# kchmck/p25rx

Measured on AMD Instinct MI355X. Metric: IQ Msamples/s through FM-demod+C4FM slice, higher is better.
Workload: dtype f32

## Files before the change

p25rx_amd/csrc/p25fe_api.hip:

```cpp
#include "p25fe_kernels.hip"

#include <hip/hip_ext.h>
#include <math.h>
#include <stdio.h>
#include <stdlib.h>
#include <string.h>

#include <chrono>
#include <new>
#include <utility>
#include <string>
#include <vector>

#include "p25fe_jit.h"

using namespace p25k;

namespace {

constexpr size_t BBPAD = 256;
constexpr size_t SHARD_HALO = 2560;
static_assert(SHARD_HALO >= (size_t)(DEC * (PLPAD + CLK_L + 160) + TMAX) && 160 >= TMAX + TMAX - 1 && SHARD_HALO % 8 == 0, "shard halo");
constexpr uint32_t STATE_MAGIC = 0x50323546u;

struct DevBuf {
    void* p = nullptr;
    size_t cap = 0;
    DevBuf() = default; DevBuf(const DevBuf&) = delete; DevBuf& operator=(const DevBuf&) = delete;
    ~DevBuf() { release(); }
    hipError_t ensure(size_t bytes)
    {
        if (bytes <= cap) return hipSuccess;
        if (p) { hipError_t e = hipFree(p); if (e != hipSuccess) return e; p = nullptr; cap = 0; }
        size_t want = bytes + bytes / 8 + 256;
        hipError_t e = hipMalloc(&p, want);
        if (e != hipSuccess) { p = nullptr; return e; }
        cap = want;
        return hipSuccess;
    }
    void release() { if (p) (void)hipFree(p); p = nullptr; cap = 0; }
    template <class T> T* as() const { return reinterpret_cast<T*>(p); }
};
template <class T> struct DevArr {
    DevBuf buf;
    hipError_t ensure(size_t count) { return buf.ensure(count * sizeof(T)); }
    T* get() const { return static_cast<T*>(buf.p); }
};

struct PinBuf {
    void* p = nullptr;
    void* dp = nullptr;
    size_t cap = 0;
    PinBuf() = default; PinBuf(const PinBuf&) = delete; PinBuf& operator=(const PinBuf&) = delete;
    ~PinBuf() { release(); }
    hipError_t ensure(size_t bytes)
    {
        if (bytes <= cap) return hipSuccess;
        release();
        const size_t want = bytes + bytes / 4 + 4096;
        hipError_t e = hipHostMalloc(&p, want, hipHostMallocCoherent | hipHostMallocMapped);
        if (e != hipSuccess) { (void)hipGetLastError(); e = hipHostMalloc(&p, want, hipHostMallocDefault); }
        if (e != hipSuccess) { p = nullptr; return e; }
        e = hipHostGetDevicePointer(&dp, p, 0);
        if (e != hipSuccess) { (void)hipHostFree(p); p = dp = nullptr; return e; }
        cap = want;
        return hipSuccess;
    }
    void release() { if (p) (void)hipHostFree(p); p = dp = nullptr; cap = 0; }
};

inline size_t round_up(size_t v, size_t m) { return (v + m - 1) / m * m; }

struct Arena {
    char* hp; char* dp; size_t off = 0;
    Arena(const PinBuf& b) : hp(static_cast<char*>(b.p)), dp(static_cast<char*>(b.dp)) {}
    template <class T> T* take(size_t count, T** dev)
    {
        T* r = reinterpret_cast<T*>(hp + off);
        *dev = reinterpret_cast<T*>(dp + off);
        off += round_up(count * sizeof(T), 64);
        return r;
    }
};

template <class... Args, class... Act>
inline void launch_ev(void (*kern)(Args...), dim3 grid, dim3 block, size_t lds, hipStream_t st, hipEvent_t e0, hipEvent_t e1,
                      Act... args)
{
    if (e0 || e1) hipExtLaunchKernelGGL(kern, grid, block, (uint32_t)lds, st, e0, e1, 0u, Args(args)...);
    else hipLaunchKernelGGL(kern, grid, block, lds, st, Args(args)...);
}
inline size_t fmt_bytes(int fmt) { return fmt == P25FE_FMT_CF32 ? 8 : 2; }

static_assert(BBPAD == (size_t)TAILN && BBPAD >= (size_t)HIST_BB + CLK_L, "baseband tail kept between calls");

constexpr int MAX_LANES = 4;
constexpr int SH_FLAG_WORDS = 8, SH_FLAG_ERR = 4;
constexpr int PROF_RING = 64, PROF_SAMPLE = 8;

struct RxScratch {
    DevArr<float> pl_f; DevArr<uint32_t> pl_bits;
    DevArr<uint16_t> evl; DevArr<float> evthr;
    DevArr<TileRec> recs; DevArr<unsigned long long> tsum; DevArr<ScanOut> outs;
    DevArr<GroupAgg> gagg; DevArr<GroupPre> gpre; DevArr<unsigned> gtick;
    DevArr<TileSumG> gsum; DevArr<ScanOutG> gouts; DevArr<uint32_t> evg;
    DevArr<GroupSumG> gsg; DevArr<GroupPreG> gpg;
};

struct Lane {
    RxScratch s;
    hipEvent_t ev_k1 = nullptr, ev_rx = nullptr;
    bool pending = false;
    hipStream_t joined = nullptr; bool joined_any = false;
};

static inline void rotate_lanes(int* cur, int* q, int depth)
{
    const int next = q[0];
    for (int k = 0; k + 2 < depth; ++k) q[k] = q[k + 1];
    q[depth - 2] = *cur;
    *cur = next;
}

struct ShardCtx {
    bool valid = false;
    bool main_out = false;
    size_t main_nbb = 0; uint64_t main_abs0 = 0;
    bool head_done = false;
    bool head_flagged = false;
    DevBuf flag;
    unsigned seq = 0; int head_tile_max = -1;
    size_t nbb = 0; long abs_bb0 = 0;
    bool gen = false;
    bool pipe = false;
    bool scan_fresh = false;
    bool main_is(size_t n_bb, uint64_t abs0) const { return main_out && main_nbb == n_bb && main_abs0 == abs0; }
    void invalidate() { valid = false; main_out = false; head_done = false; head_flagged = false; }
    void finish_pass1(size_t n_bb, long bb0, bool general) { valid = true; nbb = n_bb; abs_bb0 = bb0; gen = general; scan_fresh = true; main_out = false; head_done = false; }
};

struct StateHeader { uint32_t magic, abi; int32_t n_channels, fmt_locked; uint64_t abs_iq, abs_bb; };

struct StreamState {
    uint64_t abs_iq = 0, abs_bb = 0;
    int fmt_locked = -1;
    std::vector<char> hist_iq;
    std::vector<float> tail_bb;
    std::vector<p25fe_anchor_t> anchor;
    std::vector<uint64_t> total_dibits;
    void reset(size_t C)
    {
        abs_iq = 0; fmt_locked = -1; abs_bb = 0;
        anchor.assign(C, p25fe_anchor_t{0, 0.f, 0.f, 0.f, 0, SPS, 1}); total_dibits.assign(C, 0);
        hist_iq.assign(C * SHARD_HALO * 8, 0); tail_bb.assign(C * BBPAD, 0.f);
    }
    bool format_refused(int fmt) const { return fmt_locked >= 0 && fmt_locked != fmt && abs_iq > 0; }
    size_t n_hist() const { return abs_iq < SHARD_HALO ? (size_t)abs_iq : SHARD_HALO; }
    void commit_iq(size_t C, int fmt, size_t n, const char* fresh, size_t row_bytes)
    {
        const size_t eb = fmt_bytes(fmt);
        for (size_t c = 0; c < C; ++c) {
            char* hist = hist_iq.data() + c * SHARD_HALO * 8;
            const char* src = fresh + c * row_bytes;
            if (n >= SHARD_HALO) memcpy(hist, src + (n - SHARD_HALO) * eb, SHARD_HALO * eb);
            else { memmove(hist, hist + n * eb, (SHARD_HALO - n) * eb); memcpy(hist + (SHARD_HALO - n) * eb, src, n * eb); }
        }
        fmt_locked = fmt; abs_iq += n;
    }
    void merge_tail(size_t c, size_t nb, long look, const float* fresh)
    {
        float* t = tail_bb.data() + c * BBPAD;
        float merged[BBPAD];
        for (size_t j = 0; j < (size_t)BBPAD; ++j) {
            const long m = (long)nb - (long)BBPAD + (long)j;
            merged[j] = m >= -(long)(HIST_BB + look) ? fresh[j] : t[j + nb];
        }
        memcpy(t, merged, sizeof merged);
    }
    struct Sec { void* p; size_t bytes; };
    void sections(Sec s[4])
    {
        s[0] = {hist_iq.data(), hist_iq.size()}; s[1] = {tail_bb.data(), tail_bb.size() * sizeof(float)};
        s[2] = {anchor.data(), anchor.size() * sizeof(p25fe_anchor_t)}; s[3] = {total_dibits.data(), total_dibits.size() * sizeof(uint64_t)};
    }
    size_t blob_size() { Sec s[4]; sections(s); return sizeof(StateHeader) + s[0].bytes + s[1].bytes + s[2].bytes + s[3].bytes; }
    void write(char* p)
    {
        StateHeader hd = {STATE_MAGIC, P25FE_ABI_VERSION, (int32_t)anchor.size(), fmt_locked, abs_iq, abs_bb};
        memcpy(p, &hd, sizeof hd); p += sizeof hd;
        Sec s[4]; sections(s);
        for (int k = 0; k < 4; ++k) { memcpy(p, s[k].p, s[k].bytes); p += s[k].bytes; }
    }
    bool read(const char* p, int track)
    {
        StateHeader hd;
        memcpy(&hd, p, sizeof hd); p += sizeof hd;
        if (hd.magic != STATE_MAGIC || hd.abi != P25FE_ABI_VERSION || hd.n_channels != (int32_t)anchor.size()) return false;
        if (hd.fmt_locked != -1 && hd.fmt_locked != P25FE_FMT_U8 && hd.fmt_locked != P25FE_FMT_CF32) return false;
        if (hd.abs_iq >= P25FE_MAX_POSITION || hd.abs_bb >= P25FE_MAX_POSITION) return false;
        Sec s[4]; sections(s);
        for (size_t c = 0; c < anchor.size(); ++c) {
            p25fe_anchor_t a;
            memcpy(&a, p + s[0].bytes + s[1].bytes + c * sizeof a, sizeof a);
            if (!(a.period_d == 0 && a.period_n == 0) && !clock_plausible(a.period_d, a.period_n)) return false;
            if (!track && a.valid != 0 && !(a.period_d == 0 && a.period_n == 0) && !(a.period_d == SPS && a.period_n == 1)) return false;
            if (a.valid != 0 && (a.s >= (int64_t)P25FE_MAX_POSITION || a.s <= -(int64_t)P25FE_MAX_POSITION)) return false;
        }
        for (int k = 0; k < 4; ++k) { memcpy(s[k].p, p, s[k].bytes); p += s[k].bytes; }
        fmt_locked = hd.fmt_locked; abs_iq = hd.abs_iq; abs_bb = hd.abs_bb;
        return true;
    }
};

struct Prof {
    bool on = false;
    int level = 1;
    std::vector<hipEvent_t> ev;
    std::vector<uint8_t> mask;
    uint64_t calls = 0, seq = 0;
    int slot = -1;
    void begin()
    {
        if (on && level == 3 && (seq++ % PROF_SAMPLE) != 0) { slot = -1; return; }
        slot = on ? (int)(calls++ % PROF_RING) : -1;
        if (slot >= 0) mask[(size_t)slot] = 0;
    }
    void end() { slot = -1; }
    void mark(int idx, hipStream_t st, bool ext_events)
    {
        if (slot < 0 || (idx > 1 && level != 1) || (idx <= 1 && ext_events)) return;
        if (hipEventRecord(ev[(size_t)slot * 5 + idx], st) == hipSuccess) mask[(size_t)slot] |= (uint8_t)(1u << idx);
    }
    void k1_events(bool ext_events, hipEvent_t* e0, hipEvent_t* e1)
    {
        *e0 = *e1 = nullptr;
        if (slot < 0 || !ext_events) return;
        *e0 = ev[(size_t)slot * 5 + 0]; *e1 = ev[(size_t)slot * 5 + 1];
        mask[(size_t)slot] |= 3u;
    }
};

struct Windows {
    DevBuf buf[2], dib[2], res, anc;
    PinBuf stage[2], out;
    hipStream_t cs = nullptr, os = nullptr;
    hipEvent_t ev[4][5] = {};
    hipError_t ensure()
    {
        if (cs) return hipSuccess;
        hipError_t e = hipStreamCreateWithFlags(&cs, hipStreamNonBlocking);
        if (e == hipSuccess) e = hipStreamCreateWithFlags(&os, hipStreamNonBlocking);
        for (auto& slot : ev) for (hipEvent_t& x : slot) if (e == hipSuccess) e = hipEventCreate(&x);
        return e;
    }
};

}

struct p25fe {
    p25fe_config_t cfg;
    int C = 1, n_cu = 256;
    Taps taps;
    int k1_p = 5;
    int variant = P25FE_VARIANT_BUILTIN;
    bool long_taps = false;
    int phase = P25FE_DECIM_PHASE;
    int n_avg = BOX;
    bool u8_lut_mode = false;
    int track = 0;
    bool causal_ok = false;
    long look = 0;
    bool ext_events = true;
    int rx_cus = 0;
    int run_depth = 2;
    int sh_depth = MAX_LANES;

    int last_hip = 0;
    DevBuf d_taps;
    hipModule_t jit_mod = nullptr;
    hipFunction_t jit_fn[2][3] = {{nullptr, nullptr, nullptr}, {nullptr, nullptr, nullptr}};
    hipStream_t stream = nullptr, rx_stream = nullptr;
    const long* rs_idx = nullptr; size_t rs_n = 0, rs_stride = 0;
    Lane lanes[MAX_LANES];
    int cur = 0, lane_q[MAX_LANES - 1] = {1, 2, 3};
    Lane& lane() { return lanes[cur]; }
    RxScratch& rx() { return lanes[cur].s; }
    const RxScratch& rx() const { return lanes[cur].s; }
    DevBuf power_partial, chunk_cnt, evrec, evnext, evoff;
    unsigned long long ev_seq = 0;
    PinBuf hin, hbb, hout;
    unsigned chunk_seq = 0;
    Windows win; StreamState state; Prof prof; ShardCtx sh;
};

struct PlanarGeo {
    size_t n_tiles, n_blocks;
    explicit PlanarGeo(size_t n_bb)
    {
        n_tiles = (n_bb + TS - 1) / TS;
        if (n_tiles == 0) n_tiles = 1;
        n_blocks = (size_t)TWORDS * n_tiles + 6;
    }
    size_t floats() const { return n_blocks * PL_BLK; }
    size_t words() const { return n_blocks * SPS; }
};

constexpr size_t MAX_RANGE_BB = (size_t)0x7ff00000u * 10u;
static inline bool position_refused(uint64_t pos) { return pos >= P25FE_MAX_POSITION; }

struct Resolved {
    Taps taps;
    bool long_taps;
    bool lut_affine;
    float u8_scale, u8_offset;
    bool dflt;
};

static inline bool finite_f(float v) { return v - v == 0.0f; }
static inline bool same_bits(float a, float b) { return memcmp(&a, &b, sizeof a) == 0; }

static bool lut_is_affine(const float* lut, float sc, float of)
{
    for (int b = 0; b < 256; ++b)
        if (!same_bits(lut[b], fmaf((float)b, sc, of))) return false;
    return true;
}

static int resolve_config(const p25fe_config_t* cfg, Resolved* r)
{
    if (cfg->abi_version != P25FE_ABI_VERSION || cfg->n_decim_taps < 1 || cfg->n_decim_taps > P25FE_MAX_TAPS || cfg->n_chan_taps < 1 ||
        cfg->n_chan_taps > P25FE_MAX_TAPS || (cfg->symbol_clock != P25FE_CLOCK_FIXED && cfg->symbol_clock != P25FE_CLOCK_TRACKING && cfg->symbol_clock != P25FE_CLOCK_TRACKING_RESLICE &&
         cfg->symbol_clock != (P25FE_CLOCK_TRACKING_RESLICE | P25FE_CLOCK_CAUSAL_OK)) ||
        cfg->specialize < P25FE_SPECIALIZE_OFF || cfg->specialize > P25FE_SPECIALIZE_FORCE || cfg->decim_phase < 0 || cfg->decim_phase >= DEC ||
        cfg->n_avg_taps < 1 || cfg->n_avg_taps > P25FE_MAX_TAPS)
        return P25FE_ERR_ARG;
    memset(&r->taps, 0, sizeof r->taps);
    r->taps.n_avg = cfg->n_avg_taps;
    r->taps.avg_uniform = 1;
    for (int k = 0; k < cfg->n_avg_taps; ++k) {
        if (!finite_f(cfg->avg_taps[k])) return P25FE_ERR_ARG;
        r->taps.avg[k] = cfg->avg_taps[k];
        if (!same_bits(cfg->avg_taps[k], cfg->avg_taps[0])) r->taps.avg_uniform = 0;
    }
    for (int k = 0; k < cfg->n_decim_taps; ++k) { if (!finite_f(cfg->decim_taps[k])) return P25FE_ERR_ARG; r->taps.dec[k] = cfg->decim_taps[k]; }
    for (int k = 0; k < cfg->n_chan_taps; ++k) { if (!finite_f(cfg->chan_taps[k])) return P25FE_ERR_ARG; r->taps.ch[k] = cfg->chan_taps[k]; }
    r->long_taps = cfg->n_decim_taps > P25FE_T1 || cfg->n_chan_taps > P25FE_T2;
    if (cfg->fm_gain != 0.0f) {
        if (!finite_f(cfg->fm_gain)) return P25FE_ERR_ARG;
        r->taps.fm_gain = cfg->fm_gain;
    } else {
        if (cfg->fm_deviation_hz == 0 || cfg->fm_sample_rate_hz == 0) return P25FE_ERR_ARG;
        r->taps.fm_gain = (float)((double)cfg->fm_sample_rate_hz / (2.0 * M_PI * (double)cfg->fm_deviation_hz));
    }
    if (cfg->u8_lut_valid) {
        for (int b = 0; b < 256; ++b) { if (!finite_f(cfg->u8_lut[b])) return P25FE_ERR_ARG; r->taps.lut[b] = cfg->u8_lut[b]; }
        const float* L = r->taps.lut;
        const float cand[3][2] = {{cfg->u8_scale, cfg->u8_offset}, {L[1] - L[0], L[0]},
                                  {(float)(((double)L[255] - (double)L[0]) / 255.0), L[0]}};
        r->lut_affine = false;
        for (int c = 0; c < 3 && !r->lut_affine; ++c)
            if (finite_f(cand[c][0]) && finite_f(cand[c][1]) && lut_is_affine(L, cand[c][0], cand[c][1])) {
                r->lut_affine = true; r->u8_scale = cand[c][0]; r->u8_offset = cand[c][1];
            }
        if (!r->lut_affine) r->u8_scale = r->u8_offset = 0.0f;
    } else {
        if (!finite_f(cfg->u8_scale) || !finite_f(cfg->u8_offset)) return P25FE_ERR_ARG;
        r->lut_affine = true; r->u8_scale = cfg->u8_scale; r->u8_offset = cfg->u8_offset;
        for (int b = 0; b < 256; ++b) r->taps.lut[b] = fmaf((float)b, cfg->u8_scale, cfg->u8_offset);
    }
    Taps def;
    memset(&def, 0, sizeof def);
    memcpy(def.dec, P25FE_DEFAULT_DECIM_TAPS, sizeof(float) * P25FE_T1);
    memcpy(def.ch, P25FE_DEFAULT_CHAN_TAPS, sizeof(float) * P25FE_T2);
    memcpy(def.avg, P25FE_DEFAULT_AVG_TAPS, sizeof(float) * BOX);
    r->dflt = !r->long_taps && memcmp(def.dec, r->taps.dec, sizeof def.dec) == 0 && memcmp(def.ch, r->taps.ch, sizeof def.ch) == 0 &&
              r->taps.n_avg == BOX && memcmp(def.avg, r->taps.avg, sizeof def.avg) == 0 &&
              same_bits(r->taps.fm_gain, P25FE_FM_GAIN) && r->lut_affine && same_bits(r->u8_scale, P25FE_U8_SCALE) &&
              same_bits(r->u8_offset, P25FE_U8_OFFSET);
    return P25FE_OK;
}

static p25jit::Spec jit_spec(const Resolved& r)
{
    p25jit::Spec s;
    memset(&s, 0, sizeof s);
    s.tx = r.long_taps ? 1 : 0;
    s.t1 = r.long_taps ? TMAX : T1;
    s.t2 = r.long_taps ? TMAX : T2;
    memcpy(s.dec, r.taps.dec, sizeof s.dec);
    memcpy(s.ch, r.taps.ch, sizeof s.ch);
    s.fm_gain = r.taps.fm_gain;
    s.u8_lut = r.lut_affine ? 0 : 1;
    s.u8_scale = r.u8_scale; s.u8_offset = r.u8_offset;
    s.n_avg = r.taps.n_avg; s.avg_uniform = r.taps.avg_uniform;
    memcpy(s.avg, r.taps.avg, sizeof s.avg);
    return s;
}

static thread_local std::string t_jit_log;

static std::vector<std::string> jit_dirs()
{
    std::vector<std::string> d;
    const char* e = getenv("P25FE_SPEC_DIR");
    if (e && *e) d.push_back(e);
    d.push_back(p25jit::default_cache_dir());
    return d;
}

static void fallback_notice()
{
    static bool said = false;
    if (said) return;
    said = true;
    const char* q = getenv("P25FE_QUIET");
    if (q && atoi(q) != 0) return;
    fprintf(stderr, "p25fe: no specialised kernels for this configuration's numbers (no usable cached code object and hipRTC did not "
                    "deliver one): running the GENERIC kernels, 1.3 - 2.4 x slower.  p25fe_specialize_log() has the details; "
                    "p25fe_specialize() / $P25FE_SPEC_DIR is the ahead-of-time form.\n");
}

static int choose_variant(const p25fe_config_t* cfg, const Resolved& rs, std::vector<char>* code, std::string* path, bool* from_cache)
{
    static const bool jit_env_off = [] { const char* v = getenv("P25FE_JIT"); return v && atoi(v) == 0; }();
    const bool must = cfg->specialize >= P25FE_SPECIALIZE_REQUIRE;
    const bool want_jit = (!rs.dflt || cfg->specialize == P25FE_SPECIALIZE_FORCE) && cfg->specialize != P25FE_SPECIALIZE_OFF && !(jit_env_off && !must);
    const int plain = rs.dflt ? P25FE_VARIANT_BUILTIN : P25FE_VARIANT_GENERIC;
    if (!want_jit) return plain;
    bool ok = false;
    try {
        t_jit_log.clear();
        ok = p25jit::get_code(jit_spec(rs), jit_dirs(), true, p25jit::default_cache_dir(), false, *code, *path, t_jit_log, from_cache);
    } catch (...) {
        ok = false;
        try { t_jit_log += "exception while specialising\n"; } catch (...) { }
    }
    if (ok) return P25FE_VARIANT_SPECIALIZED;
    if (must) return P25FE_ERR_JIT;
    if (plain == P25FE_VARIANT_GENERIC) fallback_notice();
    return plain;
}

#define HIPCHK(h, expr)                                                        \
    do {                                                                       \
        hipError_t e__ = (expr);                                               \
        if (e__ != hipSuccess) { (h)->last_hip = (int)e__; return P25FE_ERR_HIP; } \
    } while (0)

extern "C" {

void p25fe_default_config(p25fe_config_t* cfg)
{
    if (!cfg) return;
    memset(cfg, 0, sizeof *cfg);
    cfg->abi_version = P25FE_ABI_VERSION;
    cfg->device = 0;
    cfg->n_channels = 1;
    cfg->n_decim_taps = P25FE_T1;
    cfg->n_chan_taps = P25FE_T2;
    memcpy(cfg->decim_taps, P25FE_DEFAULT_DECIM_TAPS, sizeof(float) * P25FE_T1);
    memcpy(cfg->chan_taps, P25FE_DEFAULT_CHAN_TAPS, sizeof(float) * P25FE_T2);
    cfg->specialize = P25FE_SPECIALIZE_AUTO;
    cfg->fm_deviation_hz = P25FE_FM_DEVIATION_HZ;
    cfg->fm_sample_rate_hz = P25FE_FM_SAMPLE_RATE_HZ;
    cfg->fm_gain = 0.0f;
    cfg->u8_scale = P25FE_U8_SCALE;
    cfg->u8_offset = P25FE_U8_OFFSET;
    cfg->u8_lut_valid = 0;
    cfg->decim_phase = P25FE_DECIM_PHASE;
    cfg->n_avg_taps = P25FE_BOXCAR;
    memcpy(cfg->avg_taps, P25FE_DEFAULT_AVG_TAPS, sizeof(float) * P25FE_BOXCAR);
}

const char* p25fe_strerror(int status)
{
    switch (status) {
    case P25FE_OK: return "ok";
    case P25FE_ERR_ARG: return "invalid argument";
    case P25FE_ERR_NO_DEVICE: return "no usable HIP device (gfx950 required; there is no CPU fallback)";
    case P25FE_ERR_HIP: return "HIP runtime error";
    case P25FE_ERR_CAPACITY: return "output buffer too small";
    case P25FE_ERR_FORMAT: return "sample format changed within a stream";
    case P25FE_ERR_NOMEM: return "out of memory";
    case P25FE_ERR_JIT: return "kernel specialisation failed (p25fe_specialize_log)";
    case P25FE_ERR_TIMEOUT: return "a device-side wait gave up (time shard: the head segment never arrived)";
    default: return "unknown status";
    }
}

int p25fe_last_hip_error(const p25fe_t* h) { return h ? h->last_hip : 0; }
int p25fe_device(const p25fe_t* h) { return h ? h->cfg.device : -1; }
int p25fe_kernel_variant(const p25fe_t* h) { return h ? h->variant : -1; }

size_t p25fe_specialize_log(char* buf, size_t cap)
{
    if (!buf || cap == 0) return 0;
    const size_t n = t_jit_log.size() < cap - 1 ? t_jit_log.size() : cap - 1;
    memcpy(buf, t_jit_log.data(), n);
    buf[n] = '\0';
    return n;
}

int p25fe_specialize(const p25fe_config_t* cfg, const char* dir, char* path_out, size_t path_cap)
{
    if (!cfg) return P25FE_ERR_ARG;
    if (path_out && path_cap) path_out[0] = '\0';
    Resolved r;
    const int rc = resolve_config(cfg, &r);
    if (rc) return rc;
    if (r.dflt && cfg->specialize != P25FE_SPECIALIZE_FORCE) return P25FE_OK;
    try {
        t_jit_log.clear();
        const std::string d = (dir && *dir) ? std::string(dir) : p25jit::default_cache_dir();
        std::vector<char> code;
        std::string path;
        if (!p25jit::get_code(jit_spec(r), {d}, true, d, true, code, path, t_jit_log) || path.empty()) return P25FE_ERR_JIT;
        if (path_out && path_cap) snprintf(path_out, path_cap, "%s", path.c_str());
    } catch (...) {
        return P25FE_ERR_NOMEM;
    }
    return P25FE_OK;
}

int p25fe_probe_variant(const p25fe_config_t* cfg)
{
    if (!cfg) return P25FE_ERR_ARG;
    Resolved r;
    const int rc = resolve_config(cfg, &r);
    if (rc) return rc;
    std::vector<char> code;
    std::string path;
    try {
        return choose_variant(cfg, r, &code, &path, nullptr);
    } catch (...) {
        return P25FE_ERR_NOMEM;
    }
}

static inline size_t n_baseband_ph(int phase, uint64_t abs0, size_t n)
{
    const size_t o0 = (size_t)(((uint64_t)phase + 5 - abs0 % 5) % 5);
    return n > o0 ? (n - o0 - 1) / 5 + 1 : 0;
}
size_t p25fe_n_baseband(uint64_t abs0, size_t n) { return n_baseband_ph(P25FE_DECIM_PHASE, abs0, n); }
size_t p25fe_n_baseband_h(const p25fe_t* h, uint64_t abs0, size_t n) { return n_baseband_ph(h ? h->phase : P25FE_DECIM_PHASE, abs0, n); }

size_t p25fe_shard_halo(void) { return SHARD_HALO; }

int p25fe_reset(p25fe_t* h)
{
    if (!h) return P25FE_ERR_ARG;
    h->rs_idx = nullptr; h->rs_n = 0; h->rs_stride = 0;
    try {
        h->state.reset((size_t)h->C);
    } catch (...) {
        return P25FE_ERR_NOMEM;
    }
    return P25FE_OK;
}

int p25fe_create(const p25fe_config_t* cfg, p25fe_t** out)
{
    if (!cfg || !out) return P25FE_ERR_ARG;
    *out = nullptr;
    if (cfg->abi_version != P25FE_ABI_VERSION || cfg->n_channels < 1 || cfg->n_channels > 65535 ) return P25FE_ERR_ARG;
    Resolved rs;
    if (int rrc = resolve_config(cfg, &rs)) return rrc;
    int ndev = 0;
    if (hipGetDeviceCount(&ndev) != hipSuccess || ndev <= 0 || cfg->device < 0 || cfg->device >= ndev)
        return P25FE_ERR_NO_DEVICE;
    if (hipSetDevice(cfg->device) != hipSuccess) return P25FE_ERR_NO_DEVICE;
    hipDeviceProp_t prop;
    if (hipGetDeviceProperties(&prop, cfg->device) != hipSuccess) return P25FE_ERR_NO_DEVICE;
    if (strncmp(prop.gcnArchName, "gfx950", 6) != 0) return P25FE_ERR_NO_DEVICE;

    p25fe_t* h = new (std::nothrow) p25fe;
    if (!h) return P25FE_ERR_NOMEM;
    h->cfg = *cfg;
    h->C = cfg->n_channels;
    h->track = cfg->symbol_clock & 0xff;
    h->causal_ok = (cfg->symbol_clock & P25FE_CLOCK_CAUSAL_OK) != 0;
    h->look = h->track ? CLK_L : 0;
    h->n_cu = prop.multiProcessorCount > 0 ? prop.multiProcessorCount : 256;
    h->taps = rs.taps;
    h->phase = cfg->decim_phase;
    h->n_avg = rs.taps.n_avg;
    h->long_taps = rs.long_taps;
    h->u8_lut_mode = !rs.lut_affine;
    h->variant = rs.dflt ? P25FE_VARIANT_BUILTIN : P25FE_VARIANT_GENERIC;
    if (hipStreamCreateWithFlags(&h->stream, hipStreamNonBlocking) != hipSuccess) { p25fe_destroy(h); return P25FE_ERR_HIP; }
    hipError_t e = hipSuccess;
    {
        const char* pv = getenv("P25FE_K1_P");
        h->k1_p = (pv && atoi(pv) == 3) ? 3 : 5;
        const char* ee = getenv("P25FE_EXT_EVENTS");
        h->ext_events = !(ee && atoi(ee) == 0);
        const char* rc_ = getenv("P25FE_RX_CUS");
        h->rx_cus = rc_ ? atoi(rc_) : 0;
        const char* pd = getenv("P25FE_SHARD_PIPE_DEPTH");
        if (pd && atoi(pd) >= 2 && atoi(pd) <= MAX_LANES) h->sh_depth = atoi(pd);
        if (cfg->symbol_clock != P25FE_CLOCK_FIXED) h->run_depth = 3;
        const char* rd = getenv("P25FE_PIPE_DEPTH");
        if (rd && atoi(rd) >= 2 && atoi(rd) <= MAX_LANES) h->run_depth = atoi(rd);
    }
    if (e == hipSuccess) e = h->d_taps.ensure(sizeof(Taps));
    if (e == hipSuccess) e = hipMemcpy(h->d_taps.p, &h->taps, sizeof(Taps), hipMemcpyHostToDevice);
    if (e != hipSuccess) { p25fe_destroy(h); return P25FE_ERR_HIP; }
    {
        std::vector<char> code;
        std::string path;
        bool from_cache = false;
        int var = choose_variant(cfg, rs, &code, &path, &from_cache);
        if (var < 0) { p25fe_destroy(h); return var; }
        if (var == P25FE_VARIANT_SPECIALIZED) {
            bool ok = false;
            try {
                hipError_t me = hipModuleLoadData(&h->jit_mod, code.data());
                if (me != hipSuccess && from_cache) {
                    (void)hipGetLastError();
                    t_jit_log += "cached code object " + path + " did not load: recompiling\n";
                    const std::string store = p25jit::default_cache_dir();
                    if (path.compare(0, store.size() + 1, store + "/") == 0) (void)remove(path.c_str());
                    h->jit_mod = nullptr;
                    if (p25jit::get_code(jit_spec(rs), {}, true, store, false, code, path, t_jit_log)) me = hipModuleLoadData(&h->jit_mod, code.data());
                }
                ok = me == hipSuccess;
                for (int f = 0; f < 2 && ok; ++f)
                    for (int k = 0; k < 3 && ok; ++k)
                        ok = hipModuleGetFunction(&h->jit_fn[f][k], h->jit_mod, p25jit::KERNEL_NAMES[f][k]) == hipSuccess;
                if (!ok) { (void)hipGetLastError(); t_jit_log += "loading the specialised code object failed\n"; }
            } catch (...) {
                ok = false;
            }
            if (!ok) {
                if (h->jit_mod) { (void)hipModuleUnload(h->jit_mod); h->jit_mod = nullptr; }
                if (cfg->specialize >= P25FE_SPECIALIZE_REQUIRE) { p25fe_destroy(h); return P25FE_ERR_JIT; }
                var = rs.dflt ? P25FE_VARIANT_BUILTIN : P25FE_VARIANT_GENERIC;
                if (var == P25FE_VARIANT_GENERIC) fallback_notice();
            }
        }
        h->variant = var;
    }
    int rc = p25fe_reset(h);
    if (rc != P25FE_OK) { p25fe_destroy(h); return rc; }
    *out = h;
    return P25FE_OK;
}

void p25fe_destroy(p25fe_t* h)
{
    if (!h) return;
    (void)hipSetDevice(h->cfg.device);
    for (hipStream_t st : {h->stream, h->rx_stream, h->win.cs, h->win.os})
        if (st) { (void)hipStreamSynchronize(st); (void)hipStreamDestroy(st); }
    if (h->jit_mod) (void)hipModuleUnload(h->jit_mod);
    for (auto& slot : h->win.ev) for (hipEvent_t e : slot) if (e) (void)hipEventDestroy(e);
    for (Lane& l : h->lanes)
        for (hipEvent_t e : {l.ev_k1, l.ev_rx}) if (e) (void)hipEventDestroy(e);
    for (auto& e : h->prof.ev) if (e) (void)hipEventDestroy(e);
    delete h;
}

}

enum K1Part { K1_ALL = 0, K1_MAIN = 1, K1_HEAD = 2 };
struct K1Launch {
    const void* src = nullptr;
    int fmt = P25FE_FMT_CF32;
    size_t ch_stride = 0, n_hist = 0, n = 0;
    uint64_t abs0 = 0;
    float* bb = nullptr; size_t bb_stride = 0;
    float* power_dbm = nullptr;
    bool planar = false;
    K1Part part = K1_ALL;
    hipEvent_t ev0 = nullptr, ev1 = nullptr;
    const ChunkRecvArgs* chunk = nullptr;
    long* head_end = nullptr;
    unsigned* done_flag = nullptr; unsigned done_seq = 0u;
    hipStream_t stream = nullptr;
};

struct K1Plan {
    bool empty;
    K1Args a;
    bool u8, ct; int pk;
    long n_seg;
    long head_end;
    size_t lds;
};
static int k1_plan(const p25fe_t* h, const K1Launch& L, K1Plan* p)
{
    const int fmt = L.fmt;
    if (fmt != P25FE_FMT_CF32 && fmt != P25FE_FMT_U8) return P25FE_ERR_ARG;
    if ((reinterpret_cast<uintptr_t>(L.src) & 15u) != 0) return P25FE_ERR_ARG;
    if (h->C > 1 && (L.ch_stride % (fmt == P25FE_FMT_CF32 ? 2 : 8)) != 0) return P25FE_ERR_ARG;
    if (L.chunk && (!L.planar || L.part)) return P25FE_ERR_ARG;
    const bool pro = seg_prologue(fmt);
    const long m_begin = !L.planar ? 0 : (pro ? -(long)PLPAD - h->look : -(long)HIST_BB - h->look);
    const size_t n_out = p25fe_n_baseband_h(h, L.abs0, L.n);
    const long total = (long)n_out - m_begin;
    K1Args& a = p->a;
    a.m_begin = m_begin; a.n_out = (long)n_out; p->head_end = 0;
    p->empty = total <= 0;
    if (p->empty) return P25FE_OK;
    const int pk = (L.planar || h->long_taps || h->variant == P25FE_VARIANT_SPECIALIZED) ? 5 : h->k1_p;
    const int t1 = h->long_taps ? TMAX : T1;
    const long sub = (long)WV * pk;
    static const long subs_env = [] { const char* e = getenv("P25FE_SUBS"); return e ? atol(e) : 0L; }();
    long subs = subs_env > 0 ? subs_env : (fmt == P25FE_FMT_U8 ? 9 : 3);
    if (L.chunk) subs = 1;
    if (subs > 32768) subs = 32768;
    const bool ct = h->variant != P25FE_VARIANT_GENERIC;
    const int t2e = h->long_taps ? TMAX : T2;
    const int t3geo = ct ? h->n_avg : TMAX;
    const long segh = seg_halo_for(h->n_avg, t2e);
    const long seg_len = pro ? subs * sub : (sub - segh) + (subs - 1) * sub;
    const long nd = pro ? t3geo + t2e - 1 : segh;
    const long lead_len = pro ? sub : sub - segh;
    const long o0 = (long)(((uint64_t)h->phase + 5 - L.abs0 % 5) % 5);
    long lead = 0;
    if (L.part && subs > 1 && !L.chunk)
        while (lead < 64 && o0 + DEC * (m_begin + lead * lead_len - nd) - (t1 - 1) < 0 && lead * lead_len < total) ++lead;
    auto seg_start = [&](long k) { return k < lead ? m_begin + k * lead_len : m_begin + lead * lead_len + (k - lead) * seg_len; };
    const long n_seg = lead * lead_len >= total ? (total + lead_len - 1) / lead_len : lead + (total - lead * lead_len + seg_len - 1) / seg_len;
    const long pl_shift = PLPAD + h->look;
    if (L.planar && pro && (m_begin + pl_shift < 0 || (m_begin + pl_shift) % PL_BLK != 0 || seg_len % PL_BLK != 0)) return P25FE_ERR_ARG;
    if (L.planar && !pro && (m_begin + pl_shift < 0 || (m_begin + pl_shift) % 80 != 0 || seg_len % 80 != 0)) return P25FE_ERR_ARG;
    if (L.planar && n_out > MAX_RANGE_BB) return P25FE_ERR_ARG;
    long seg_first = 0, seg_count = n_seg;
    if (L.part) {
        if (L.power_dbm) return P25FE_ERR_ARG;
        long k_min = 0;
        while (k_min < n_seg && o0 + DEC * (seg_start(k_min) - nd) - (t1 - 1) < 0) ++k_min;
        if (L.part == K1_MAIN) { seg_first = k_min; seg_count = n_seg - k_min; }
        else seg_count = k_min;
        p->head_end = seg_start(k_min) - m_begin;
        p->empty = seg_count <= 0;
        if (p->empty) return P25FE_OK;
    }
    if (seg_count * (long)h->C > 0x7fffffffL) return P25FE_ERR_ARG;
    p->u8 = fmt == P25FE_FMT_U8; p->ct = ct; p->pk = pk; p->n_seg = n_seg;
    a.x = L.src; a.ch_stride = (long)L.ch_stride; a.n_hist = (long)L.n_hist; a.n_new = (long)L.n; a.o0 = (int)o0; a.n_ch = h->C;
    a.bb = L.bb; a.bb_stride = (long)L.bb_stride; a.power_partial = nullptr;
    a.subs_per_seg = (int)subs; a.seg_first = (int)seg_first; a.seg_count = (int)seg_count; a.lead_segs = (int)lead; a.seg_halo = (int)segh;
    a.bbp = nullptr; a.bbp_ch_stride = 0; a.bits = nullptr; a.bits_ch_stride = 0; a.pl_shift = (int)pl_shift;
    a.done_flag = L.planar ? L.done_flag : nullptr; a.done_seq = L.done_seq;
    if (L.planar) {
        const PlanarGeo g(n_out);
        a.bbp = h->rx().pl_f.get(); a.bbp_ch_stride = (long)g.floats();
        a.bits = reinterpret_cast<uint8_t*>(h->rx().pl_bits.get()); a.bits_ch_stride = (long)(4 * g.words());
    }
    const bool lut = p->u8 && (!ct || h->u8_lut_mode);
    p->lds = h->long_taps ? k1_lds_bytes<Geo<5, 1>>(ct, lut, t3geo) : (pk == 3 ? k1_lds_bytes<Geo<3>>(ct, lut, t3geo) : k1_lds_bytes<Geo<5>>(ct, lut, t3geo));
    static const size_t lds_pad_env = [] { const char* e = getenv("P25FE_K1_LDS_PAD"); return e ? (size_t)atol(e) : (size_t)0; }();
    p->lds += lds_pad_env;
    return P25FE_OK;
}

using K1Kernel = void (*)(K1Args, const Taps*);
using ChunkKernel = void (*)(K1Args, const Taps*, ChunkTail);
template <int FMT> static K1Kernel k1_kernel_of(bool ct, int pk, bool planar, bool long_taps)
{
    if (long_taps) return planar ? k_frontend<FMT, false, 5, OUT_PLANAR, 1> : k_frontend<FMT, false, 5, OUT_LINEAR, 1>;
    if (planar) return ct ? k_frontend<FMT, true, 5, OUT_PLANAR, 0> : k_frontend<FMT, false, 5, OUT_PLANAR, 0>;
    if (pk == 3) return ct ? k_frontend<FMT, true, 3, OUT_LINEAR, 0> : k_frontend<FMT, false, 3, OUT_LINEAR, 0>;
    return ct ? k_frontend<FMT, true, 5, OUT_LINEAR, 0> : k_frontend<FMT, false, 5, OUT_LINEAR, 0>;
}
template <int FMT> static ChunkKernel chunk_kernel_of(bool ct, bool long_taps)
{
    if (long_taps) return k_chunk<FMT, false, 1>;
    return ct ? k_chunk<FMT, true, 0> : k_chunk<FMT, false, 0>;
}

static int launch_k1(p25fe_t* h, const K1Launch& L)
{
    K1Plan p;
    if (int rc = k1_plan(h, L, &p)) return rc;
    if (L.head_end) *L.head_end = p.head_end;
    hipStream_t st = L.stream;
    if (p.empty) {
        if (L.power_dbm) HIPCHK(h, hipMemsetAsync(L.power_dbm, 0xff, sizeof(float) * (size_t)h->C, st));
        return P25FE_OK;
    }
    K1Args& a = p.a;
    if (L.power_dbm) {
        HIPCHK(h, h->power_partial.ensure(sizeof(float) * (size_t)h->C * (size_t)p.n_seg));
        a.power_partial = h->power_partial.as<float>();
    }
    ChunkTail tail;
    if (L.chunk) {
        if (!h->chunk_cnt.p) {
            HIPCHK(h, h->chunk_cnt.ensure(sizeof(unsigned) * (size_t)h->C));
            HIPCHK(h, hipMemsetAsync(h->chunk_cnt.p, 0, sizeof(unsigned) * (size_t)h->C, h->stream));
        }
        tail.r = *L.chunk; tail.counter = h->chunk_cnt.as<unsigned>(); tail.wg_per_ch = a.seg_count;
    }
    const Taps* dt = h->d_taps.as<Taps>();
    const dim3 grid((unsigned)a.seg_count, (unsigned)h->C);
    if (h->variant == P25FE_VARIANT_SPECIALIZED) {
        hipFunction_t f = h->jit_fn[p.u8 ? 1 : 0][L.chunk ? 2 : (L.planar ? 1 : 0)];
        void* params[3] = {&a, &dt, &tail};
        if (L.ev0 || L.ev1)
            HIPCHK(h, hipExtModuleLaunchKernel(f, grid.x * WV, grid.y, 1, WV, 1, 1, p.lds, st, params, nullptr, L.ev0, L.ev1, 0));
        else
            HIPCHK(h, hipModuleLaunchKernel(f, grid.x, grid.y, 1, WV, 1, 1, (unsigned)p.lds, st, params, nullptr));
    } else if (L.chunk) {
        const ChunkKernel k = p.u8 ? chunk_kernel_of<P25FE_FMT_U8>(p.ct, h->long_taps) : chunk_kernel_of<P25FE_FMT_CF32>(p.ct, h->long_taps);
        hipLaunchKernelGGL(k, grid, dim3(WV), p.lds, st, a, dt, tail);
    } else {
        const K1Kernel k = p.u8 ? k1_kernel_of<P25FE_FMT_U8>(p.ct, p.pk, L.planar, h->long_taps)
                                : k1_kernel_of<P25FE_FMT_CF32>(p.ct, p.pk, L.planar, h->long_taps);
        launch_ev(k, grid, dim3(WV), p.lds, st, L.ev0, L.ev1, a, dt);
    }
    HIPCHK(h, hipGetLastError());
    if (L.power_dbm) {
        hipLaunchKernelGGL(k_power_finish, dim3((unsigned)h->C), dim3(256), 0, st, a.power_partial, (int)p.n_seg, a.n_out, L.power_dbm);
        HIPCHK(h, hipGetLastError());
    }
    return P25FE_OK;
}

static int ensure_slice_scratch(p25fe_t* h, size_t n_bb)
{
    const size_t C = (size_t)h->C;
    const PlanarGeo g(n_bb);
    const size_t nt = C * g.n_tiles, ng = C * (size_t)n_groups_of((int)g.n_tiles);
    RxScratch& s = h->rx();
    HIPCHK(h, s.pl_f.ensure(C * g.floats())); HIPCHK(h, s.pl_bits.ensure(C * g.words()));
    HIPCHK(h, s.evl.ensure(nt * EVCAP)); HIPCHK(h, s.evthr.ensure(nt * EVTHR_N * 3));
    HIPCHK(h, s.recs.ensure(nt)); HIPCHK(h, s.tsum.ensure(nt)); HIPCHK(h, s.outs.ensure(nt));
    HIPCHK(h, s.gagg.ensure(ng)); HIPCHK(h, s.gpre.ensure(ng));
    const unsigned* before = s.gtick.get();
    HIPCHK(h, s.gtick.ensure(ng + C));
    if (s.gtick.get() != before) HIPCHK(h, hipMemset(s.gtick.get(), 0, s.gtick.buf.cap));
    if (h->track || h->rs_n) {
        HIPCHK(h, s.gsum.ensure(nt)); HIPCHK(h, s.gouts.ensure(nt)); HIPCHK(h, s.evg.ensure(nt * EVCAP));
        HIPCHK(h, s.gsg.ensure(ng)); HIPCHK(h, s.gpg.ensure(ng));
    }
    return P25FE_OK;
}

struct RecvRange {
    size_t n_bb = 0;
    long abs_bb0 = 0;
    const p25fe_anchor_t* anchor_in = nullptr;
};
struct RecvDest {
    uint8_t* dibits = nullptr; size_t dibit_stride = 0;
    uint8_t* dibits2 = nullptr;
    int64_t* sync_pos = nullptr; uint64_t* sync_dibit = nullptr;
    size_t sync_stride = 0;
    p25fe_result_t* result = nullptr;
};
struct RecvCall {
    bool gen = false;
    bool reslice = false;
    RecvOpt opt;
    RecvRange range;
    RecvDest dest;
    bool detect = true;
    bool slice = true;
    bool wait_head = false;
    const ShardFix* fix = nullptr;
    hipEvent_t ev_done = nullptr;
    hipStream_t stream = nullptr;
};
static RecvCall recv_call(const p25fe_t* h)
{
    RecvCall c;
    c.opt.track = h->track;
    c.opt.n_resync = (int)h->rs_n;
    c.opt.resync = h->rs_idx;
    c.opt.resync_stride = (long)h->rs_stride;
    c.gen = h->track != 0 || h->rs_n != 0;
    return c;
}
static inline int n_tiles_of(const RecvRange& r) { return r.n_bb ? (int)PlanarGeo(r.n_bb).n_tiles : 0; }

static Planar planar_view(const p25fe_t* h, const PlanarGeo& g)
{
    Planar p;
    p.f = h->rx().pl_f.get(); p.f_ch = (long)g.floats();
    p.bits = h->rx().pl_bits.get(); p.bits_ch = (long)g.words();
    return p;
}

template <class A> static void view_planes(const p25fe_t* h, const RecvRange& r, A* a)
{
    a->pl = planar_view(h, PlanarGeo(r.n_bb)); a->n = (long)r.n_bb; a->abs0 = r.abs_bb0;
    a->evl = h->rx().evl.get(); a->evthr = h->rx().evthr.get();
}
template <class A> static void view_tiles(const p25fe_t* h, A* a) { a->recs = h->rx().recs.get(); a->tsum = h->rx().tsum.get(); }
template <class A> static void view_general(const p25fe_t* h, A* a) { a->gsum = h->rx().gsum.get(); a->evg = h->rx().evg.get(); }
template <class A> static void view_scan(const p25fe_t* h, const RecvCall& rc, A* a)
{
    a->recs = h->rx().recs.get(); a->tickets = h->rx().gtick.get();
    a->n_tiles = n_tiles_of(rc.range); a->n = (long)rc.range.n_bb; a->abs0 = rc.range.abs_bb0; a->n_baseband = rc.range.n_bb;
    a->anchor_in = rc.range.anchor_in; a->result = rc.dest.result;
}
template <class A> static void view_dest(const RecvRange& r, const RecvDest& d, A* a)
{
    a->anchor_in = r.anchor_in;
    a->dibits = d.dibits; a->dibit_stride = (long)d.dibit_stride;
    a->sync_pos = (d.sync_pos && d.sync_dibit) ? d.sync_pos : nullptr; a->sync_dibit = d.sync_dibit; a->sync_stride = (long)d.sync_stride;
}

static int launch_planarize(p25fe_t* h, const float* d_bb, size_t bb_stride, size_t n_hist_bb, size_t n_bb, hipStream_t st)
{
    const PlanarGeo g(n_bb);
    PlanarizeArgs a;
    a.bb = d_bb; a.bb_stride = (long)bb_stride; a.n_hist = (long)n_hist_bb; a.n = (long)n_bb;
    a.f = h->rx().pl_f.get(); a.f_ch = (long)g.floats();
    a.bits = h->rx().pl_bits.get(); a.bits_ch = (long)g.words(); a.n_blocks = (long)g.n_blocks;
    a.shift = (int)h->look;
    hipLaunchKernelGGL(k_planarize, dim3((unsigned)((g.n_blocks + 1) / 2), (unsigned)h->C), dim3(WV * SPS), 0, st, a);
    HIPCHK(h, hipGetLastError());
    return P25FE_OK;
}

static int launch_detect(p25fe_t* h, const RecvCall& rc)
{
    DetArgs d;
    d.head_flag = nullptr; d.head_seq = 0u; d.head_tile_max = -1; d.head_err = nullptr;
    if (rc.wait_head) {
        d.head_flag = h->sh.flag.as<unsigned>(); d.head_seq = h->sh.seq; d.head_tile_max = h->sh.head_tile_max;
        d.head_err = h->sh.flag.as<unsigned>() + SH_FLAG_ERR;
    }
    view_planes(h, rc.range, &d); view_tiles(h, &d); view_general(h, &d);
    d.n_tiles = n_tiles_of(rc.range); d.opt = rc.opt;
    const dim3 grid((unsigned)d.n_tiles, (unsigned)h->C);
    if (rc.gen) hipLaunchKernelGGL(k_detect<true>, grid, dim3(WV), 0, rc.stream, d);
    else hipLaunchKernelGGL(k_detect<false>, grid, dim3(WV), 0, rc.stream, d);
    HIPCHK(h, hipGetLastError());
    return P25FE_OK;
}

enum ScanStep { SCAN_WHOLE, SCAN_RANGE, SCAN_TILES_G };
static int launch_scan(p25fe_t* h, const RecvCall& rc, ScanStep step, hipEvent_t ev_done)
{
    const dim3 grid = step == SCAN_RANGE ? dim3((unsigned)h->C) : dim3((unsigned)n_groups_of(n_tiles_of(rc.range)), (unsigned)h->C);
    if (rc.gen) {
        ScanArgsG c;
        view_scan(h, rc, &c);
        c.gsum = h->rx().gsum.get(); c.outs = h->rx().gouts.get(); c.gsg = h->rx().gsg.get(); c.gpg = h->rx().gpg.get();
        c.track = h->track;
        launch_ev(step == SCAN_WHOLE ? k_scan_tiles_g : step == SCAN_RANGE ? k_range_scan_g : k_scan_g_groups, grid, dim3(WV), 0, rc.stream,
                  nullptr, ev_done, c);
    } else {
        ScanArgs c;
        view_scan(h, rc, &c);
        c.tsum = h->rx().tsum.get(); c.outs = h->rx().outs.get(); c.gagg = h->rx().gagg.get(); c.gpre = h->rx().gpre.get();
        launch_ev(step == SCAN_WHOLE ? k_scan_tiles : k_range_scan, grid, dim3(WV), 0, rc.stream, nullptr, ev_done, c);
    }
    HIPCHK(h, hipGetLastError());
    return P25FE_OK;
}

static int launch_slice(p25fe_t* h, const RecvCall& rc)
{
    SliceArgs l;
    view_planes(h, rc.range, &l); view_tiles(h, &l); view_dest(rc.range, rc.dest, &l);
    l.n_tiles = n_tiles_of(rc.range); l.outs = h->rx().outs.get(); l.gpre = h->rx().gpre.get(); l.dibits2 = rc.dest.dibits2;
    if (rc.fix) l.fix = *rc.fix; else memset(&l.fix, 0, sizeof l.fix);
    launch_ev(k_slice, dim3((unsigned)l.n_tiles + (rc.fix ? 1u : 0u), (unsigned)h->C), dim3(WV), 0, rc.stream, nullptr, rc.ev_done, l);
    HIPCHK(h, hipGetLastError());
    return P25FE_OK;
}

static int launch_slice_g(p25fe_t* h, const RecvCall& rc)
{
    SliceArgsG l;
    view_planes(h, rc.range, &l); view_general(h, &l); view_dest(rc.range, rc.dest, &l);
    l.n_tiles = n_tiles_of(rc.range); l.outs = h->rx().gouts.get(); l.recs = h->rx().recs.get();
    l.track = h->track; l.dibits2 = rc.dest.dibits2;
    launch_ev(k_slice_g, dim3((unsigned)l.n_tiles, (unsigned)h->C), dim3(WV), 0, rc.stream, nullptr, rc.ev_done, l);
    HIPCHK(h, hipGetLastError());
    return P25FE_OK;
}

static int launch_slice_by_detection(p25fe_t* h, const RecvCall& rc)
{
    const size_t C = (size_t)h->C, n_bb = rc.range.n_bb;
    const int n_tiles = n_tiles_of(rc.range);
    hipStream_t st = rc.stream;
    size_t cap_ev = (size_t)n_tiles * EVCAP;
    const size_t bound = n_bb / (size_t)(W + 1) + (size_t)n_tiles + 8;
    if (bound < cap_ev) cap_ev = bound;
    const size_t stride = cap_ev + 2;
    HIPCHK(h, h->evrec.ensure(C * stride * sizeof(EvRec)));
    HIPCHK(h, h->evoff.ensure(C * (stride + 1) * sizeof(unsigned long long)));
    {
        const void* before = h->evnext.p;
        HIPCHK(h, h->evnext.ensure(C * stride * sizeof(EvNext)));
        if (h->evnext.p != before) HIPCHK(h, hipMemsetAsync(h->evnext.p, 0, h->evnext.cap, st));
    }
    EvArgs e;
    view_planes(h, rc.range, &e); view_general(h, &e); view_dest(rc.range, rc.dest, &e);
    e.n_tiles = n_tiles; e.outs = h->rx().gouts.get();
    e.rec = h->evrec.as<EvRec>(); e.nxt = h->evnext.as<EvNext>(); e.off = h->evoff.as<unsigned long long>();
    e.ev_stride = (long)stride; e.seq = ++h->ev_seq; e.result = rc.dest.result;
    hipLaunchKernelGGL(k_ev_collect, dim3((unsigned)n_tiles, (unsigned)h->C), dim3(WV), 0, st, e);
    HIPCHK(h, hipGetLastError());
    hipLaunchKernelGGL(k_ev_count, dim3((unsigned)(n_tiles < 1024 ? n_tiles : 1024), (unsigned)h->C), dim3(WV), 0, st, e);
    HIPCHK(h, hipGetLastError());
    hipLaunchKernelGGL(k_ev_scan, dim3((unsigned)h->C), dim3(WV), 0, st, e);
    HIPCHK(h, hipGetLastError());
    const size_t max_dibits = n_bb / (SPS - 1) + (size_t)n_tiles + 64;
    const size_t lim = rc.dest.dibit_stride < max_dibits ? rc.dest.dibit_stride : max_dibits;
    launch_ev(k_ev_slice, dim3((unsigned)((lim + WV * 4 - 1) / (WV * 4)), (unsigned)h->C), dim3(WV), 0, st, nullptr, rc.ev_done, e);
    HIPCHK(h, hipGetLastError());
    return P25FE_OK;
}

static int launch_recv(p25fe_t* h, const RecvCall& rc)
{
    const int n_tiles = n_tiles_of(rc.range);
    const bool detect = rc.detect && n_tiles != 0, slice = rc.slice && n_tiles != 0, scan = rc.fix == nullptr;
    hipStream_t st = rc.stream;
    int e = detect ? launch_detect(h, rc) : P25FE_OK;
    if (e) return e;
    h->prof.mark(2, st, h->ext_events);
    if (scan && (e = launch_scan(h, rc, detect ? SCAN_WHOLE : SCAN_RANGE, slice ? nullptr : rc.ev_done)) != P25FE_OK) return e;
    h->prof.mark(3, st, h->ext_events);
    if (slice) {
        if (!rc.gen) e = launch_slice(h, rc);
        else if ((e = launch_scan(h, rc, SCAN_TILES_G, nullptr)) == P25FE_OK) e = rc.reslice ? launch_slice_by_detection(h, rc) : launch_slice_g(h, rc);
        if (e) return e;
    }
    if (rc.ev_done && !scan && !slice) HIPCHK(h, hipEventRecord(rc.ev_done, st));
    h->prof.mark(4, st, h->ext_events);
    return P25FE_OK;
}

static int launch_k1_planar(p25fe_t* h, K1Launch& k, hipEvent_t k1_done, hipStream_t waiter)
{
    h->prof.mark(0, k.stream, h->ext_events);
    bool attached = false;
    if (p25fe_n_baseband_h(h, k.abs0, k.n)) {
        h->prof.k1_events(h->ext_events, &k.ev0, &k.ev1);
        if (k1_done && h->ext_events) {
            if (k.ev1) k1_done = k.ev1;
            else k.ev1 = k1_done;
            attached = true;
        }
        k.planar = true;
        if (int rc = launch_k1(h, k)) return rc;
    }
    if (k1_done) {
        if (!attached) HIPCHK(h, hipEventRecord(k1_done, k.stream));
        HIPCHK(h, hipStreamWaitEvent(waiter, k1_done, 0));
    }
    return P25FE_OK;
}

static int launch_planar_recv(p25fe_t* h, K1Launch& k, const RecvCall& rc, hipEvent_t k1_done = nullptr)
{
    if (int e = launch_k1_planar(h, k, k1_done, rc.stream)) return e;
    if (rc.range.n_bb) h->prof.mark(1, k.stream, h->ext_events);
    return launch_recv(h, rc);
}

static inline bool piecewise_refused(const p25fe_t* h) { return h->track == P25FE_CLOCK_TRACKING_RESLICE && !h->causal_ok; }

extern "C" {

int p25fe_demod_dev(p25fe_t* h, const void* d_iq, int fmt, size_t ch_stride, size_t n_hist, size_t n, uint64_t abs0,
                    float* d_bb, size_t bb_stride, float* d_power_dbm, void* stream)
{
    if (!h || !d_iq || !d_bb || position_refused(abs0)) return P25FE_ERR_ARG;
    HIPCHK(h, hipSetDevice(h->cfg.device));
    K1Launch k;
    k.src = d_iq; k.fmt = fmt; k.ch_stride = ch_stride; k.n_hist = n_hist; k.n = n; k.abs0 = abs0;
    k.bb = d_bb; k.bb_stride = bb_stride; k.power_dbm = d_power_dbm; k.stream = (hipStream_t)stream;
    return launch_k1(h, k);
}

size_t p25fe_n_predecim(uint64_t abs0, size_t n)
{
    const size_t o0 = (size_t)((PD - 1 + PD - abs0 % PD) % PD);
    return n > o0 ? (n - o0 - 1) / PD + 1 : 0;
}

int p25fe_predecim_dev(p25fe_t* h, const float* d_iq, size_t ch_stride, size_t n_hist, size_t n, uint64_t abs0,
                       float* d_out, size_t out_stride, void* stream)
{
    if (!h || !d_iq || !d_out || position_refused(abs0)) return P25FE_ERR_ARG;
    if ((reinterpret_cast<uintptr_t>(d_iq) & 15u) != 0 || (h->C > 1 && (ch_stride & 1))) return P25FE_ERR_ARG;
    HIPCHK(h, hipSetDevice(h->cfg.device));
    const size_t n_out = p25fe_n_predecim(abs0, n);
    if (n_out == 0) return P25FE_OK;
    K0Args a;
    a.x = d_iq; a.ch_stride = (long)ch_stride; a.n_hist = (long)n_hist; a.n_new = (long)n;
    a.o0 = (int)((PD - 1 + PD - abs0 % PD) % PD);
    a.y = d_out; a.y_stride = (long)out_stride; a.n_out = (long)n_out;
    const size_t per_wg = (size_t)K0_SUB * K0_SUBS;
    dim3 grid((unsigned)((n_out + per_wg - 1) / per_wg), (unsigned)h->C);
    hipLaunchKernelGGL(k_predecim, grid, dim3(WV), 0, (hipStream_t)stream, a);
    HIPCHK(h, hipGetLastError());
    return P25FE_OK;
}

int p25fe_channelise_dev(p25fe_t* h, const float* d_iq, size_t n_hist, size_t n, uint64_t abs0, float* d_out,
                         size_t out_stride, void* stream)
{
    static_assert(P25FE_CHZ_CHANNELS_ABI == CZ_M, "header and spec disagree");
    if (!h || !d_iq || !d_out || position_refused(abs0)) return P25FE_ERR_ARG;
    if ((reinterpret_cast<uintptr_t>(d_iq) & 15u) != 0 || (reinterpret_cast<uintptr_t>(d_out) & 7u) != 0) return P25FE_ERR_ARG;
    HIPCHK(h, hipSetDevice(h->cfg.device));
    const size_t n_out = p25fe_n_predecim(abs0, n);
    if (n_out == 0) return P25FE_OK;
    if (out_stride < round_up(n_out, (size_t)WV)) return P25FE_ERR_ARG;
    ChzArgs a;
    a.x = d_iq; a.n_hist = (long)n_hist; a.n_new = (long)n; a.abs0 = (long)abs0;
    a.o0 = (int)((PD - 1 + PD - abs0 % PD) % PD);
    a.y = d_out; a.y_stride = (long)out_stride; a.n_out = (long)n_out;
    hipLaunchKernelGGL(k_channelise, dim3((unsigned)((n_out + WV - 1) / WV)), dim3(WV), 0, (hipStream_t)stream, a);
    HIPCHK(h, hipGetLastError());
    return P25FE_OK;
}

static int pipe_join(p25fe_t* h, hipStream_t st)
{
    for (Lane& l : h->lanes)
        if (l.pending && !(l.joined_any && l.joined == st)) {
            HIPCHK(h, hipStreamWaitEvent(st, l.ev_rx, 0));
            l.joined = st; l.joined_any = true;
        }
    return P25FE_OK;
}

int p25fe_slice_dev(p25fe_t* h, const float* d_bb, size_t bb_stride, size_t n_hist_bb, size_t n_bb, uint64_t abs_bb0,
                    const p25fe_anchor_t* d_anchor_in, uint8_t* d_dibits, size_t dibit_stride, int64_t* d_sync_pos,
                    uint64_t* d_sync_dibit, size_t sync_stride, p25fe_result_t* d_result, void* stream)
{
    if (!h || !d_bb || !d_dibits || !d_result || position_refused(abs_bb0)) return P25FE_ERR_ARG;
    HIPCHK(h, hipSetDevice(h->cfg.device));
    if (n_bb > MAX_RANGE_BB) return P25FE_ERR_ARG;
    hipStream_t st = (hipStream_t)stream;
    h->sh.invalidate();
    if (int jrc = pipe_join(h, st)) return jrc;
    int rc = ensure_slice_scratch(h, n_bb ? n_bb : 1);
    if (rc) return rc;
    RecvCall rcall = recv_call(h);
    rcall.reslice = h->track == P25FE_CLOCK_TRACKING_RESLICE;
    h->rs_n = 0;
    rcall.range.n_bb = n_bb; rcall.range.anchor_in = d_anchor_in;
    rcall.range.abs_bb0 = (long)abs_bb0 - h->look;
    rcall.dest.dibits = d_dibits; rcall.dest.dibit_stride = dibit_stride; rcall.dest.result = d_result;
    rcall.dest.sync_pos = d_sync_pos; rcall.dest.sync_dibit = d_sync_dibit; rcall.dest.sync_stride = sync_stride;
    rcall.stream = st;
    if (n_bb)
        if ((rc = launch_planarize(h, d_bb, bb_stride, n_hist_bb, n_bb, st)) != P25FE_OK) return rc;
    return launch_recv(h, rcall);
}

int p25fe_join_dev(p25fe_t* h, void* stream)
{
    if (!h) return P25FE_ERR_ARG;
    HIPCHK(h, hipSetDevice(h->cfg.device));
    return pipe_join(h, (hipStream_t)stream);
}

static int ensure_rx_stream(p25fe_t* h)
{
    if (!h->rx_stream) {
        if (h->rx_cus > 0) {
            uint32_t mask[8] = {0, 0, 0, 0, 0, 0, 0, 0};
            const int ncu = h->n_cu < 256 ? h->n_cu : 256;
            const int want = h->rx_cus < ncu ? h->rx_cus : ncu;
            for (int k = 0; k < want; ++k) mask[k / 32] |= 1u << (k % 32);
            if (hipExtStreamCreateWithCUMask(&h->rx_stream, (uint32_t)((ncu + 31) / 32), mask) != hipSuccess) {
                (void)hipGetLastError();
                h->rx_stream = nullptr;
            }
        }
        if (!h->rx_stream) {
            int prio_lo = 0, prio_hi = 0;
            if (hipDeviceGetStreamPriorityRange(&prio_lo, &prio_hi) != hipSuccess ||
                hipStreamCreateWithPriority(&h->rx_stream, hipStreamNonBlocking, prio_hi) != hipSuccess) {
                (void)hipGetLastError();
                h->rx_stream = nullptr;
                HIPCHK(h, hipStreamCreateWithFlags(&h->rx_stream, hipStreamNonBlocking));
            }
        }
    }
    return P25FE_OK;
}
static int pipe_open(p25fe_t* h, hipStream_t st, int depth = 2)
{
    if (int rc = ensure_rx_stream(h)) return rc;
    for (Lane& l : h->lanes) {
        if (!l.ev_k1) HIPCHK(h, hipEventCreateWithFlags(&l.ev_k1, hipEventDisableTiming));
        if (!l.ev_rx) HIPCHK(h, hipEventCreateWithFlags(&l.ev_rx, hipEventDisableTiming));
    }
    rotate_lanes(&h->cur, h->lane_q, depth);
    Lane& l = h->lane();
    if (l.pending) {
        const bool nowait = P25FE_M_PIPE_NOWAIT();
        if (!nowait && !(l.joined_any && l.joined == st)) HIPCHK(h, hipStreamWaitEvent(st, l.ev_rx, 0));
        l.pending = false;
    }
    l.joined_any = false;
    return P25FE_OK;
}

static int run_dev(p25fe_t* h, const void* d_iq, int fmt, size_t ch_stride, size_t n, const RecvDest& dest, hipStream_t st, bool pipelined)
{
    if (!h || !d_iq || !dest.dibits || !dest.result || p25fe_n_baseband_h(h, 0, n) > MAX_RANGE_BB) return P25FE_ERR_ARG;
    HIPCHK(h, hipSetDevice(h->cfg.device));
    h->sh.invalidate();
    if (int orc = pipelined ? pipe_open(h, st, h->run_depth) : pipe_join(h, st)) return orc;
    Lane& lane = h->lane();
    const size_t n_bb = p25fe_n_baseband_h(h, 0, n);
    int rc = ensure_slice_scratch(h, n_bb ? n_bb : 1);
    if (rc) return rc;
    RecvCall rcall = recv_call(h);
    rcall.reslice = h->track == P25FE_CLOCK_TRACKING_RESLICE;
    h->rs_n = 0;
    rcall.range.n_bb = n_bb; rcall.range.abs_bb0 = -h->look;
    rcall.dest = dest;
    rcall.stream = pipelined ? h->rx_stream : st;
    if (pipelined && h->ext_events) rcall.ev_done = lane.ev_rx;
    K1Launch k;
    k.src = d_iq; k.fmt = fmt; k.ch_stride = ch_stride; k.n = n; k.stream = st;
    if (n_bb) h->prof.begin();
    rc = launch_planar_recv(h, k, rcall, pipelined ? lane.ev_k1 : nullptr);
    h->prof.end();
    if (rc || !pipelined) return rc;
    if (!h->ext_events) HIPCHK(h, hipEventRecord(lane.ev_rx, h->rx_stream));
    lane.pending = true;
    return P25FE_OK;
}

int p25fe_run_dev_pipelined(p25fe_t* h, const void* d_iq, int fmt, size_t ch_stride, size_t n, uint8_t* d_dibits,
                            size_t dibit_stride, p25fe_result_t* d_result, void* stream)
{
    RecvDest dest;
    dest.dibits = d_dibits; dest.dibit_stride = dibit_stride; dest.result = d_result;
    return run_dev(h, d_iq, fmt, ch_stride, n, dest, (hipStream_t)stream, true);
}

int p25fe_run_dev(p25fe_t* h, const void* d_iq, int fmt, size_t ch_stride, size_t n, uint8_t* d_dibits,
                  size_t dibit_stride, p25fe_result_t* d_result, void* stream)
{
    RecvDest dest;
    dest.dibits = d_dibits; dest.dibit_stride = dibit_stride; dest.result = d_result;
    return run_dev(h, d_iq, fmt, ch_stride, n, dest, (hipStream_t)stream, false);
}

enum { SH_MAIN = 1, SH_HEAD = 2, SH_RECV = 4 };
static int shard_pass1_part(p25fe_t* h, const void* d_iq, int fmt, size_t ch_stride, size_t n_hist, size_t n, uint64_t abs0,
                            p25fe_result_t* d_result, hipStream_t st, int what)
{
    const bool do_main = (what & SH_MAIN) != 0, do_finish = (what & SH_RECV) != 0;
    bool do_head = (what & SH_HEAD) != 0;
    if (!h || !d_iq || (do_finish && !d_result) || position_refused(abs0) || p25fe_n_baseband_h(h, abs0, n) > MAX_RANGE_BB || piecewise_refused(h)) return P25FE_ERR_ARG;
    if (do_main) h->sh.invalidate();
    if (n_hist < SHARD_HALO && n_hist != abs0) return P25FE_ERR_ARG;
    HIPCHK(h, hipSetDevice(h->cfg.device));
    if (!h->sh.pipe)
        if (int jrc = pipe_join(h, st)) return jrc;
    const size_t n_bb = p25fe_n_baseband_h(h, abs0, n);
    const long abs_bb0 = (long)p25fe_n_baseband_h(h, 0, (size_t)abs0) - h->look;
    int rc = ensure_slice_scratch(h, n_bb ? n_bb : 1);
    if (rc) return rc;
    K1Launch k;
    k.src = d_iq; k.fmt = fmt; k.ch_stride = ch_stride; k.n_hist = n_hist; k.n = n; k.abs0 = abs0; k.planar = true; k.stream = st;
    if (do_main) {
        h->prof.begin();
        k.part = do_head ? K1_ALL : K1_MAIN;
        rc = launch_k1_planar(h, k, h->sh.pipe ? h->lane().ev_k1 : nullptr, h->rx_stream);
        if (rc) return rc;
        h->sh.main_out = true; h->sh.main_nbb = n_bb; h->sh.main_abs0 = abs0;
        h->sh.head_done = do_head;
        do_head = false;
    } else {
        if (!h->sh.main_is(n_bb, abs0)) return P25FE_ERR_ARG;
    }
    if ((do_head || do_finish) && !h->sh.head_done) {
        long head_end = 0;
        const bool own_stream = !do_finish;
        h->sh.head_flagged = false;
        if (n_bb) {
            if (own_stream) {
                if (!h->sh.flag.p) {
                    HIPCHK(h, h->sh.flag.ensure(SH_FLAG_WORDS * sizeof(unsigned)));
                    HIPCHK(h, hipMemsetAsync(h->sh.flag.p, 0, SH_FLAG_WORDS * sizeof(unsigned), st));
                }
                ++h->sh.seq;
                if (h->sh.seq == 0u) ++h->sh.seq;
            }
            k.part = K1_HEAD; k.ev0 = k.ev1 = nullptr; k.head_end = &head_end;
            k.done_flag = own_stream ? h->sh.flag.as<unsigned>() : nullptr; k.done_seq = h->sh.seq;
            rc = launch_k1(h, k);
            if (rc) return rc;
            if (own_stream && head_end > 0) {
                h->sh.head_flagged = true;
                h->sh.head_tile_max = (int)(head_end / TS);
            }
        }
        h->sh.head_done = true;
    }
    if (!do_finish) return P25FE_OK;
    h->prof.mark(1, st, h->ext_events);
    RecvCall rcall = recv_call(h);
    h->rs_n = 0;
    rcall.range.n_bb = n_bb; rcall.range.abs_bb0 = abs_bb0;
    rcall.dest.result = d_result;
    rcall.slice = false; rcall.wait_head = h->sh.head_flagged; rcall.stream = st;
    rc = launch_recv(h, rcall);
    h->sh.head_flagged = false;
    h->prof.end();
    if (rc) return rc;
    h->sh.finish_pass1(n_bb, abs_bb0, rcall.gen);
    return P25FE_OK;
}

int p25fe_shard_pass1(p25fe_t* h, const void* d_iq, int fmt, size_t ch_stride, size_t n_hist, size_t n, uint64_t abs0,
                      p25fe_result_t* d_result, void* stream)
{
    return shard_pass1_part(h, d_iq, fmt, ch_stride, n_hist, n, abs0, d_result, (hipStream_t)stream, SH_MAIN | SH_HEAD | SH_RECV);
}

int p25fe_shard_pass1_main(p25fe_t* h, const void* d_iq, int fmt, size_t ch_stride, size_t n_hist, size_t n, uint64_t abs0,
                           void* stream)
{
    return shard_pass1_part(h, d_iq, fmt, ch_stride, n_hist, n, abs0, nullptr, (hipStream_t)stream, SH_MAIN);
}

int p25fe_shard_pass1_head(p25fe_t* h, const void* d_iq, int fmt, size_t ch_stride, size_t n_hist, size_t n, uint64_t abs0,
                           void* stream)
{
    return shard_pass1_part(h, d_iq, fmt, ch_stride, n_hist, n, abs0, nullptr, (hipStream_t)stream, SH_HEAD);
}

int p25fe_shard_pass1_k1(p25fe_t* h, const void* d_iq, int fmt, size_t ch_stride, size_t n_hist, size_t n, uint64_t abs0, void* stream)
{
    return shard_pass1_part(h, d_iq, fmt, ch_stride, n_hist, n, abs0, nullptr, (hipStream_t)stream, SH_MAIN | SH_HEAD);
}

int p25fe_shard_pass1_finish(p25fe_t* h, const void* d_iq, int fmt, size_t ch_stride, size_t n_hist, size_t n, uint64_t abs0,
                             p25fe_result_t* d_result, void* stream)
{
    return shard_pass1_part(h, d_iq, fmt, ch_stride, n_hist, n, abs0, d_result, (hipStream_t)stream, SH_RECV);
}

int p25fe_shard_pipe_begin(p25fe_t* h, void* stream, void** rx_stream)
{
    if (!h || !rx_stream || h->sh.pipe) return P25FE_ERR_ARG;
    HIPCHK(h, hipSetDevice(h->cfg.device));
    h->sh.invalidate();
    if (int orc = pipe_open(h, (hipStream_t)stream, h->sh_depth)) return orc;
    h->sh.pipe = true;
    *rx_stream = h->rx_stream;
    return P25FE_OK;
}

int p25fe_rx_stream(p25fe_t* h, void** rx_stream)
{
    if (!h || !rx_stream) return P25FE_ERR_ARG;
    HIPCHK(h, hipSetDevice(h->cfg.device));
    if (int rc = ensure_rx_stream(h)) return rc;
    *rx_stream = h->rx_stream;
    return P25FE_OK;
}

int p25fe_shard_pipe_end(p25fe_t* h, void* last_stream)
{
    if (!h || !h->sh.pipe) return P25FE_ERR_ARG;
    h->sh.pipe = false;
    HIPCHK(h, hipSetDevice(h->cfg.device));
    HIPCHK(h, hipEventRecord(h->lane().ev_rx, last_stream ? (hipStream_t)last_stream : h->rx_stream));
    h->lane().pending = true;
    return P25FE_OK;
}

static RecvCall shard_pass2_call(const p25fe_t* h, const p25fe_anchor_t* d_anchor_in, uint8_t* d_dibits, size_t dibit_stride, p25fe_result_t* d_result,
                                 hipStream_t st)
{
    RecvCall c = recv_call(h);
    c.gen = h->sh.gen;
    c.detect = false;
    c.range.n_bb = h->sh.nbb; c.range.abs_bb0 = h->sh.abs_bb0; c.range.anchor_in = d_anchor_in;
    c.dest.dibits = d_dibits; c.dest.dibit_stride = dibit_stride; c.dest.result = d_result;
    c.stream = st;
    return c;
}

int p25fe_shard_pass2(p25fe_t* h, const p25fe_anchor_t* d_anchor_in, uint8_t* d_dibits, size_t dibit_stride,
                      p25fe_result_t* d_result, void* stream)
{
    if (!h || !d_dibits || !d_result || !h->sh.valid) return P25FE_ERR_ARG;
    HIPCHK(h, hipSetDevice(h->cfg.device));
    RecvCall rcall = shard_pass2_call(h, d_anchor_in, d_dibits, dibit_stride, d_result, (hipStream_t)stream);
    h->sh.scan_fresh = false;
    h->prof.begin();
    const int rc = launch_recv(h, rcall);
    h->prof.end();
    return rc;
}

int p25fe_shard_pass2_dev(p25fe_t* h, const p25fe_result_t* d_summaries, const uint64_t* d_shard_bb0, const uint64_t* d_shard_bb_n,
                          size_t n_shards, size_t rank, p25fe_anchor_t* d_anchor_in, uint64_t* d_dibit_offset, uint8_t* d_dibits,
                          size_t dibit_stride, uint8_t* d_dibits_dup, p25fe_result_t* d_result, void* stream)
{
    if (!h || !d_summaries || !d_shard_bb0 || !d_shard_bb_n || !d_anchor_in || !d_dibit_offset || !d_dibits || !d_result || !h->sh.valid ||
        n_shards == 0 || n_shards > 0x7fffffffu || rank >= n_shards || h->C != 1)
        return P25FE_ERR_ARG;
    HIPCHK(h, hipSetDevice(h->cfg.device));
    hipStream_t st = (hipStream_t)stream;
    RecvCall rcall = shard_pass2_call(h, d_anchor_in + rank, d_dibits, dibit_stride, d_result, st);
    rcall.dest.dibits2 = d_dibits_dup;
    ShardFix fx;
    if (rcall.gen || !h->sh.scan_fresh || h->sh.nbb == 0) {
        h->sh.scan_fresh = false;
        hipLaunchKernelGGL(k_shard_resolve, dim3(1), dim3(64), 0, st, d_summaries, d_shard_bb0, d_shard_bb_n, (int)n_shards, h->track,
                           d_anchor_in, d_dibit_offset);
        HIPCHK(h, hipGetLastError());
    } else {
        fx.summ = d_summaries; fx.bb0 = d_shard_bb0; fx.bbn = d_shard_bb_n; fx.n_shards = (int)n_shards; fx.rank = (int)rank;
        fx.anc_out = d_anchor_in; fx.off_out = d_dibit_offset; fx.result = d_result;
        rcall.range.anchor_in = nullptr; rcall.fix = &fx;
    }
    h->prof.begin();
    const int rc = launch_recv(h, rcall);
    h->prof.end();
    return rc;
}

int p25fe_shard_resolve(const p25fe_result_t* summaries, const uint64_t* shard_bb0, const uint64_t* shard_bb_n,
                        size_t n_shards, int symbol_clock, p25fe_anchor_t* anchor_in, uint64_t* dibit_offset)
{
    if (!summaries || !shard_bb0 || !shard_bb_n || !anchor_in || !dibit_offset || n_shards > 0x7fffffffu) return P25FE_ERR_ARG;
    for (size_t r = 0; r < n_shards; ++r)
        if (position_refused(shard_bb0[r]) || position_refused(shard_bb_n[r]) || position_refused(shard_bb0[r] + shard_bb_n[r])) return P25FE_ERR_ARG;
    shard_resolve_impl(summaries, shard_bb0, shard_bb_n, (int)n_shards, symbol_clock, anchor_in, dibit_offset);
    return P25FE_OK;
}

int p25fe_shard_resolve_dev(p25fe_t* h, const p25fe_result_t* d_summaries, const uint64_t* d_shard_bb0,
                            const uint64_t* d_shard_bb_n, size_t n_shards, p25fe_anchor_t* d_anchor_in,
                            uint64_t* d_dibit_offset, void* stream)
{
    if (!h || !d_summaries || !d_shard_bb0 || !d_shard_bb_n || !d_anchor_in || !d_dibit_offset || n_shards > 0x7fffffffu) return P25FE_ERR_ARG;
    HIPCHK(h, hipSetDevice(h->cfg.device));
    hipLaunchKernelGGL(k_shard_resolve, dim3(1), dim3(64), 0, (hipStream_t)stream, d_summaries, d_shard_bb0, d_shard_bb_n,
                       (int)n_shards, h->track, d_anchor_in, d_dibit_offset);
    HIPCHK(h, hipGetLastError());
    return P25FE_OK;
}

int p25fe_shard_head_check(p25fe_t* h)
{
    if (!h) return P25FE_ERR_ARG;
    if (!h->sh.flag.p) return P25FE_OK;
    HIPCHK(h, hipSetDevice(h->cfg.device));
    unsigned err = 0u;
    HIPCHK(h, hipMemcpy(&err, h->sh.flag.as<unsigned>() + SH_FLAG_ERR, sizeof err, hipMemcpyDeviceToHost));
    return err ? P25FE_ERR_TIMEOUT : P25FE_OK;
}

int p25fe_streams_share_queue(p25fe_t* h, void* stream_a, void* stream_b, int* shared)
{
    if (!h || !shared) return P25FE_ERR_ARG;
    *shared = 0;
    if (stream_a == stream_b) { *shared = 1; return P25FE_OK; }
    HIPCHK(h, hipSetDevice(h->cfg.device));
    if (!h->sh.flag.p) {
        HIPCHK(h, h->sh.flag.ensure(SH_FLAG_WORDS * sizeof(unsigned)));
        HIPCHK(h, hipMemset(h->sh.flag.p, 0, SH_FLAG_WORDS * sizeof(unsigned)));
    }
    unsigned* w = h->sh.flag.as<unsigned>() + 2;
    HIPCHK(h, hipStreamSynchronize((hipStream_t)stream_a));
    HIPCHK(h, hipStreamSynchronize((hipStream_t)stream_b));
    int votes = 0;
    for (int rep = 0; rep < 3; ++rep) {
        HIPCHK(h, hipMemset(w, 0, 2 * sizeof(unsigned)));
        hipLaunchKernelGGL(k_queue_probe_wait, dim3(1), dim3(1), 0, (hipStream_t)stream_a, w, 20000ull);
        hipLaunchKernelGGL(k_queue_probe_set, dim3(1), dim3(1), 0, (hipStream_t)stream_b, w);
        HIPCHK(h, hipGetLastError());
        HIPCHK(h, hipStreamSynchronize((hipStream_t)stream_a));
        HIPCHK(h, hipStreamSynchronize((hipStream_t)stream_b));
        unsigned r[2] = {0u, 0u};
        HIPCHK(h, hipMemcpy(r, w, sizeof r, hipMemcpyDeviceToHost));
        if (r[1] == 2u) ++votes;
    }
    *shared = votes == 3;
    return P25FE_OK;
}

int p25fe_shard_compact_dev(p25fe_t* h, const uint8_t* d_gathered, size_t cap, const uint64_t* d_dibit_offset,
                            size_t n_shards, uint8_t* d_out, size_t out_cap, void* stream)
{
    if (!h || !d_gathered || !d_dibit_offset || !d_out || n_shards == 0 || n_shards > 65535) return P25FE_ERR_ARG;
    HIPCHK(h, hipSetDevice(h->cfg.device));
    const unsigned bx = (unsigned)((cap + 256 * 16 - 1) / (256 * 16));
    hipLaunchKernelGGL(k_shard_compact, dim3(bx ? bx : 1, (unsigned)n_shards), dim3(256), 0, (hipStream_t)stream, d_gathered,
                       (unsigned long long)cap, d_dibit_offset, 0, (int)n_shards, d_out, (unsigned long long)out_cap);
    HIPCHK(h, hipGetLastError());
    return P25FE_OK;
}

int p25fe_shard_compact_from_dev(p25fe_t* h, const uint8_t* d_gathered, size_t cap, const uint64_t* d_dibit_offset, size_t first_shard,
                                 size_t n_shards, uint8_t* d_out, size_t out_cap, void* stream)
{
    if (!h || !d_gathered || !d_dibit_offset || !d_out || n_shards == 0 || n_shards > 65535 || first_shard > n_shards) return P25FE_ERR_ARG;
    if (first_shard == n_shards) return P25FE_OK;
    HIPCHK(h, hipSetDevice(h->cfg.device));
    const unsigned bx = (unsigned)((cap + 256 * 16 - 1) / (256 * 16));
    hipLaunchKernelGGL(k_shard_compact, dim3(bx ? bx : 1, (unsigned)(n_shards - first_shard)), dim3(256), 0, (hipStream_t)stream, d_gathered,
                       (unsigned long long)cap, d_dibit_offset, (int)first_shard, (int)n_shards, d_out, (unsigned long long)out_cap);
    HIPCHK(h, hipGetLastError());
    return P25FE_OK;
}

struct Staged { size_t stride, n_hist; char* host; const char* dev; };
static int stage_iq(p25fe_t* h, const void* iq, int fmt, size_t n, Staged* s)
{
    if (h->state.format_refused(fmt)) return P25FE_ERR_FORMAT;
    const size_t C = (size_t)h->C, eb = fmt_bytes(fmt);
    s->stride = SHARD_HALO + round_up(n, 8) + 8;
    HIPCHK(h, h->hin.ensure(C * s->stride * eb));
    s->host = static_cast<char*>(h->hin.p);
    s->dev = static_cast<const char*>(h->hin.dp);
    s->n_hist = h->state.n_hist();
    for (size_t c = 0; c < C; ++c) {
// ... 595 lines not shown
```

p25rx_amd/csrc/p25fe_jit.cpp:

```cpp
#include "p25fe_jit.h"

#include <dlfcn.h>
#include <errno.h>
#include <fcntl.h>
#include <hip/hiprtc.h>
#include <math.h>
#include <stdio.h>
#include <stdlib.h>
#include <string.h>
#include <sys/stat.h>
#include <sys/types.h>
#include <unistd.h>

#include "p25fe_embed.inc"

namespace p25jit {

const char* const KERNEL_NAMES[2][3] = {
    {"p25jit_k1_cf32_lin", "p25jit_k1_cf32_pl", "p25jit_chunk_cf32"},
    {"p25jit_k1_u8_lin", "p25jit_k1_u8_pl", "p25jit_chunk_u8"},
};

static const char* const OPTIONS[] = {"--offload-arch=gfx950", "-O3", "-std=c++17", "-ffp-contract=off", "-fno-fast-math",
                                      "-fhip-fp32-correctly-rounded-divide-sqrt", "-Wno-unused-function"};
static const int N_OPTIONS = (int)(sizeof OPTIONS / sizeof OPTIONS[0]);

static const char WRAPPER[] =
    "#include \"p25fe_jit_spec.h\"\n"
    "#include \"p25fe_kernels.hip\"\n"
    "using namespace p25k;\n"
    "#define P25JIT_K1(NAME, FMT, OM, WPS) extern \"C\" __global__ __launch_bounds__(WV, WPS) void NAME(K1Args a, const Taps* __restrict__ t) "
    "{ frontend_body<FMT, true, 5, OM, P25FE_JIT_TX>(a, t); }\n"
    "P25JIT_K1(p25jit_k1_cf32_lin, P25FE_FMT_CF32, OUT_LINEAR, Geo<5>::WAVES_PER_SIMD)\n"
    "P25JIT_K1(p25jit_k1_u8_lin, P25FE_FMT_U8, OUT_LINEAR, Geo<5>::WAVES_PER_SIMD)\n"
    "P25JIT_K1(p25jit_k1_cf32_pl, P25FE_FMT_CF32, OUT_PLANAR, P25FE_K1_PLANAR_WPS)\n"
    "P25JIT_K1(p25jit_k1_u8_pl, P25FE_FMT_U8, OUT_PLANAR, (P25FE_JIT_AVG_N > AVG_DPP_MAX ? 2 : P25FE_K1_PLANAR_WPS_U8))\n"
    "extern \"C\" __global__ __launch_bounds__(WV, 2) void p25jit_chunk_cf32(K1Args a, const Taps* __restrict__ t, ChunkTail c) "
    "{ chunk_body<P25FE_FMT_CF32, true, P25FE_JIT_TX>(a, t, c); }\n"
    "extern \"C\" __global__ __launch_bounds__(WV, 2) void p25jit_chunk_u8(K1Args a, const Taps* __restrict__ t, ChunkTail c) "
    "{ chunk_body<P25FE_FMT_U8, true, P25FE_JIT_TX>(a, t, c); }\n";

namespace rtc {
struct Api {
    void* lib = nullptr;
    decltype(&hiprtcCreateProgram) create = nullptr;
    decltype(&hiprtcCompileProgram) compile = nullptr;
    decltype(&hiprtcGetProgramLogSize) log_size = nullptr;
    decltype(&hiprtcGetProgramLog) log = nullptr;
    decltype(&hiprtcGetCodeSize) code_size = nullptr;
    decltype(&hiprtcGetCode) code = nullptr;
    decltype(&hiprtcDestroyProgram) destroy = nullptr;
    decltype(&hiprtcGetErrorString) error_string = nullptr;
    decltype(&hiprtcVersion) version = nullptr;
    bool ok = false;
};
static const Api& api()
{
    static const Api a = [] {
        Api x;
        const char* env = getenv("P25FE_HIPRTC");
        const char* names[] = {"libhiprtc.so.7", "libhiprtc.so", "/opt/rocm/lib/libhiprtc.so"};
        if (env && *env) x.lib = dlopen(env, RTLD_NOW | RTLD_LOCAL);
        else
            for (const char* n : names)
                if ((x.lib = dlopen(n, RTLD_NOW | RTLD_LOCAL)) != nullptr) break;
        if (!x.lib) return x;
#define P25_SYM(field, name) x.field = reinterpret_cast<decltype(x.field)>(dlsym(x.lib, name))
        P25_SYM(create, "hiprtcCreateProgram"); P25_SYM(compile, "hiprtcCompileProgram");
        P25_SYM(log_size, "hiprtcGetProgramLogSize"); P25_SYM(log, "hiprtcGetProgramLog"); P25_SYM(code_size, "hiprtcGetCodeSize");
        P25_SYM(code, "hiprtcGetCode"); P25_SYM(destroy, "hiprtcDestroyProgram"); P25_SYM(error_string, "hiprtcGetErrorString");
        P25_SYM(version, "hiprtcVersion");
#undef P25_SYM
        x.ok = x.create && x.compile && x.log_size && x.log && x.code_size && x.code && x.destroy && x.error_string;
        return x;
    }();
    return a;
}
}

static uint64_t fnv(uint64_t h, const void* p, size_t n)
{
    const unsigned char* b = static_cast<const unsigned char*>(p);
    for (size_t i = 0; i < n; ++i) { h ^= b[i]; h *= 0x100000001b3ull; }
    return h;
}

uint64_t spec_hash(const Spec& s)
{
    uint64_t h = 0xcbf29ce484222325ull;
    h = fnv(h, "p25fe-jit-2", 11);
    h = fnv(h, P25FE_SRC_KERNELS, sizeof P25FE_SRC_KERNELS);
    h = fnv(h, P25FE_SRC_RECV, sizeof P25FE_SRC_RECV);
    h = fnv(h, P25FE_SRC_P25FE_H, sizeof P25FE_SRC_P25FE_H);
    h = fnv(h, P25FE_SRC_SPEC_H, sizeof P25FE_SRC_SPEC_H);
    h = fnv(h, WRAPPER, sizeof WRAPPER);
    for (int i = 0; i < N_OPTIONS; ++i) h = fnv(h, OPTIONS[i], strlen(OPTIONS[i]) + 1);
    h = fnv(h, &s.tx, sizeof s.tx);
    h = fnv(h, &s.t1, sizeof s.t1);
    h = fnv(h, &s.t2, sizeof s.t2);
    h = fnv(h, s.dec, sizeof(float) * (size_t)s.t1);
    h = fnv(h, s.ch, sizeof(float) * (size_t)s.t2);
    h = fnv(h, &s.fm_gain, sizeof s.fm_gain);
    h = fnv(h, &s.u8_lut, sizeof s.u8_lut);
    if (s.u8_lut) {
    } else {
        h = fnv(h, &s.u8_scale, sizeof s.u8_scale);
        h = fnv(h, &s.u8_offset, sizeof s.u8_offset);
    }
    h = fnv(h, &s.n_avg, sizeof s.n_avg);
    h = fnv(h, &s.avg_uniform, sizeof s.avg_uniform);
    h = fnv(h, s.avg, sizeof(float) * (size_t)s.n_avg);
    return h;
}

std::string file_name(uint64_t hash)
{
    char b[64];
    snprintf(b, sizeof b, "p25fe-%016llx.hsaco", (unsigned long long)hash);
    return b;
}

std::string versioned_file_name(uint64_t hash)
{
    const rtc::Api& R = rtc::api();
    int major = 0, minor = 0;
    if (!R.ok || !R.version || R.version(&major, &minor) != HIPRTC_SUCCESS) return std::string();
    char b[96];
    snprintf(b, sizeof b, "p25fe-%016llx-rtc%d_%d.hsaco", (unsigned long long)hash, major, minor);
    return b;
}

std::string default_cache_dir()
{
    const char* e = getenv("P25FE_CACHE_DIR");
    if (e && *e) return e;
    e = getenv("XDG_CACHE_HOME");
    if (e && *e) return std::string(e) + "/p25fe";
    e = getenv("HOME");
    if (e && *e && access(e, W_OK) == 0) return std::string(e) + "/.cache/p25fe";
    char b[64];
    snprintf(b, sizeof b, "/tmp/p25fe-cache-%u", (unsigned)geteuid());
    return b;
}

static bool owner_ok(const struct stat& st) { return (st.st_uid == geteuid() || st.st_uid == 0) && (st.st_mode & 022) == 0; }
bool dir_trusted(const std::string& dir, std::string* why)
{
    struct stat st;
    if (lstat(dir.c_str(), &st) != 0) { if (why) *why = dir + ": does not exist"; return false; }
    if (!S_ISDIR(st.st_mode)) { if (why) *why = dir + ": not a directory (symbolic links are not followed)"; return false; }
    if (!owner_ok(st)) { if (why) *why = dir + ": owned by another user or writable by group / others -- not used for code objects"; return false; }
    return true;
}

static bool mkdir_p(const std::string& dir)
{
    std::string cur;
    for (size_t i = 0; i <= dir.size(); ++i) {
        if (i == dir.size() || dir[i] == '/') {
            if (!cur.empty() && mkdir(cur.c_str(), 0700) != 0 && errno != EEXIST) return false;
        }
        if (i < dir.size()) cur.push_back(dir[i]);
    }
    return dir_trusted(dir, nullptr);
}

static bool elf_complete(const char* d, size_t n)
{
    if (n < 64 || memcmp(d, "\x7f" "ELF", 4) != 0 || d[4] != 2 ) return false;
    uint64_t shoff = 0;
    uint16_t shentsize = 0, shnum = 0;
    memcpy(&shoff, d + 0x28, 8);
    memcpy(&shentsize, d + 0x3a, 2);
    memcpy(&shnum, d + 0x3c, 2);
    return shoff >= 64 && shnum > 0 && shoff <= n && (uint64_t)shentsize * shnum <= n - shoff;
}

struct Trailer { char magic[8]; uint64_t spec, content, length; };
static const char TRAILER_MAGIC[8] = {'P', '2', '5', 'F', 'E', 'H', 'S', '1'};
static uint64_t content_hash(const char* d, size_t n) { return fnv(fnv(0xcbf29ce484222325ull, "p25fe-obj", 9), d, n); }

static bool read_file(const std::string& path, uint64_t spec, std::vector<char>& out, std::string* why)
{
    struct stat st;
    if (lstat(path.c_str(), &st) != 0) return false;
    if (!S_ISREG(st.st_mode) || !owner_ok(st)) { if (why) *why += path + ": not a private regular file -- ignored\n"; return false; }
    FILE* f = fopen(path.c_str(), "rb");
    if (!f) return false;
    bool ok = false;
    if (fseek(f, 0, SEEK_END) == 0) {
        const long n = ftell(f);
        if (n > 64 + (long)sizeof(Trailer) && n < (64L << 20) && fseek(f, 0, SEEK_SET) == 0) {
            out.resize((size_t)n);
            if (fread(out.data(), 1, (size_t)n, f) == (size_t)n) {
                Trailer t;
                const size_t len = (size_t)n - sizeof t;
                memcpy(&t, out.data() + len, sizeof t);
                ok = memcmp(t.magic, TRAILER_MAGIC, 8) == 0 && t.length == len && t.spec == spec && elf_complete(out.data(), len) &&
                     t.content == content_hash(out.data(), len);
                if (ok) out.resize(len);
            }
        }
    }
    fclose(f);
    if (!ok) { out.clear(); if (why) *why += path + ": truncated, damaged or built for other numbers -- ignored\n"; }
    return ok;
}

static bool write_file_atomic(const std::string& dir, const std::string& name, uint64_t spec, const std::vector<char>& data)
{
    if (!mkdir_p(dir)) return false;
    char tmp[64];
    snprintf(tmp, sizeof tmp, "/.tmp-%ld-%p", (long)getpid(), (const void*)&data);
    const std::string t = dir + tmp, final_ = dir + "/" + name;
    Trailer tr;
    memcpy(tr.magic, TRAILER_MAGIC, 8);
    tr.spec = spec; tr.content = content_hash(data.data(), data.size()); tr.length = data.size();
    const int fd = open(t.c_str(), O_WRONLY | O_CREAT | O_EXCL | O_NOFOLLOW, 0600);
    if (fd < 0) return false;
    FILE* f = fdopen(fd, "wb");
    if (!f) { close(fd); unlink(t.c_str()); return false; }
    const bool ok = fwrite(data.data(), 1, data.size(), f) == data.size() && fwrite(&tr, 1, sizeof tr, f) == sizeof tr;
    if (fclose(f) != 0 || !ok || rename(t.c_str(), final_.c_str()) != 0) { unlink(t.c_str()); return false; }
    return true;
}

static void put_float(std::string& o, float v)
{
    char b[48];
    if (v != v || v - v != 0.0f) snprintf(b, sizeof b, "__builtin_nanf(\"\")");
    else snprintf(b, sizeof b, "%af", (double)v);
    o += b;
}

static std::string gen_header(const Spec& s)
{
    std::string o;
    o.reserve(8192);
    o += "typedef signed char int8_t; typedef unsigned char uint8_t; typedef short int16_t; typedef unsigned short uint16_t;\n"
         "typedef int int32_t; typedef unsigned int uint32_t; typedef long int64_t; typedef unsigned long uint64_t;\n"
         "typedef unsigned long size_t; typedef unsigned long uintptr_t;\n"
         "#define P25FE_JIT 1\n";
    char b[256];
// ... 87 lines not shown
```

p25rx_amd/csrc/p25fe_kernels.hip:

```cpp
#ifndef __HIPCC_RTC__
#include <hip/hip_runtime.h>
#include <stdint.h>
#endif

#include "p25fe.h"
#include "p25fe_spec.h"

namespace p25k {

#ifdef P25FE_MEASURE
#include "p25fe_measure.inc"
#else
#define P25FE_M_LOAD_OFFSET(product_, cached_row_) (product_)
#define P25FE_M_ENTRY do { } while (0)
#define P25FE_M_LOCALS do { } while (0)
#define P25FE_M_ITEM do { } while (0)
#define P25FE_M_SUBTILE do { } while (0)
#define P25FE_M_EXIT do { } while (0)
#define K1_STAMP(i) do { } while (0)
#define K1_PIN2(a, b) do { } while (0)
#define P25FE_M_PIN_V2(arr_, n_) do { } while (0)
#define P25FE_M_PIN_F2(arr_, n_) do { } while (0)
#define P25FE_M_CUT_LOADS do { } while (0)
#define P25FE_M_CUT(stage_) do { } while (0)
#define P25FE_M_CUT_KEEP_F2(stage_, arr_, n_) do { } while (0)
#define P25FE_M_CUT_KEEP_F(stage_, arr_, n_) do { } while (0)
#define P25FE_M_KEEP1(a_) do { } while (0)
#define P25FE_M_KEEP2(a_, b_) do { } while (0)
#define P25FE_M_K6_STORES_ONLY do { } while (0)
#define P25FE_M_NO_BB_STORES false
#define P25FE_M_NO_SIGN_PLANES false
#define P25FE_M_NO_CH_FMA false
#define P25FE_M_NO_OUT_STAGE false
#define P25FE_M_DET_CUT_SCREEN do { } while (0)
#define P25FE_M_DET_NO_PEAK_TEST false
#define P25FE_M_PIPE_NOWAIT() false
#define P25FE_M_API_EXTRAS
#endif


template <int V> struct icst { static constexpr int value = V; };
template <bool B, class A, class C> struct cond { using type = A; };
template <class A, class C> struct cond<false, A, C> { using type = C; };

#ifdef P25FE_JIT
#define K1_CT_DECIM_TAPS P25FE_JIT_DECIM_TAPS
#define K1_CT_CHAN_TAPS P25FE_JIT_CHAN_TAPS
#define K1_CT_FM_GAIN P25FE_JIT_FM_GAIN
#define K1_CT_U8_SCALE P25FE_JIT_U8_SCALE
#define K1_CT_U8_OFFSET P25FE_JIT_U8_OFFSET
#define K1_CT_U8_LUT P25FE_JIT_U8_LUT
#define K1_CT_AVG_N P25FE_JIT_AVG_N
#define K1_CT_AVG_TAPS P25FE_JIT_AVG_TAPS
#define K1_CT_AVG_UNIFORM P25FE_JIT_AVG_UNIFORM
#else
#define K1_CT_DECIM_TAPS P25FE_DEFAULT_DECIM_TAPS
#define K1_CT_CHAN_TAPS P25FE_DEFAULT_CHAN_TAPS
#define K1_CT_FM_GAIN P25FE_FM_GAIN
#define K1_CT_U8_SCALE P25FE_U8_SCALE
#define K1_CT_U8_OFFSET P25FE_U8_OFFSET
#define K1_CT_U8_LUT 0
#define K1_CT_AVG_N P25FE_BOXCAR
#define K1_CT_AVG_TAPS P25FE_DEFAULT_AVG_TAPS
#define K1_CT_AVG_UNIFORM 1
#endif

constexpr int WV = 64;
constexpr int DEC = P25FE_DECIM;
constexpr int T1 = P25FE_T1;
constexpr int T2 = P25FE_T2;
constexpr int BOX = P25FE_BOXCAR;
constexpr int HALO_Y = BOX;
constexpr int HALO_D = HALO_Y + (T2 - 1);
constexpr int TMAX = P25FE_MAX_TAPS;
constexpr int AVG_DPP_MAX = 11;
constexpr int SEG_HALO = 80;
__host__ __device__ constexpr int seg_halo_for(int t3, int t2) { return t3 + t2 - 1 <= 80 ? 80 : 160; }
static_assert(SEG_HALO == seg_halo_for(BOX, TMAX) && seg_halo_for(TMAX, TMAX) >= TMAX + TMAX - 1, "segment halo covers the filter memory and is byte-aligned per plane");
#ifndef P25FE_K1_PRO_CF32
#define P25FE_K1_PRO_CF32 0
#endif
__host__ __device__ constexpr bool seg_prologue(int fmt) { return fmt == P25FE_FMT_U8 || P25FE_K1_PRO_CF32 != 0; }

constexpr int SPS_ = P25FE_SPS;
constexpr int PLPAD = 320;
static_assert(PLPAD % 320 == 0 && PLPAD >= 240 + 2, "planar pad holds the receiver's history");
constexpr int OUT_LINEAR = 0, OUT_PLANAR = 1;
constexpr int PL_BLK = 32 * P25FE_SPS;
__host__ __device__ inline long planar_index(long i, int r) { return (i >> 5) * PL_BLK + r * 32 + (i & 31); }
constexpr int HIST_IQ = DEC * HALO_D + (T1 - 1) + (DEC - 1);
constexpr int HIST_IQ_MAX = DEC * (TMAX + TMAX - 1) + (TMAX - 1) + (DEC - 1);

template <int PK, int TX = 0> struct Geo {
    static constexpr int T1 = TX ? TMAX : P25FE_T1;
    static constexpr int T2 = TX ? TMAX : P25FE_T2;
    static constexpr int D_CARRY = (T2 - 1 + 1) & ~1;
    static constexpr int P = PK;
    static constexpr int SUB = WV * PK;
    static constexpr int XWIN = DEC * SUB + (T1 - DEC);
    static constexpr int XIN_N = (XWIN + 1 + 7) / 8 * 8;
    static constexpr int D_N = D_CARRY + SUB;
    static constexpr int TAPS_N = T1 + T2 + 3 + TMAX + 1;
    static constexpr size_t LDS_BASE = sizeof(float2) * (D_CARRY + XIN_N);
    static_assert(sizeof(float2) * XIN_N >= sizeof(float2) * SUB + sizeof(float) * SUB, "d and the transpose fit the window region");
    static constexpr int WAVES_PER_SIMD = PK <= 3 ? 4 : 2;
};

struct Taps {
    float dec[TMAX];
    float ch[TMAX];
    float lut[256];
    float fm_gain;
    int n_avg;
    int avg_uniform;
    float pad_;
    float avg[TMAX];
};
#ifndef P25FE_K1_AVG_LDS_CF32
#define P25FE_K1_AVG_LDS_CF32 0
#endif
template <class G> __host__ __device__ constexpr size_t k1_lds_bytes(bool ct, bool lut, int t3)
{
    return G::LDS_BASE + sizeof(float) * (size_t)((ct ? 0 : G::TAPS_N) + (lut ? 256 : 0) + (t3 > AVG_DPP_MAX || !ct || P25FE_K1_AVG_LDS_CF32 ? t3 - 1 + G::SUB : 0));
}

__device__ __forceinline__ float spec_atan2f(float y, float x)
{
    const float ax = __builtin_fabsf(x), ay = __builtin_fabsf(y);
    const float mx = ax > ay ? ax : ay;
    const float mn = ax > ay ? ay : ax;
    const float t = mn / mx;
    const float s = t * t;
    float p = P25FE_ATAN_COEFFS[P25FE_ATAN_NCOEF - 1];
#pragma unroll
    for (int i = P25FE_ATAN_NCOEF - 2; i >= 0; --i) p = __builtin_fmaf(p, s, P25FE_ATAN_COEFFS[i]);
    float r = p * t;
    if (ay > ax) r = P25FE_HALF_PI - r;
    if (x < 0.0f) r = P25FE_PI - r;
    if (y < 0.0f) r = -r;
    return mx == 0.0f ? 0.0f : r;
}

__device__ __forceinline__ float fm_discriminate(float2 s, float2 prev, float gain)
{
    const float t = s.y * prev.y;
    const float re = __builtin_fmaf(s.x, prev.x, t);
    const float u = s.x * prev.y;
    const float im = __builtin_fmaf(s.y, prev.x, -u);
    return spec_atan2f(im, re) * gain;
}

typedef float v2f __attribute__((ext_vector_type(2)));
#ifndef P25FE_K1_SCALAR_FMA
#define P25FE_K1_SCALAR_FMA 0
#endif
__device__ __forceinline__ v2f cfma(float tap, v2f s, v2f acc)
{
#if P25FE_K1_SCALAR_FMA
    float re = __builtin_fmaf(tap, s.x, acc.x), im = __builtin_fmaf(tap, s.y, acc.y);
    asm volatile("" : "+v"(re));
    return v2f{re, im};
#else
    const v2f t = {tap, tap};
    return __builtin_elementwise_fma(t, s, acc);
#endif
}

__device__ __forceinline__ v2f lds_read_v2(const float2* p)
{
    typedef const volatile unsigned long long __attribute__((address_space(3))) * lds_u64_ptr;
    const unsigned long long u = *((lds_u64_ptr)p);
    return __builtin_bit_cast(v2f, u);
}
__device__ __forceinline__ float2 lds_read_c(const float2* p)
{
    const v2f v = lds_read_v2(p);
    return make_float2(v.x, v.y);
}

template <int OFF> __device__ __forceinline__ v2f lds_issue_b64(unsigned addr)
{
    v2f v;
    asm volatile("ds_read_b64 %0, %1 offset:%2" : "=v"(v) : "v"(addr), "n"(OFF) : "memory");
    return v;
}
template <int N> __device__ __forceinline__ void lds_landed(v2f& v)
{
    static_assert(N >= 0 && N <= 15, "lgkmcnt is a 4-bit field");
    asm volatile("s_waitcnt lgkmcnt(%1)" : "+v"(v) : "n"(N));
// ... 114 lines not shown
        "v_writelane_b32 %0, %1, 0\n\tv_writelane_b32 %0, %2, 5\n\t"
        "v_writelane_b32 %0, %3, 1\n\tv_writelane_b32 %0, %4, 6\n\t"
        "v_writelane_b32 %0, %5, 2\n\tv_writelane_b32 %0, %6, 7\n\t"
        "v_writelane_b32 %0, %7, 3\n\tv_writelane_b32 %0, %8, 8\n\t"
        "v_writelane_b32 %0, %9, 4\n\tv_writelane_b32 %0, %10, 9"
        : "+v"(v)
        : "s"((unsigned)m[0]), "s"((unsigned)(m[0] >> 32)), "s"((unsigned)m[1]), "s"((unsigned)(m[1] >> 32)),
          "s"((unsigned)m[2]), "s"((unsigned)(m[2] >> 32)), "s"((unsigned)m[3]), "s"((unsigned)(m[3] >> 32)),
          "s"((unsigned)m[4]), "s"((unsigned)(m[4] >> 32)));
    return v;
}
__device__ __forceinline__ unsigned lane_gather(unsigned v, int src)
{
    return (unsigned)__builtin_amdgcn_ds_bpermute(src << 2, (int)v);
}

__device__ __forceinline__ void phase_sync()
{
    __builtin_amdgcn_fence(__ATOMIC_RELEASE, "wavefront");
    __builtin_amdgcn_wave_barrier();
    __builtin_amdgcn_fence(__ATOMIC_ACQUIRE, "wavefront");
}

__device__ __forceinline__ float u8_to_f32(unsigned b) { return __builtin_fmaf((float)b, K1_CT_U8_SCALE, K1_CT_U8_OFFSET); }

#ifndef P25FE_K1_LD_AUX
#define P25FE_K1_LD_AUX 0
#endif
template <int FMT, int PK, int TX = 0, int NVX = 0> struct Loader {
    using G = Geo<PK, TX>;
    static constexpr int LOG_SPV = 1;
    static constexpr int SPV = 1 << LOG_SPV;
    static constexpr int NV = NVX ? NVX : (G::XWIN + SPV + SPV * WV - 1) / (SPV * WV);
    using V = typename cond<FMT == P25FE_FMT_CF32, uint4, unsigned>::type;
    V v[NV];

    typedef unsigned v4u_t __attribute__((ext_vector_type(4)));
    static constexpr int BPS = FMT == P25FE_FMT_CF32 ? 8 : 2;
    static constexpr int VB = BPS * SPV;
    __amdgpu_buffer_rsrc_t rs;
    long base_idx;

    __device__ __forceinline__ void init(const void* base, long first0, long n_hist, long n_new, long i_last)
    {
        const long f_al = (first0 >> LOG_SPV) << LOG_SPV;
        const long lo_al = ((-n_hist) >> LOG_SPV) << LOG_SPV;
        base_idx = f_al > lo_al ? f_al : lo_al;
        const long last = i_last < n_new - 1 ? i_last : n_new - 1;
        long bytes = ((last + 1 - base_idx + SPV - 1) >> LOG_SPV) * VB;
        bytes = bytes < 0 ? 0 : (bytes > (1L << 30) ? (1L << 30) : bytes);
        const uintptr_t p = reinterpret_cast<uintptr_t>(base) + (uintptr_t)(base_idx * BPS);
        const unsigned plo = __builtin_amdgcn_readfirstlane((unsigned)p), phi = __builtin_amdgcn_readfirstlane((unsigned)(p >> 32));
        rs = __builtin_amdgcn_make_buffer_rsrc(reinterpret_cast<void*>(((uintptr_t)phi << 32) | plo), 0,
                                               __builtin_amdgcn_readfirstlane((int)bytes), 0x00020000);
    }
    __device__ __forceinline__ void load_first(long first, int tid)
    {
        const long f_al = (first >> LOG_SPV) << LOG_SPV;
        long rel = (f_al - base_idx) * BPS;
        rel = rel < -(1L << 30) ? -(1L << 30) : (rel > (1L << 30) ? (1L << 30) : rel);
        const int voff = (int)rel + VB * tid;
#pragma unroll
        for (int j = 0; j < NV; ++j) {
            int o = voff + j * VB * WV;
            o = o < 0 ? 0x7ffffff0 : o;
            if constexpr (FMT == P25FE_FMT_CF32) {
                const v4u_t t = __builtin_amdgcn_raw_buffer_load_b128(rs, o, 0, P25FE_K1_LD_AUX);
                v[j] = make_uint4(t.x, t.y, t.z, t.w);
            } else {
                v[j] = __builtin_amdgcn_raw_buffer_load_b32(rs, o, 0, P25FE_K1_LD_AUX);
            }
        }
    }
    __device__ __forceinline__ void load(long first, int tid)
    {
        const long f_al = (first >> LOG_SPV) << LOG_SPV;
        long rel = (f_al - base_idx) * BPS;
        rel = rel < -(1L << 30) ? -(1L << 30) : (rel > (1L << 30) ? (1L << 30) : rel);
        const int voff = (int)rel + VB * tid;
#pragma unroll
        for (int j = 0; j < NV; ++j) {
            const int o = P25FE_M_LOAD_OFFSET(voff + j * VB * WV, VB * tid);
            if constexpr (FMT == P25FE_FMT_CF32) {
                const v4u_t t = __builtin_amdgcn_raw_buffer_load_b128(rs, o, 0, P25FE_K1_LD_AUX);
                v[j] = make_uint4(t.x, t.y, t.z, t.w);
            } else {
                v[j] = __builtin_amdgcn_raw_buffer_load_b32(rs, o, 0, P25FE_K1_LD_AUX);
            }
        }
    }

    template <bool LUTM = false>
    __device__ __forceinline__ void store(float2* XIN, long first, long n_hist, long n_new, int tid, const float* lut = nullptr) const
    {
        float4* XV = reinterpret_cast<float4*>(__builtin_assume_aligned(XIN, 16));
#pragma unroll
        for (int j = 0; j < NV; ++j) {
            float2 s[SPV];
#pragma unroll
            for (int e = 0; e < SPV; ++e) {
                if constexpr (FMT == P25FE_FMT_CF32) {
                    const unsigned w[4] = {v[j].x, v[j].y, v[j].z, v[j].w};
                    s[e] = make_float2(__uint_as_float(w[2 * e]), __uint_as_float(w[2 * e + 1]));
                } else {
                    const unsigned pair = (v[j] >> (16 * e)) & 0xffffu;
                    if constexpr (LUTM) s[e] = make_float2(lut[pair & 0xffu], lut[pair >> 8]);
                    else s[e] = make_float2(u8_to_f32(pair & 0xffu), u8_to_f32(pair >> 8));
                }
            }
            if (j < NV - 1 || SPV * (tid + j * WV) + SPV <= G::XIN_N) XV[tid + j * WV] = make_float4(s[0].x, s[0].y, s[1].x, s[1].y);
        }
    }
    __device__ __forceinline__ void fixup(float2* XIN, long first, long n_hist, long n_new, int tid) const
    {
        const long first_al = (first >> LOG_SPV) << LOG_SPV;
        if (first_al >= -n_hist && first_al + (long)NV * SPV * WV <= n_new) return;
#pragma unroll
        for (int j = 0; j < NV; ++j)
#pragma unroll
            for (int e = 0; e < SPV; ++e) {
                const long i = first_al + SPV * (long)(tid + j * WV) + e;
                const int k = SPV * (tid + j * WV) + e;
                if ((i < -n_hist || i >= n_new) && k < G::XIN_N) XIN[k] = make_float2(0.f, 0.f);
            }
    }
};

struct K1Args {
    const void* x;
    long ch_stride;
    long n_hist;
    long n_new;
    int o0;
    float* bb;
    long bb_stride;
    long n_out;
    int subs_per_seg;
    int seg_count;
    int n_ch;
    int seg_first;
    long m_begin;
    float* power_partial;
    float* bbp;
    long bbp_ch_stride;
    uint8_t* bits;
    long bits_ch_stride;
    int pl_shift;
    unsigned* done_flag;
    unsigned done_seq;
    int lead_segs;
    int seg_halo;
};

#ifndef P25FE_K1_PLANAR_WPS
#define P25FE_K1_PLANAR_WPS 2
#endif
#ifndef P25FE_K1_PLANAR_WPS_U8
#define P25FE_K1_PLANAR_WPS_U8 3
#endif
#ifndef P25FE_K1_TURNAROUND_PRIO
#define P25FE_K1_TURNAROUND_PRIO 3
#endif
#ifndef P25FE_K1_PF_CF32
#define P25FE_K1_PF_CF32 1
#endif
#ifndef P25FE_K1_NT_STORES
#define P25FE_K1_NT_STORES 1
#endif
#ifndef P25FE_K1_PF_U8
#define P25FE_K1_PF_U8 2
#endif
template <int FMT, bool CT, int PK, int OM = OUT_LINEAR, int TX = 0>
__device__ __forceinline__ void frontend_body(const K1Args& a, const Taps* __restrict__ gtaps)
{
    constexpr int PF = (PK != 5 || TX != 0) ? 1 : (FMT == P25FE_FMT_U8 ? P25FE_K1_PF_U8 : P25FE_K1_PF_CF32);
#ifndef P25FE_JIT
    static_assert(TX == 0 || !CT, "the 64-tap geometry is for caller-supplied taps");
#endif
    static_assert(OM == OUT_LINEAR || PK == 5, "the planar epilogue maps a 320-sample sub-tile onto 10 planes x 32 symbols");
    P25FE_M_ENTRY;
    using G = Geo<PK, TX>;
    constexpr int SUB = G::SUB;
    constexpr int P = PK;
    constexpr int T1 = G::T1, T2 = G::T2, D_CARRY = G::D_CARRY;
    constexpr int T3 = CT ? K1_CT_AVG_N : TMAX;
    constexpr bool AVG_DPP = CT && T3 <= AVG_DPP_MAX && !(P25FE_K1_AVG_LDS_CF32 != 0 && FMT == P25FE_FMT_CF32);
    constexpr int HY = T3;
    constexpr int NBACK = AVG_DPP ? ((T3 - 1 + PK - 1) / PK > 0 ? (T3 - 1 + PK - 1) / PK : 1) : 1;
    static_assert(T3 >= 1 && T3 <= TMAX && NBACK <= 3, "post-discriminator filter length");
    extern __shared__ __attribute__((aligned(16))) char smem[];
    float2* D = reinterpret_cast<float2*>(smem);
    float2* XIN = D + D_CARRY;
    float* OUT = reinterpret_cast<float*>(D + G::D_N);
    float* TAPS = reinterpret_cast<float*>(D + D_CARRY + G::XIN_N);
    float* const LUT = TAPS + (CT ? 0 : G::TAPS_N);
    float* const AVT = TAPS + (T1 + T2 + 3);
    constexpr bool LUTM = FMT == P25FE_FMT_U8 && (!CT || K1_CT_U8_LUT != 0);
    const int tid = threadIdx.x;
    if (!CT) {
        for (int k = tid; k < T1; k += WV) TAPS[k] = gtaps->dec[k];
        for (int k = tid; k < T2; k += WV) TAPS[T1 + k] = gtaps->ch[k];
        for (int k = tid; k < TMAX; k += WV) AVT[k] = gtaps->avg[k];
    }
    if constexpr (LUTM)
        for (int k = tid; k < 256; k += WV) LUT[k] = gtaps->lut[k];
    float* const FM = LUT + (FMT == P25FE_FMT_U8 && (!CT || K1_CT_U8_LUT != 0) ? 256 : 0);
    float fm_gain = K1_CT_FM_GAIN;
    int n_avg = T3, avg_uniform = K1_CT_AVG_UNIFORM;
    if constexpr (!CT) {
        fm_gain = __int_as_float(__builtin_amdgcn_readfirstlane(__float_as_int(gtaps->fm_gain)));
        n_avg = __builtin_amdgcn_readfirstlane(gtaps->n_avg);
        avg_uniform = __builtin_amdgcn_readfirstlane(gtaps->avg_uniform);
    }
    const int SEGH = CT ? seg_halo_for(T3, T2) : a.seg_halo;
    auto tap_dec = [&](int k) -> float { return CT ? K1_CT_DECIM_TAPS[k] : TAPS[k]; };
    auto tap_ch = [&](int k) -> float { return CT ? K1_CT_CHAN_TAPS[k] : TAPS[T1 + k]; };

    constexpr bool PRO = seg_prologue(FMT);
    const long seg_len = PRO ? (long)a.subs_per_seg * SUB : (long)(SUB - SEGH) + (long)(a.subs_per_seg - 1) * SUB;
    constexpr int ND = HY + (T2 - 1);
    constexpr int PWIN = DEC * (ND - 1) + T1;
    constexpr int NVP = (PWIN + 2 + 2 * WV - 1) / (2 * WV);
    constexpr int PBASE = 2 * WV * NVP;
    constexpr int NDL = (ND + WV - 1) / WV;
    static_assert(PBASE + ND <= G::XIN_N && D_CARRY <= ND, "prologue scratch fits the window region");
    P25FE_M_LOCALS;
    const long n_items = (long)a.seg_count * a.n_ch;
    const bool grid2d = gridDim.x == (unsigned)a.seg_count;
    for (long item = grid2d ? (long)blockIdx.y * a.seg_count + blockIdx.x : (long)blockIdx.x; item < n_items;
         item += grid2d ? n_items : (long)gridDim.x) {
    P25FE_M_ITEM;
    const int ch = grid2d ? (int)blockIdx.y : (int)((unsigned)item / (unsigned)a.seg_count);
    const long seg_rel = grid2d ? (long)blockIdx.x : item - (long)ch * a.seg_count;
    const long seg = seg_rel + a.seg_first;
    const bool lead = seg < (long)a.lead_segs;
    const long LEAD_LEN = PRO ? (long)SUB : (long)(SUB - SEGH);
    const long this_len = lead ? LEAD_LEN : seg_len;
    const int subs_this = lead ? 1 : a.subs_per_seg;
    const long m_seg0 = a.m_begin + (lead ? seg * LEAD_LEN : (long)a.lead_segs * LEAD_LEN + (seg - a.lead_segs) * seg_len);
    if (m_seg0 >= a.n_out) continue;
    const long m_seg1 = (m_seg0 + this_len < a.n_out) ? m_seg0 + this_len : a.n_out;
    const char* xb = reinterpret_cast<const char*>(a.x) + (size_t)ch * a.ch_stride * (FMT == P25FE_FMT_CF32 ? 8 : 2);
    float* bb = a.bb + (size_t)ch * a.bb_stride;
    phase_sync();

    using LoaderT = Loader<FMT, PK, TX>;
    using LoaderP = Loader<FMT, PK, TX, NVP>;
    LoaderT ld0, ld1;
    long dlo = PRO ? m_seg0 : m_seg0 - SEGH;
    const long i_last = (long)a.o0 + DEC * (m_seg1 - 1);
    float pw = 0.f;
    float2 y_carry = make_float2(0.f, 0.f);
    float f_carry[NBACK][P];
    if constexpr (!PRO) {
        for (int k = tid; k < D_CARRY; k += WV) D[k] = make_float2(0.f, 0.f);
        if constexpr (!AVG_DPP)
            for (int k = tid; k < T3 - 1; k += WV) FM[k] = 0.f;
        ld0.init(xb, (long)a.o0 + DEC * dlo - (T1 - 1), a.n_hist, a.n_new, i_last);
        ld0.load_first((long)a.o0 + DEC * dlo - (T1 - 1), tid);
        if constexpr (PF == 2) {
            ld1.rs = ld0.rs; ld1.base_idx = ld0.base_idx;
            ld1.load((long)a.o0 + DEC * (dlo + SUB) - (T1 - 1), tid);
        }
#pragma unroll
        for (int b = 0; b < NBACK; ++b)
#pragma unroll
            for (int p = 0; p < P; ++p) f_carry[b][p] = 0.f;
    } else {
    LoaderP lp;
    const long pfirst = (long)a.o0 + DEC * (m_seg0 - ND) - (T1 - 1);
    ld0.init(xb, pfirst, a.n_hist, a.n_new, i_last);
    lp.rs = ld0.rs; lp.base_idx = ld0.base_idx;
    lp.load_first(pfirst, tid);
    constexpr bool LATE_LD0 = FMT == P25FE_FMT_CF32;
    if constexpr (!LATE_LD0) {
        ld0.load_first((long)a.o0 + DEC * dlo - (T1 - 1), tid);
        if constexpr (PF == 2) {
            ld1.rs = ld0.rs; ld1.base_idx = ld0.base_idx;
            ld1.load_first((long)a.o0 + DEC * (dlo + SUB) - (T1 - 1), tid);
        }
    }
    {
        float2* const PD_ = XIN + PBASE;
        lp.template store<LUTM>(XIN, pfirst, a.n_hist, a.n_new, tid, LUT);
        lp.fixup(XIN, pfirst, a.n_hist, a.n_new, tid);
        if constexpr (LATE_LD0) {
            ld0.load_first((long)a.o0 + DEC * dlo - (T1 - 1), tid);
            if constexpr (PF == 2) {
                ld1.rs = ld0.rs; ld1.base_idx = ld0.base_idx;
                ld1.load_first((long)a.o0 + DEC * (dlo + SUB) - (T1 - 1), tid);
            }
        }
        phase_sync();
        const int pxsh = (int)(pfirst & 1);
        v2f dacc[NDL];
#pragma unroll
        for (int r = 0; r < NDL; ++r) {
            dacc[r] = v2f{0.f, 0.f};
            const int l = tid + WV * r;
            if (NDL == 1 || l < ND) {
                const float2* w = XIN + pxsh + DEC * l;
                lds_walk<T1, CT>(w, [&](auto jc, v2f sv) {
                    constexpr int j = decltype(jc)::value;
                    dacc[r] = cfma(tap_dec(T1 - 1 - j), sv, dacc[r]);
                });
            }
        }
#pragma unroll
        for (int r = 0; r < NDL; ++r) {
            const int l = tid + WV * r;
            if (l < ND) PD_[l] = make_float2(dacc[r].x, dacc[r].y);
        }
        phase_sync();
        v2f yv = v2f{0.f, 0.f};
        if (tid < HY) {
            const float2* w = PD_ + (ND - HY) - (T2 - 1) + tid;
            lds_walk<T2, CT>(w, [&](auto jc, v2f sv) {
                constexpr int j = decltype(jc)::value;
                yv = cfma(tap_ch(T2 - 1 - j), sv, yv);
            });
        }
        float2 yp;
        yp.x = wave_shr1(yv.x, 0.f);
        yp.y = wave_shr1(yv.y, 0.f);
        const float fmv = fm_discriminate(make_float2(yv.x, yv.y), yp, fm_gain);
        y_carry.x = lane_bcast<HY - 1>(yv.x);
        y_carry.y = lane_bcast<HY - 1>(yv.y);
        static_for<0, NBACK>([&](auto bc) {
            constexpr int b = decltype(bc)::value;
            static_for<0, P>([&](auto pc) {
                constexpr int p = decltype(pc)::value;
                constexpr int l = HY - (b + 1) * P + p;
                if constexpr (AVG_DPP && l >= 1) f_carry[b][p] = lane_bcast<l>(fmv);
                else f_carry[b][p] = 0.f;
            });
        });
        if constexpr (!AVG_DPP)
            if (tid >= 1 && tid < HY) FM[tid - 1] = fmv;
        for (int k = tid; k < D_CARRY; k += WV) D[k] = PD_[ND - D_CARRY + k];
        phase_sync();
    }
    }

    float outv[P];
#pragma unroll
    for (int q = 0; q < P; ++q) outv[q] = 0.f;
    int out_rel = -2 * SUB;
    const int seg_n = (int)(m_seg1 - m_seg0);
    float* const bb_seg = OM == OUT_LINEAR ? bb + m_seg0 : nullptr;
    const int pl_sym = tid & 31, pl_h5 = (tid >> 5) * 5;
    const int i_seg = OM == OUT_PLANAR ? (int)((m_seg0 + a.pl_shift) / SPS_) : 0;
    float* const bbp_ch = OM == OUT_PLANAR ? a.bbp + (size_t)ch * a.bbp_ch_stride : nullptr;
    uint8_t* const bits_ch = OM == OUT_PLANAR ? a.bits + (size_t)ch * a.bits_ch_stride : nullptr;
    unsigned bitsv = 0u;
    auto flush_outputs = [&]() {
        if constexpr (OM == OUT_LINEAR) {
#pragma unroll
            for (int q = 0; q < P; ++q) {
                const int r = out_rel + tid + q * WV;
                if (r >= 0 && r < seg_n) bb_seg[r] = outv[q];
            }
        } else {
            if constexpr (PRO) {
            const int blk = (i_seg >> 5) + out_rel / SUB;
            float* const row = bbp_ch + (size_t)blk * PL_BLK + pl_sym + 32 * pl_h5;
#pragma unroll
            for (int q = 0; q < P; ++q) {
                const int r = out_rel + SPS_ * pl_sym + pl_h5 + q;
#if P25FE_K1_NT_STORES
                if (r >= 0 && r < seg_n) __builtin_nontemporal_store(outv[q], row + 32 * q);
#else
                if (r >= 0 && r < seg_n) row[32 * q] = outv[q];
#endif
            }
            if (tid < SPS_ && out_rel >= 0 && out_rel < seg_n)
                reinterpret_cast<unsigned*>(bits_ch)[(size_t)blk * SPS_ + tid] = bitsv;
            } else {
            const int i_sub = i_seg + out_rel / SPS_;
            const int i = i_sub + pl_sym;
            float* const row = bbp_ch + (size_t)(i >> 5) * PL_BLK + (i & 31) + 32 * pl_h5;
#pragma unroll
            for (int q = 0; q < P; ++q) {
                const int r = out_rel + SPS_ * pl_sym + pl_h5 + q;
                if constexpr (P25FE_M_NO_BB_STORES) { P25FE_M_KEEP2(outv[q], r); }
                else {
#if P25FE_K1_NT_STORES
                if (r >= 0 && r < seg_n) __builtin_nontemporal_store(outv[q], row + 32 * q);
#else
                if (r >= 0 && r < seg_n) row[32 * q] = outv[q];
#endif
                }
            }
            const int r0 = out_rel + 8 * SPS_ * (tid & 3) + (tid >> 2);
            const int ib = i_sub + 8 * (tid & 3);
            if constexpr (!P25FE_M_NO_SIGN_PLANES)
            if (tid < 4 * SPS_ && r0 >= 0 && r0 < seg_n)
                bits_ch[((size_t)(ib >> 5) * SPS_ + (tid >> 2)) * 4 + ((ib >> 3) & 3)] = (uint8_t)bitsv;
            }
        }
    };

    auto sub_tile = [&](auto& ld) -> bool {
        if (dlo >= m_seg1) return false;
        P25FE_M_SUBTILE;
        const long first = (long)a.o0 + DEC * dlo - (T1 - 1);
        const int xsh = (int)(first & 1);
#if P25FE_K1_TURNAROUND_PRIO
        __builtin_amdgcn_s_setprio(P25FE_K1_TURNAROUND_PRIO);
#endif
        ld.template store<LUTM>(XIN, first, a.n_hist, a.n_new, tid, LUT);
        ld.fixup(XIN, first, a.n_hist, a.n_new, tid);
        phase_sync();
        K1_STAMP(0);
        flush_outputs();
        ld.load(first + (long)(PF * DEC) * SUB, tid);
#if P25FE_K1_TURNAROUND_PRIO
        __builtin_amdgcn_s_setprio(0);
#endif
        K1_STAMP(1);

        P25FE_M_CUT_LOADS;
        {
            const float2* w = XIN + xsh + (DEC * P) * tid;
            v2f acc[P];
#pragma unroll
            for (int p = 0; p < P; ++p) acc[p] = v2f{0.f, 0.f};
            lds_walk<DEC * (P - 1) + T1, CT>(w, [&](auto jc, v2f s) {
                constexpr int j = decltype(jc)::value;
#pragma unroll
                for (int p = 0; p < P; ++p) {
                    const int k = DEC * p + (T1 - 1) - j;
                    if (k >= 0 && k < T1) acc[p] = cfma(tap_dec(k), s, acc[p]);
                }
            });
            phase_sync();
            P25FE_M_PIN_V2(acc, P);
            K1_STAMP(2);
#pragma unroll
            for (int p = 0; p < P; ++p) D[D_CARRY + P * tid + p] = make_float2(acc[p].x, acc[p].y);
        }
        phase_sync();

        P25FE_M_CUT(2);
        float2 y[P];
        {
            const float2* w = D + (D_CARRY - (T2 - 1)) + P * tid;
            v2f yv[P];
#pragma unroll
            for (int p = 0; p < P; ++p) yv[p] = v2f{0.f, 0.f};
            lds_walk<(P - 1) + T2, CT>(w, [&](auto jc, v2f s) {
                constexpr int j = decltype(jc)::value;
#pragma unroll
                for (int p = 0; p < P; ++p) {
                    const int k = p + (T2 - 1) - j;
                    if constexpr (P25FE_M_NO_CH_FMA) { if (k == 0) yv[p] = s; }
                    else if (k >= 0 && k < T2) yv[p] = cfma(tap_ch(k), s, yv[p]);
                }
            });
#pragma unroll
            for (int p = 0; p < P; ++p) y[p] = make_float2(yv[p].x, yv[p].y);
            if (a.power_partial) {
#pragma unroll
                for (int p = 0; p < P; ++p) {
                    const long m = dlo + P * tid + p;
                    if (m >= m_seg0 && m < m_seg1 && m >= 0) {
                        const float q0 = y[p].x * y[p].x, q1 = y[p].y * y[p].y;
                        pw = pw + (q0 + q1);
                    }
                }
            }
        }
        P25FE_M_PIN_F2(y, P);
        K1_STAMP(3);
        phase_sync();
        for (int k = tid; k < D_CARRY; k += WV) D[k] = D[SUB + k];

        P25FE_M_CUT_KEEP_F2(3, y, P);
        float f[P];
        {
            float2 yprev;
            yprev.x = wave_shr1(y[P - 1].x, y_carry.x);
            yprev.y = wave_shr1(y[P - 1].y, y_carry.y);
            f[0] = fm_discriminate(y[0], yprev, fm_gain);
#pragma unroll
            for (int p = 1; p < P; ++p) f[p] = fm_discriminate(y[p], y[p - 1], fm_gain);
            y_carry.x = lane_bcast<WV - 1>(y[P - 1].x);
            y_carry.y = lane_bcast<WV - 1>(y[P - 1].y);
        }
        K1_PIN2(f[0], f[1]); K1_PIN2(f[2], f[P - 2]); K1_PIN2(f[P - 1], f[0]);
        K1_STAMP(4);
        P25FE_M_CUT_KEEP_F(4, f, P);
        if constexpr (AVG_DPP) {
        {
            float prevf[NBACK][P];
#pragma unroll
            for (int p = 0; p < P; ++p) prevf[0][p] = wave_shr1(f[p], f_carry[0][p]);
#pragma unroll
            for (int b = 1; b < NBACK; ++b)
#pragma unroll
                for (int p = 0; p < P; ++p) prevf[b][p] = wave_shr1(prevf[b - 1][p], f_carry[b][p]);
            auto fm_back = [&](int p, int j) -> float {
                const int q = p - j;
                if (q >= 0) return f[q];
                const int b = (-q + P - 1) / P;
                return prevf[b - 1][q + b * P];
            };
#pragma unroll
            for (int p = 0; p < P; ++p) {
// ... 4 lines not shown
                    for (int j = 1; j < T3; ++j) acc = acc + fm_back(p, j);
                    acc = acc * K1_CT_AVG_TAPS[0];
                } else {
                    acc = 0.f;
#pragma unroll
                    for (int j = 0; j < T3; ++j) acc = __builtin_fmaf(K1_CT_AVG_TAPS[j], fm_back(p, j), acc);
                }
                if constexpr (P25FE_M_NO_OUT_STAGE) { P25FE_M_KEEP1(acc); }
                else OUT[P * tid + p] = acc;
            }
#pragma unroll
            for (int p = 0; p < P; ++p) {
                if constexpr (NBACK >= 3) f_carry[2][p] = lane_bcast<WV - 3>(f[p]);
                if constexpr (NBACK >= 2) f_carry[1][p] = lane_bcast<WV - 2>(f[p]);
                f_carry[0][p] = lane_bcast<WV - 1>(f[p]);
            }
        }
        } else {
#pragma unroll
            for (int p = 0; p < P; ++p) FM[(T3 - 1) + P * tid + p] = f[p];
            phase_sync();
            const float* w = FM + (T3 - 1) + P * tid;
            float acc[P];
            if constexpr (CT) {
                if constexpr (K1_CT_AVG_UNIFORM) {
#pragma unroll
                    for (int p = 0; p < P; ++p) acc[p] = 0.f;
                    static_for<0, T3 + P - 1>([&](auto ic) {
                        constexpr int i = decltype(ic)::value;
                        const float v = w[(P - 1) - i];
#pragma unroll
                        for (int p = 0; p < P; ++p) {
                            const int j = p + i - (P - 1);
                            if (j == 0) acc[p] = v;
                            else if (j > 0 && j < T3) acc[p] = acc[p] + v;
                        }
                        if constexpr (i % 8 == 7) __builtin_amdgcn_sched_barrier(0);
                    });
#pragma unroll
                    for (int p = 0; p < P; ++p) acc[p] = acc[p] * K1_CT_AVG_TAPS[0];
                } else {
#pragma unroll
                    for (int p = 0; p < P; ++p) acc[p] = 0.f;
                    static_for<0, T3 + P - 1>([&](auto ic) {
                        constexpr int i = decltype(ic)::value;
                        const float v = w[(P - 1) - i];
#pragma unroll
                        for (int p = 0; p < P; ++p) {
                            const int j = p + i - (P - 1);
                            if (j >= 0 && j < T3) acc[p] = __builtin_fmaf(K1_CT_AVG_TAPS[j], v, acc[p]);
                        }
                        if constexpr (i % 8 == 7) __builtin_amdgcn_sched_barrier(0);
                    });
                }
            } else if (avg_uniform) {
#pragma unroll
                for (int p = 0; p < P; ++p) acc[p] = w[p];
                for (int j = 1; j < n_avg; ++j)
#pragma unroll
                    for (int p = 0; p < P; ++p) acc[p] = acc[p] + w[p - j];
                const float sc = AVT[0];
#pragma unroll
                for (int p = 0; p < P; ++p) acc[p] = acc[p] * sc;
            } else {
#pragma unroll
                for (int p = 0; p < P; ++p) acc[p] = 0.f;
                for (int j = 0; j < n_avg; ++j) {
                    const float hj = AVT[j];
#pragma unroll
                    for (int p = 0; p < P; ++p) acc[p] = __builtin_fmaf(hj, w[p - j], acc[p]);
                }
            }
#pragma unroll
            for (int p = 0; p < P; ++p) OUT[P * tid + p] = acc[p];
            phase_sync();
            for (int k = tid; k < T3 - 1; k += WV) FM[k] = FM[SUB + k];
        }
        if constexpr (P25FE_M_NO_OUT_STAGE) return true;
        phase_sync();
        K1_STAMP(5);
        if constexpr (OM == OUT_LINEAR) {
#pragma unroll
            for (int q = 0; q < P; ++q) outv[q] = OUT[tid + q * WV];
        } else {
            unsigned w = 0u;
            unsigned long long sg[5];
#pragma unroll
            for (int q = 0; q < P; ++q) {
                outv[q] = OUT[SPS_ * pl_sym + pl_h5 + q];
                sg[q] = __builtin_amdgcn_ballot_w64(__float_as_int(outv[q]) < 0);
            }
            if constexpr (!P25FE_M_NO_SIGN_PLANES) w = lanes_from_ballots(sg);
            if constexpr (PRO) {
                bitsv = w;
            } else {
                const unsigned pw_ = lane_gather(w, tid >> 2);
                bitsv = (pw_ >> (8 * (tid & 3))) & 0xffu;
            }
        }
        out_rel = (int)(dlo - m_seg0);
        phase_sync();
        K1_PIN2(outv[0], outv[P - 1]);
        K1_STAMP(6);
        return true;
    };
    if constexpr (PF == 1) {
        for (int it = 0; it < subs_this; ++it, dlo += SUB)
            if (!sub_tile(ld0)) break;
    } else {
        for (int it = 0; it < subs_this; it += 2) {
            if (!sub_tile(ld0)) break;
            dlo += SUB;
            if (it + 1 >= subs_this || !sub_tile(ld1)) break;
            dlo += SUB;
        }
    }
    flush_outputs();

    if (a.power_partial) {
#pragma unroll
        for (int d = 32; d > 0; d >>= 1) pw = pw + __shfl_down(pw, d, 64);
        if (tid == 0) a.power_partial[(size_t)ch * a.seg_count + seg_rel] = pw;
    }
    }
    if constexpr (OM == OUT_PLANAR) {
        if (a.done_flag) {
            asm volatile("s_waitcnt vmcnt(0)" ::: "memory");
            __builtin_amdgcn_fence(__ATOMIC_RELEASE, "agent");
            asm volatile("s_waitcnt vmcnt(0)" ::: "memory");
            unsigned ticket = 0u;
            if (tid == 0) ticket = __hip_atomic_fetch_add(a.done_flag + 1, 1u, __ATOMIC_RELAXED, __HIP_MEMORY_SCOPE_AGENT);
            ticket = (unsigned)__builtin_amdgcn_readfirstlane((int)ticket);
            if (ticket == gridDim.x * gridDim.y - 1u) {
                __builtin_amdgcn_fence(__ATOMIC_ACQUIRE, "agent");
                if (tid == 0) {
                    __hip_atomic_store(a.done_flag + 1, 0u, __ATOMIC_RELAXED, __HIP_MEMORY_SCOPE_AGENT);
                    __hip_atomic_store(a.done_flag, a.done_seq, __ATOMIC_RELEASE, __HIP_MEMORY_SCOPE_AGENT);
                }
            }
        }
    }
    P25FE_M_EXIT;
}

constexpr int k1_wps(int fmt, bool ct, int pk, int om)
{
    if (om == OUT_PLANAR) return fmt == P25FE_FMT_U8 ? (ct ? P25FE_K1_PLANAR_WPS_U8 : 2) : P25FE_K1_PLANAR_WPS;
    return (fmt == P25FE_FMT_U8 && !ct && pk <= 3) ? 3 : (pk <= 3 ? 4 : 2);
}
template <int FMT, bool CT, int PK, int OM = OUT_LINEAR, int TX = 0>
__global__ __launch_bounds__(WV, k1_wps(FMT, CT, PK, OM)) void k_frontend(K1Args a, const Taps* __restrict__ gtaps)
{
    frontend_body<FMT, CT, PK, OM, TX>(a, gtaps);
}

constexpr int PD = P25FE_PRE_DECIM;
constexpr int T0 = P25FE_T0;
#ifndef P25FE_K0_P
#define P25FE_K0_P 3
#endif
constexpr int K0_P = P25FE_K0_P;
constexpr int K0_SUB = WV * K0_P;
#ifndef P25FE_K0_SUBS
#define P25FE_K0_SUBS 2
#endif
#ifndef P25FE_K0_WPS
#define P25FE_K0_WPS 2
#endif
constexpr int K0_SUBS = P25FE_K0_SUBS;
constexpr int K0_HALO = T0 - PD;
constexpr int K0_NIN = PD * K0_SUB + K0_HALO;
constexpr int k0_row_pitch(int need) { return need + ((13 - need % 16) + 16) % 16; }
constexpr int K0_JP = k0_row_pitch(K0_NIN / PD + 2);
static_assert(K0_JP >= K0_NIN / PD + 2 && K0_JP % 16 == 13, "polyphase row pitch");
constexpr int K0_NV = (K0_NIN + 2 + 2 * WV - 1) / (2 * WV);
constexpr int HIST_PRE = K0_HALO + PD - 1;

struct K0Args {
    const float* x;
    long ch_stride;
    long n_hist, n_new;
    int o0;
    float* y;
    long y_stride;
    long n_out;
};

#ifndef P25FE_JIT
__global__ __launch_bounds__(WV, P25FE_K0_WPS) void k_predecim(K0Args a)
{
    __shared__ float2 X[PD * K0_JP];
    __shared__ float2 OUT[K0_SUB];
    const int tid = threadIdx.x, ch = blockIdx.y;
    const long m_wg0 = (long)blockIdx.x * (K0_SUB * K0_SUBS);
    const uint4* xb = reinterpret_cast<const uint4*>(a.x + 2 * (size_t)ch * a.ch_stride);
    float2* yb = reinterpret_cast<float2*>(a.y) + (size_t)ch * a.y_stride;

    const long wg_last = (long)a.o0 + PD * (m_wg0 + (long)(K0_SUBS - 1) * K0_SUB) - (T0 - 1);
    uint4 v[K0_NV];
    auto load = [&](long m0) {
        const long base = (long)a.o0 + PD * m0 - (T0 - 1);
        const long v0 = base >> 1;
        long lo = ((-a.n_hist) >> 1) - v0, hi = ((a.n_new - 1) >> 1) - v0;
        const long seg_hi = ((wg_last + K0_NIN) >> 1) - v0;
        hi = hi < seg_hi ? hi : seg_hi;
        lo = lo < -(1L << 30) ? -(1L << 30) : (lo > (1L << 30) ? (1L << 30) : lo);
        hi = hi < -(1L << 30) ? -(1L << 30) : (hi > (1L << 30) ? (1L << 30) : hi);
        const int lo32 = (int)lo, hi32 = (int)hi;
        const uint4* q = xb + v0;
#pragma unroll
        for (int j = 0; j < K0_NV; ++j) {
            int r = tid + j * WV;
            r = r < lo32 ? lo32 : r;
            r = r > hi32 ? hi32 : r;
            v[j] = q[r];
        }
    };
    auto stage = [&](long m0) {
        const long base = (long)a.o0 + PD * m0 - (T0 - 1);
        const long v0 = base >> 1;
        const int sh = (int)(base - (v0 << 1));
        const bool interior = (v0 << 1) >= -a.n_hist && (v0 << 1) + 2L * K0_NV * WV <= a.n_new;
#pragma unroll
        for (int j = 0; j < K0_NV; ++j) {
            const unsigned w[4] = {v[j].x, v[j].y, v[j].z, v[j].w};
#pragma unroll
            for (int e = 0; e < 2; ++e) {
                const int k = 2 * (tid + j * WV) + e - sh;
                float2 s2 = make_float2(__uint_as_float(w[2 * e]), __uint_as_float(w[2 * e + 1]));
                if (!interior) {
                    const long i = ((v0 + tid + (long)j * WV) << 1) + e;
                    if (i < -a.n_hist || i >= a.n_new) s2 = make_float2(0.f, 0.f);
                }
                if (k >= 0 && k < K0_NIN) X[((unsigned)k % PD) * K0_JP + (unsigned)k / PD] = s2;
            }
        }
    };

    float2 outv[K0_P];
#pragma unroll
    for (int q = 0; q < K0_P; ++q) outv[q] = make_float2(0.f, 0.f);
    long out_m0 = -1;
    auto flush = [&]() {
        if (out_m0 >= 0) {
#pragma unroll
            for (int q = 0; q < K0_P; ++q) {
                const long m = out_m0 + tid + q * WV;
                if (m < a.n_out) yb[m] = outv[q];
            }
        }
    };

    load(m_wg0);
#pragma unroll 1
    for (int it = 0; it < K0_SUBS; ++it) {
        const long m0 = m_wg0 + (long)it * K0_SUB;
        if (m0 >= a.n_out) break;
        stage(m0);
        phase_sync();
        flush();
        load(m0 + K0_SUB);
        float2 acc[K0_P];
#pragma unroll
        for (int p = 0; p < K0_P; ++p) acc[p] = make_float2(0.f, 0.f);
        const float2* col = X + K0_P * tid;
#pragma unroll
        for (int u = K0_P - 1 + T0 / PD - 1; u >= 0; --u) {
            float2 ph[PD];
#pragma unroll
            for (int r = 0; r < PD; ++r) ph[r] = lds_read_c(col + r * K0_JP + u);
#pragma unroll
            for (int p = 0; p < K0_P; ++p) {
                const int q = p + (T0 / PD - 1) - u;
                if (q >= 0 && q < T0 / PD) {
#pragma unroll
                    for (int rr = 0; rr < PD; ++rr) {
                        const float h = P25FE_DEFAULT_PRE_TAPS[PD * q + rr];
                        acc[p].x = __builtin_fmaf(h, ph[PD - 1 - rr].x, acc[p].x);
                        acc[p].y = __builtin_fmaf(h, ph[PD - 1 - rr].y, acc[p].y);
                    }
                }
            }
        }
#pragma unroll
        for (int p = 0; p < K0_P; ++p) OUT[K0_P * tid + p] = acc[p];
        phase_sync();
#pragma unroll
        for (int q = 0; q < K0_P; ++q) outv[q] = OUT[tid + q * WV];
        out_m0 = m0;
        phase_sync();
    }
    flush();
}
#endif

constexpr int CZ_M = P25FE_CHZ_CHANNELS;
constexpr int CZ_C1 = 12, CZ_C2 = 16, CZ_P1 = T0 / CZ_C2;
static_assert(T0 == CZ_C2 * CZ_P1 && CZ_M == CZ_C1 * CZ_C2 && CZ_P1 == 5, "factorisation of the 192-point DFT");
#ifndef P25FE_CZ_G
#define P25FE_CZ_G 3
#endif
#ifndef P25FE_CZ_WPS
#define P25FE_CZ_WPS 3
#endif
constexpr int CZ_G = P25FE_CZ_G;
constexpr int CZ_NIN = PD * WV + (T0 - PD);
// ... 214 lines not shown
                                             unsigned long long dibit_stride, unsigned long long sync_stride)
{
    __shared__ unsigned long long LO[256], HI[256];
    __shared__ unsigned long long raw_sh;
    __shared__ unsigned best_sh[4];
    const int tid = threadIdx.x, k = blockIdx.x;
    if (results) {
        const p25fe_result_t r = results[blockIdx.y];
        if ((unsigned long long)k >= r.n_sync) return;
        n_dibits = r.n_dibits;
        dibits += blockIdx.y * dibit_stride;
        sync_dibit += blockIdx.y * sync_stride;
        if (sync_pos) sync_pos += blockIdx.y * sync_stride;
        out += blockIdx.y * sync_stride;
    }
    {
        unsigned long long a = 0, b = 0;
#pragma unroll
        for (int i = 0; i < 8; ++i)
            if (tid & (1 << i)) { a ^= P25FE_NID_ROWS[i]; b ^= P25FE_NID_ROWS[8 + i]; }
        LO[tid] = a; HI[tid] = b;
    }
    const unsigned long long D = sync_dibit[k];
    const bool have = D + 33 <= n_dibits;
    if (tid == 0) {
        unsigned long long raw = 0;
        if (have)
            for (int j = 0; j < 33; ++j)
                if (j != 11) raw = (raw << 2) | (unsigned long long)(dibits[D + j] & 3u);
        raw_sh = raw;
    }
    __syncthreads();
    const unsigned long long cw = raw_sh >> 1;
    unsigned best = 0xffffffffu;
    for (unsigned d = (unsigned)tid; d < 65536u; d += 256u) {
        const unsigned dist = (unsigned)__popcll((HI[d >> 8] ^ LO[d & 255u]) ^ cw);
        const unsigned key = (dist << 16) | d;
        best = key < best ? key : best;
    }
#pragma unroll
    for (int o = 32; o > 0; o >>= 1) {
        const unsigned v = __shfl_down(best, o, 64);
        best = v < best ? v : best;
    }
    if ((tid & 63) == 0) best_sh[tid >> 6] = best;
    __syncthreads();
    if (tid == 0) {
        unsigned b = best_sh[0];
        for (int w = 1; w < 4; ++w) b = best_sh[w] < b ? best_sh[w] : b;
        p25fe_nid_t r;
        r.raw = have ? raw_sh : 0ull;
        r.sync_pos = sync_pos ? sync_pos[k] : 0;
        const unsigned data = b & 0xffffu, dist = b >> 16;
        r.nac = have ? (uint16_t)(data >> 4) : 0;
        r.duid = have ? (uint8_t)(data & 15u) : 0;
        r.n_errors = have ? (uint8_t)dist : 0;
        r.valid = have ? (dist <= P25FE_NID_T ? 1 : 0) : -1;
        out[k] = r;
    }
}
#endif

#ifndef P25FE_JIT
__global__ __launch_bounds__(256) void k_chan_stats(const p25fe_result_t* results, const p25fe_nid_t* nid,
                                                    unsigned long long sync_stride, const float* power_dbm,
                                                    p25fe_chan_stats_t* stats)
{
    __shared__ unsigned long long sh[3][4];
    const int tid = threadIdx.x, ch = blockIdx.x;
    const p25fe_result_t r = results[ch];
    unsigned long long words = 0, errs = 0, fixed = 0;
    if (nid) {
        const unsigned long long n = r.n_sync < sync_stride ? r.n_sync : sync_stride;
        for (unsigned long long k = tid; k < n; k += 256) {
            const p25fe_nid_t v = nid[ch * sync_stride + k];
            if (v.valid >= 0) { ++words; if (v.valid == 0) ++errs; else fixed += v.n_errors; }
        }
    }
    unsigned long long acc[3] = {words, errs, fixed};
#pragma unroll
    for (int q = 0; q < 3; ++q) {
#pragma unroll
        for (int o = 32; o > 0; o >>= 1) acc[q] += __shfl_down(acc[q], o, 64);
        if ((tid & 63) == 0) sh[q][tid >> 6] = acc[q];
    }
    __syncthreads();
    if (tid == 0) {
        p25fe_chan_stats_t o;
        o.sig_power_dbm = power_dbm ? power_dbm[ch] : __int_as_float(0x7fc00000);
        o.locked = r.anchor_out.valid != 0 ? 1 : 0;
        o.n_dibits = r.n_dibits;
        o.n_sync = r.n_sync;
        o.last_sync_pos = (r.n_sync > 0 && r.anchor_out.valid) ? r.anchor_out.s : -1;
        o.bch.words = sh[0][0] + sh[0][1] + sh[0][2] + sh[0][3];
        o.bch.errs = sh[1][0] + sh[1][1] + sh[1][2] + sh[1][3];
        o.bch.fixed = sh[2][0] + sh[2][1] + sh[2][2] + sh[2][3];
        o.bch.size = 63; o.bch.reserved = 0;
        stats[ch] = o;
    }
}
#endif

struct ChunkTail {
    ChunkRecvArgs r;
    unsigned* counter;
    int wg_per_ch;
};

template <int FMT, bool CT, int TX>
__device__ __forceinline__ void chunk_body(const K1Args& a, const Taps* __restrict__ gtaps, const ChunkTail& t)
{
    frontend_body<FMT, CT, 5, OUT_PLANAR, TX>(a, gtaps);
    asm volatile("s_waitcnt vmcnt(0)" ::: "memory");
    __builtin_amdgcn_fence(__ATOMIC_RELEASE, "agent");
    asm volatile("s_waitcnt vmcnt(0)" ::: "memory");
    unsigned ticket = 0u;
    if (threadIdx.x == 0) ticket = __hip_atomic_fetch_add(&t.counter[blockIdx.y], 1u, __ATOMIC_RELAXED, __HIP_MEMORY_SCOPE_AGENT);
    ticket = (unsigned)__builtin_amdgcn_readfirstlane((int)ticket);
    if (ticket != (unsigned)t.wg_per_ch - 1u) return;
    __builtin_amdgcn_fence(__ATOMIC_ACQUIRE, "agent");
    if (threadIdx.x == 0) t.counter[blockIdx.y] = 0u;
    recv_one_tile(t.r, (int)blockIdx.y);
}

template <int FMT, bool CT, int TX>
__global__ __launch_bounds__(WV, 2) void k_chunk(K1Args a, const Taps* __restrict__ gtaps, ChunkTail t)
{
    chunk_body<FMT, CT, TX>(a, gtaps, t);
}


#ifndef P25FE_JIT
__global__ __launch_bounds__(256) void k_shard_compact(const uint8_t* gathered, unsigned long long cap, const uint64_t* offset,
                                                        int first_shard, int n_shards, uint8_t* out, unsigned long long out_cap)
{
    const int r = first_shard + (int)blockIdx.y;
    if (r >= n_shards) return;
    const unsigned long long o0 = offset[r], n = offset[r + 1] - o0;
    const uint8_t* src = gathered + (unsigned long long)r * cap;
    for (unsigned long long i = (unsigned long long)blockIdx.x * 256 + threadIdx.x; i < n && i < cap; i += (unsigned long long)gridDim.x * 256)
        if (o0 + i < out_cap) out[o0 + i] = src[i];
}
#endif

#ifndef P25FE_JIT
__global__ void k_queue_probe_wait(unsigned* word, unsigned long long ticks)
{
    const unsigned long long t0 = wall_clock64();
    unsigned seen = 0u;
    while (!(seen = __hip_atomic_load(word, __ATOMIC_RELAXED, __HIP_MEMORY_SCOPE_AGENT)) && wall_clock64() - t0 < ticks) __builtin_amdgcn_s_sleep(8);
    word[1] = seen ? 1u : 2u;
}
__global__ void k_queue_probe_set(unsigned* word) { __hip_atomic_store(word, 1u, __ATOMIC_RELAXED, __HIP_MEMORY_SCOPE_AGENT); }
#endif

#ifndef P25FE_JIT
__global__ void k_anchors_from_results(const p25fe_result_t* results, p25fe_anchor_t* anchors, int n_ch)
{
    const int c = blockIdx.x * blockDim.x + threadIdx.x;
    if (c < n_ch) anchors[c] = results[c].anchor_out;
}
#endif

#ifndef P25FE_JIT
__global__ void k_shard_resolve(const p25fe_result_t* summaries, const uint64_t* shard_bb0, const uint64_t* shard_bb_n,
                                int n_shards, int symbol_clock, p25fe_anchor_t* anchor_in, uint64_t* dibit_offset)
{
    if (blockIdx.x == 0 && threadIdx.x == 0)
        shard_resolve_impl(summaries, shard_bb0, shard_bb_n, n_shards, symbol_clock, anchor_in, dibit_offset);
}
#endif

}
```

p25rx_amd/csrc/p25fe_measure.inc:

```
#ifndef P25FE_MEASURE_INC
#define P25FE_MEASURE_INC

#ifndef P25FE_ABLATE
#define P25FE_ABLATE 99
#endif
#ifndef P25FE_EXP
#define P25FE_EXP 0
#endif

#if P25FE_ABLATE == 6 || defined(P25FE_ABLATE_CACHED)
#define P25FE_M_LOAD_OFFSET(product_, cached_row_) (cached_row_)
#else
#define P25FE_M_LOAD_OFFSET(product_, cached_row_) (product_)
#endif

#define P25FE_M_NO_BB_STORES ((P25FE_EXP & 8) != 0)
#define P25FE_M_NO_SIGN_PLANES ((P25FE_EXP & 1) != 0)
#define P25FE_M_NO_CH_FMA ((P25FE_EXP & 4) != 0)
#define P25FE_M_NO_OUT_STAGE (P25FE_ABLATE == 5)
#define P25FE_M_KEEP1(a_) asm volatile("" ::"v"(a_))
#define P25FE_M_KEEP2(a_, b_) asm volatile("" ::"v"(a_), "v"(b_))

#ifdef P25FE_K1_STAMP
constexpr int K1_STAMP_SLOTS = 8192;
__device__ unsigned long long g_k1_stamp[K1_STAMP_SLOTS][16];
#define K1_STAMP(i)                                                                   \
    do {                                                                              \
        unsigned long long t_;                                                        \
        asm volatile("s_memtime %0\n\ts_waitcnt lgkmcnt(0)" : "=s"(t_)::"memory");   \
        st_acc[i] += t_ - st_last;                                                    \
        st_last = t_;                                                                 \
    } while (0)
#define K1_PIN2(a, b) asm volatile("" : "+v"(a), "+v"(b))
#define P25FE_M_PIN_V2(arr_, n_) _Pragma("unroll") for (int p_ = 0; p_ < (n_); ++p_) K1_PIN2((arr_)[p_].x, (arr_)[p_].y)
#define P25FE_M_PIN_F2(arr_, n_) _Pragma("unroll") for (int p_ = 0; p_ < (n_); ++p_) K1_PIN2((arr_)[p_].x, (arr_)[p_].y)
#define P25FE_M_ENTRY                                                                                                   \
    unsigned long long st_t0, st_r0;                                   \
    asm volatile("s_memtime %0\n\ts_memrealtime %1\n\ts_waitcnt lgkmcnt(0)" : "=s"(st_t0), "=s"(st_r0)::"memory")
#define P25FE_M_LOCALS unsigned long long st_acc[8] = {0, 0, 0, 0, 0, 0, 0, 0}, st_last = 0, st_n = 0, st_pro = 0, st_items = 0
#define P25FE_M_ITEM                                                                  \
    unsigned long long st_i0;                                                         \
    asm volatile("s_memtime %0\n\ts_waitcnt lgkmcnt(0)" : "=s"(st_i0)::"memory");    \
    bool st_first_sub = true;                                                         \
    ++st_items
#define P25FE_M_SUBTILE                                                               \
    do {                                                                              \
        asm volatile("s_memtime %0\n\ts_waitcnt lgkmcnt(0)" : "=s"(st_last)::"memory"); \
        if (st_first_sub) { st_pro += st_last - st_i0; st_first_sub = false; }        \
        ++st_n;                                                                       \
    } while (0)
#define P25FE_M_EXIT                                                                                                    \
    if (tid == 0) {                                                                                                     \
        unsigned long long st_t1, st_r1;                                                                                \
        asm volatile("s_memtime %0\n\ts_memrealtime %1\n\ts_waitcnt lgkmcnt(0)" : "=s"(st_t1), "=s"(st_r1)::"memory");  \
        unsigned long long* slot = g_k1_stamp[blockIdx.x % K1_STAMP_SLOTS];                                             \
        for (int i = 0; i < 7; ++i) atomicAdd(&slot[i], st_acc[i]);                                                     \
        atomicAdd(&slot[7], st_n);                                                                                      \
        atomicAdd(&slot[8], st_pro);                                    \
        atomicAdd(&slot[9], st_t1 - st_t0);                                                  \
        atomicAdd(&slot[10], st_r1 - st_r0);                                                \
        atomicAdd(&slot[11], 1ull);                                                                      \
        atomicAdd(&slot[12], st_items);                                                                  \
    }
#else
#define K1_STAMP(i) do { } while (0)
#define K1_PIN2(a, b) do { } while (0)
#define P25FE_M_PIN_V2(arr_, n_) do { } while (0)
#define P25FE_M_PIN_F2(arr_, n_) do { } while (0)
#define P25FE_M_ENTRY do { } while (0)
#define P25FE_M_LOCALS do { } while (0)
#define P25FE_M_ITEM do { } while (0)
#define P25FE_M_SUBTILE do { } while (0)
#define P25FE_M_EXIT do { } while (0)
#endif

#if P25FE_ABLATE <= 1
#if defined(P25FE_ABLATE_STORES)
#define P25FE_M_CUT_STORES_ out_rel = (int)(dlo - m_seg0);
#else
#define P25FE_M_CUT_STORES_
#endif
#if defined(P25FE_DRIFT)
#define P25FE_M_CUT_DRIFT_                                                                                   \
    {                                                                                                        \
        unsigned hsh = (unsigned)blockIdx.x * 2654435761u + (unsigned)(dlo & 0xffff) * 40503u;               \
        hsh ^= hsh >> 13;                                                                                    \
        const int units = P25FE_DRIFT + (int)(hsh % (unsigned)(P25FE_DRIFT_SPREAD + 1));                     \
        for (int u = 0; u < units; ++u) __builtin_amdgcn_s_sleep(1);                                         \
    }
#else
#define P25FE_M_CUT_DRIFT_
#endif
#define P25FE_M_CUT_LOADS do { P25FE_M_CUT_STORES_ P25FE_M_CUT_DRIFT_ return true; } while (0)
#else
#define P25FE_M_CUT_LOADS do { } while (0)
#endif
#define P25FE_M_CUT(stage_) do { if constexpr (P25FE_ABLATE <= (stage_)) return true; } while (0)
#define P25FE_M_CUT_KEEP_F2(stage_, arr_, n_)                                                                \
    do { if constexpr (P25FE_ABLATE <= (stage_)) {                                                           \
        _Pragma("unroll") for (int p_ = 0; p_ < (n_); ++p_) asm volatile("" ::"v"((arr_)[p_].x), "v"((arr_)[p_].y)); \
        return true; } } while (0)
#define P25FE_M_CUT_KEEP_F(stage_, arr_, n_)                                                                 \
    do { if constexpr (P25FE_ABLATE <= (stage_)) {                                                           \
        _Pragma("unroll") for (int p_ = 0; p_ < (n_); ++p_) asm volatile("" ::"v"((arr_)[p_]));              \
        return true; } } while (0)

#if defined(P25FE_ABLATE6)
#if P25FE_ABLATE6 == 2
#define P25FE_M_K6_STORES_ONLY                                                                               \
    {                                                                                                        \
        const float2 xv = lds_read_c(X + lane);                                                              \
        float4* const y4 = reinterpret_cast<float4*>(yb - (lane & 1));                                       \
        _Pragma("unroll 1") for (int c = 0; c < CZ_M; c += 2) {                                              \
            typedef float __attribute__((ext_vector_type(4))) f32x4;                                         \
            f32x4 ov; ov.x = xv.x + (float)c; ov.y = xv.y; ov.z = xv.x; ov.w = xv.y;                          \
            __builtin_nontemporal_store(ov, reinterpret_cast<f32x4*>(reinterpret_cast<float2*>(y4) + (size_t)(c + (lane & 1)) * a.y_stride)); \
        }                                                                                                    \
        return;                                                                                              \
    }
#else
#define P25FE_M_K6_STORES_ONLY                                                                               \
    {                                                                                                        \
        const float2 xv = lds_read_c(X + lane);                                                              \
        _Pragma("unroll 1") for (int c = 0; c < CZ_M; ++c) yb[(size_t)c * a.y_stride] = make_float2(xv.x + (float)c, xv.y); \
        return;                                                                                              \
    }
#endif
#else
#define P25FE_M_K6_STORES_ONLY do { } while (0)
#endif

#ifndef P25FE_ABLATE_DET
#define P25FE_ABLATE_DET 0
#endif
#define P25FE_M_DET_CUT_SCREEN                                                                               \
    do { if constexpr (P25FE_ABLATE_DET == 1) {                                                              \
        if (lane == 0) a.tsum[(size_t)ch * a.n_tiles + tile] = (hw[0] | hw[1] | hw[2] | hw[3]) == 0x12345u ? 1ull : 0ull; \
        return; } } while (0)
#define P25FE_M_DET_NO_PEAK_TEST (P25FE_ABLATE_DET == 2)

#ifdef P25FE_MEASURE_UNSAFE
#define P25FE_M_PIPE_NOWAIT() ([] { static const bool nowait = [] { const char* e = getenv("P25FE_PIPE_NOWAIT"); return e && atoi(e) != 0; }(); return nowait; }())
#else
#define P25FE_M_PIPE_NOWAIT() false
#endif
#ifdef P25FE_K1_STAMP
#define P25FE_M_API_EXTRAS                                                                                               \
    int p25fe_debug_k1_stamps(uint64_t out[16])                                                                          \
    {                                                                                                                    \
        std::vector<unsigned long long> z((size_t)p25k::K1_STAMP_SLOTS * 16, 0ull), v(z.size());                         \
        if (hipMemcpyFromSymbol(v.data(), HIP_SYMBOL(p25k::g_k1_stamp), v.size() * 8) != hipSuccess) return P25FE_ERR_HIP; \
        if (hipMemcpyToSymbol(HIP_SYMBOL(p25k::g_k1_stamp), z.data(), z.size() * 8) != hipSuccess) return P25FE_ERR_HIP;   \
        for (int i = 0; i < 16; ++i) out[i] = 0;                                                                         \
        for (size_t k = 0; k < v.size(); ++k) out[k & 15] += v[k];                                                       \
        return P25FE_OK;                                                                                                 \
    }
#else
#define P25FE_M_API_EXTRAS
#endif

#endif
```

p25rx_amd/csrc/p25fe_recv.hip:

```cpp
#ifndef __HIPCC_RTC__
#include <hip/hip_runtime.h>
#include <stdint.h>
#endif

namespace p25k {

constexpr int W = P25FE_PEAK_W;
constexpr int SPS = P25FE_SPS;
constexpr int NSYN = P25FE_SYNC_DIBITS;
constexpr int SYNC_SPAN = P25FE_SYNC_SPAN;
constexpr int HIST_BB = SYNC_SPAN + 2 * W;
static_assert(SPS == SPS_ && PLPAD >= HIST_BB + P25FE_CLK_LOOKAHEAD, "planar layout matches the receiver");

constexpr int TSYM = 768;
constexpr int TS = TSYM * SPS;
constexpr int TWORDS = TSYM / 32;
constexpr int EVCAP = TS / (W + 1) + 8;
constexpr unsigned SYNC_NEG_MASK = ~P25FE_SYNC_SIGN_MASK & 0xffffffu;
constexpr int SCREEN_MAX_MISMATCH = 4;

struct Planar {
    const float* f;
    long f_ch;
    const uint32_t* bits;
// ... 55 lines not shown
                                             bool* usable = nullptr)
{
    D = SPS; N = 1;
    if (usable) *usable = false;
    if (track && prev_valid) {
        const long dd = s_new - s_prev, nn = (dd + SPS / 2) / SPS;
        const long err = dd > SPS * nn ? dd - SPS * nn : SPS * nn - dd;
        if (nn >= 1 && dd <= (1L << P25FE_CLK_DMAX_LOG2) && (err << P25FE_CLK_TOL_SHIFT) <= SPS * nn) {
            if (usable) *usable = true;
            const long d4 = 4 * dd + (f_new - f_prev);
            if (d4 != 4 * SPS * nn) { D = (int)d4; N = (int)(4 * nn); }
        }
    }
}
__host__ __device__ inline bool clock_plausible(int D, int N)
{
    if (N == 1 && D == SPS) return true;
    if (N < 4 || (N & 3) != 0 || D <= 0) return false;
    const long nn = N / 4, d4 = D, nom = 4L * SPS * nn;
    if (d4 > 4 * (1L << P25FE_CLK_DMAX_LOG2) + 4) return false;
    const long err = d4 > nom ? d4 - nom : nom - d4;
    return err <= 4 * ((SPS * nn) >> P25FE_CLK_TOL_SHIFT) + 4;
}
__host__ __device__ inline long clock_J(long x, int D, int N)
{
    if (x <= 0) return 0;
    if (N == 1 && D == SPS) return (x - 1) / SPS;
    return (x * (long)N - 1) / (long)D;
}
__host__ __device__ inline long clock_count(long s, int D, int N, long lo, long hi)
{
    if (lo < s + W + 1) lo = s + W + 1;
    if (hi <= lo) return 0;
    return clock_J(hi - s, D, N) - clock_J(lo - s, D, N);
}

struct RecvOpt {
    int track;
    int n_resync;
    const long* resync;
    long resync_stride;
};
__device__ __forceinline__ long first_kill(const RecvOpt& o, int ch, long x)
{
    if (o.n_resync == 0) return 0x7fffffffffffffffL;
    const long* r = o.resync + (size_t)ch * o.resync_stride;
    const long key = x + (o.track ? CLK_L : 0);
    int lo = 0, hi = o.n_resync;
    while (lo < hi) {
        const int mid = (lo + hi) >> 1;
        if (r[mid] < key) lo = mid + 1; else hi = mid;
    }
    return lo < o.n_resync ? r[lo] - (o.track ? CLK_L : 0) : 0x7fffffffffffffffL;
}

struct alignas(8) TileSumG {
    unsigned pre_end1;
    unsigned first1;
    unsigned end0;
    unsigned last1;
    unsigned n_det_flags;
    unsigned post_rest;
    int out_D, out_N;
};
constexpr unsigned G_FIRST_TRACKS = 1u;
constexpr unsigned G_OUT_VALID = 2u;
constexpr unsigned G_OUT_PERIOD_KNOWN = 4u;

__device__ __forceinline__ unsigned char slice_dibit(float v, float hi, float mid, float lo)
{
    return v >= hi ? 1 : v >= mid ? 0 : v >= lo ? 2 : 3;
}

__device__ __forceinline__ void sync_gather(const float* __restrict__ f, long p, float (&v)[NSYN])
{
    const long i = p / SPS;
    const int r = (int)(p - i * SPS);
    const long first = i - (NSYN - 1);
    const float* base = f + planar_index(first, r);
    const int n0 = 32 - (int)(first & 31);
#pragma unroll
    for (int j = 0; j < NSYN; ++j) v[j] = base[j + (j >= n0 ? PL_BLK - 32 : 0)];
}

__device__ __forceinline__ void sync_corr(const float (&w)[NSYN], float& c, float& e)
{
    float cc = 0.f, ee = 0.f;
#pragma unroll
    for (int j = 0; j < NSYN; ++j) {
        const float x = w[j];
        cc = ((P25FE_SYNC_SIGN_MASK >> j) & 1u) ? cc + x : cc - x;
        ee = __builtin_fmaf(x, x, ee);
    }
    c = cc; e = ee;
}

__device__ __forceinline__ void sync_thresholds(const float (&w)[NSYN], float& hi, float& mid, float& lo)
{
    float Pp = 0.f, Nn = 0.f;
#pragma unroll
    for (int j = 0; j < NSYN; ++j) {
        const float v = w[j];
        if ((P25FE_SYNC_SIGN_MASK >> j) & 1u) Pp = Pp + v; else Nn = Nn + v;
    }
    Pp = Pp * P25FE_SYNC_INV_NPOS;
    Nn = Nn * P25FE_SYNC_INV_NNEG;
    mid = (Pp + Nn) * 0.5f;
    const float span = (Pp - Nn) * 0.5f;
    const float d = span * P25FE_SLICE_FRAC;
    hi = mid + d;
    lo = mid - d;
}

__device__ __forceinline__ int wave_sum_i(int v)
{
#pragma unroll
    for (int d = 32; d >= 1; d >>= 1) v += __shfl_xor(v, d, 64);
    return v;
}
__device__ __forceinline__ int wave_incl_sum(int v, int lane)
{
#pragma unroll
    for (int d = 1; d < 64; d <<= 1) {
        const int o = __shfl_up(v, d, 64);
        if (lane >= d) v += o;
    }
    return v;
}
__device__ __forceinline__ unsigned long long wave_incl_sum64(unsigned long long v, int lane)
{
#pragma unroll
    for (int d = 1; d < 64; d <<= 1) {
        const unsigned long long o = __shfl_up(v, d, 64);
        if (lane >= d) v += o;
    }
    return v;
}
__device__ __forceinline__ int lane_rank(unsigned long long mask)
{
    return (int)__builtin_amdgcn_mbcnt_hi((unsigned)(mask >> 32), __builtin_amdgcn_mbcnt_lo((unsigned)mask, 0u));
}

template <class T> __device__ __forceinline__ void publish(T* dst, const T& v)
{
    static_assert(sizeof(T) % 8 == 0 && alignof(T) >= 8, "whole 8-byte words");
    unsigned long long w[sizeof(T) / 8];
    __builtin_memcpy(w, &v, sizeof(T));
    unsigned long long* d = reinterpret_cast<unsigned long long*>(dst);
#pragma unroll
    for (unsigned k = 0; k < sizeof(T) / 8; ++k) __hip_atomic_store(d + k, w[k], __ATOMIC_RELAXED, __HIP_MEMORY_SCOPE_AGENT);
}

constexpr int GT = 64;
#ifndef P25FE_HEAD_WAIT_TICKS
#define P25FE_HEAD_WAIT_TICKS 200000000ull
#endif
constexpr unsigned long long HEAD_WAIT_TICKS = P25FE_HEAD_WAIT_TICKS;
struct GroupAgg {
    long first_event;
    long last_s;
    unsigned long long after_first;
    int src;
    unsigned n_events;
};
struct GroupPre {
    long s;
    unsigned long long dibit_off;
    unsigned long long carry_cnt;
    int src;
    int valid;
    unsigned event_off;
    unsigned pad_;
};
struct ScanArgs {
    const unsigned long long* tsum;
    const TileRec* recs;
    int n_tiles;
    long n;
    long abs0;
    ScanOut* outs;
    GroupAgg* gagg;
    GroupPre* gpre;
    unsigned* tickets;
    const p25fe_anchor_t* anchor_in;
    p25fe_result_t* result;
    unsigned long long n_baseband;
};
__host__ __device__ inline int n_groups_of(int n_tiles) { return (n_tiles + GT - 1) / GT; }

struct DetArgs {
    Planar pl;
    long n;
    long abs0;
    int n_tiles;
    TileRec* recs;
    unsigned long long* tsum;
    uint16_t* evl;
    float* evthr;
    RecvOpt opt;
    TileSumG* gsum;
    uint32_t* evg;
    const unsigned* head_flag;
    unsigned head_seq;
    int head_tile_max;
    unsigned* head_err;
};

constexpr int EVTHR_N = 4;
constexpr int K2_DCAP = 64;
constexpr int K2_LANES = 60;
constexpr int K2_HCAP = 2048;

template <bool GEN> __device__ __forceinline__ void detect_tile(const DetArgs& a, const int tile, const int ch)
{
    struct Phase1 {
        uint16_t hits[K2_HCAP];
        uint16_t cands[WV];
        float cn[5][12];
        float cthr[WV][3];
    };
    struct Phase2 {
        uint16_t evs[EVCAP];
        uint16_t endo[GEN ? EVCAP : 1];
    };
    union Arena { Phase1 p1; Phase2 p2; };
    __shared__ Arena AR;
    auto& HITS = AR.p1.hits;
    auto& CANDS = AR.p1.cands;
    auto& CN = AR.p1.cn;
    auto& CTHR = AR.p1.cthr;
    auto& EVS = AR.p2.evs;
    __shared__ unsigned EVB[TS / 32];
    __shared__ uint16_t DETE[K2_DCAP];
    __shared__ float DETT[K2_DCAP][3];
    __shared__ unsigned DETN;
    static_assert(TS % (W + 1) == 0, "fraction table: whole blocks");
    __shared__ uint8_t FRO[GEN ? TS / (W + 1) : 4];
    auto fro_set = [&](int off, int v) { FRO[off / (W + 1)] = (uint8_t)(v & 7); };
    auto fro_get = [&](int off) -> unsigned { return (unsigned)FRO[off / (W + 1)] & 7u; };
    const int lane = threadIdx.x;
    const float* f = a.pl.f + (size_t)ch * a.pl.f_ch;
    const long t0 = (long)tile * TS;
    const int tn = a.n - t0 < TS ? (int)(a.n - t0) : TS;
    const long pbase = t0 + PLPAD - W;

    for (int k = lane; k < TS / 32; k += WV) EVB[k] = 0u;
    if (lane == 0) DETN = 0u;

    unsigned hw[4] = {0u, 0u, 0u, 0u};
    const int r = lane / 6, blk = lane % 6;
    const int dlt = r >= SPS / 2 ? 1 : 0;
    if (lane < K2_LANES) {
        const uint32_t* bw = a.pl.bits + (size_t)ch * a.pl.bits_ch + ((size_t)tile * TWORDS + 4 * blk) * SPS + r;
        unsigned wd[6];
#pragma unroll
        for (int k = 0; k < 5; ++k) wd[k] = bw[SPS * k];
        wd[5] = 0u;
        if (dlt) {
#pragma unroll
            for (int k = 4; k >= 1; --k) wd[k] = __builtin_amdgcn_alignbit(wd[k], wd[k - 1], 31);
            wd[0] <<= 1;
        }
#pragma unroll
        for (int j = 0; j < 4; ++j) {
            unsigned acc = 0u;
#pragma unroll
            for (int u = 31; u >= 0; --u) {
                const unsigned win = u <= 22 ? __builtin_amdgcn_alignbit(wd[j + 1], wd[j], 9 + u)
                                             : __builtin_amdgcn_alignbit(wd[j + 2], wd[j + 1], u - 23);
                const unsigned x = (win ^ SYNC_NEG_MASK) & 0xffffffu;
                const int t = __builtin_popcount(x) - (SCREEN_MAX_MISMATCH + 1);
                acc = __builtin_amdgcn_alignbit(acc, (unsigned)t, 31);
            }
            hw[j] = acc;
        }
    }

    P25FE_M_DET_CUT_SCREEN;
    int nh = 0;
    auto flush_hits = [&]() {
        for (int b = 0; b < nh; b += WV) {
            const int h = b + lane;
            const bool act = h < nh;
            const int eo = act ? (int)HITS[h] : 0;
            bool cand = false;
            float th_hi = 0.f, th_mid = 0.f, th_lo = 0.f;
            if (act) {
                float c, e, v[NSYN];
                sync_gather(f, pbase + eo, v);
                sync_corr(v, c, e);
                cand = (c > 0.0f) && (e >= P25FE_SYNC_E_MIN) && (c * c >= P25FE_SYNC_RHO2_N * e);
                if (cand) sync_thresholds(v, th_hi, th_mid, th_lo);
            }
            unsigned long long cm = __ballot(cand);
            if constexpr (P25FE_M_DET_NO_PEAK_TEST) { cm = 0ull; if (cand) EVB[eo >> 5] = 1u; }
            const int nc = __popcll(cm);
            if (cand) {
                const int slot = lane_rank(cm);
                CANDS[slot] = (uint16_t)eo;
                CTHR[slot][0] = th_hi; CTHR[slot][1] = th_mid; CTHR[slot][2] = th_lo;
            }
            phase_sync();
            for (int cb = 0; cb < nc; cb += 5) {
                const int q = lane / 11, d = lane - 11 * q;
                const bool act2 = lane < 55 && cb + q < nc;
                const int ec = act2 ? (int)CANDS[cb + q] : 0;
                if (act2) {
                    float c, e, v[NSYN];
                    sync_gather(f, pbase + ec + d - W, v);
                    sync_corr(v, c, e);
// ... 1514 lines not shown
```

p25rx_amd/frontend.py:

```python
import ctypes as C

import numpy as np

from . import _lib
from ._lib import FMT_CF32, FMT_U8, RESULT_DTYPE, ANCHOR_DTYPE
CHZ_CHANNELS = 192


def _p(a):
    return a.ctypes.data_as(C.c_void_p)


class FrontEnd:
    def __init__(self, n_channels=1, device=0, decim_taps=None, chan_taps=None, symbol_clock=0, **spec):
        self.L = _lib.load()
        cfg = _lib.make_config(n_channels=n_channels, device=device, decim_taps=decim_taps, chan_taps=chan_taps,
                               symbol_clock=symbol_clock, **spec)
        self.symbol_clock = symbol_clock & 0xff
        self.cfg = cfg
        self.C = n_channels
        self.device = device
        self.h = C.c_void_p()
        rc = self.L.p25fe_create(C.byref(cfg), C.byref(self.h))
        if rc == _lib.ERR_JIT:
# ... 21 lines not shown
        pw = np.zeros(self.C, dtype=np.float32)
        self._chk(fn(self.h, _p(arr), n_units, _p(bb), cap, C.byref(n_out), _p(pw) if want_power else None))
        out = bb[:, :n_out.value]
        out = out[0].copy() if self.C == 1 else out.copy()
        if want_power:
            return out, (float(pw[0]) if self.C == 1 else pw)
        return out

    def demod_u8(self, data, want_power=False):
        data = np.ascontiguousarray(data, dtype=np.uint8).reshape(self.C, -1)
        return self._demod(self.L.p25fe_demod_u8, data, data.shape[1], data.shape[1] // 2, want_power)

    def demod_cf32(self, iq, want_power=False):
        iq = np.ascontiguousarray(iq, dtype=np.complex64).reshape(self.C, -1)
        return self._demod(self.L.p25fe_demod_cf32, iq, iq.shape[1], iq.shape[1], want_power)

    def slice(self, bb, sync_cap=None):
        bb = np.ascontiguousarray(bb, dtype=np.float32).reshape(self.C, -1)
        n = bb.shape[1]
        cap = n // 6 + 2
        scap = sync_cap if sync_cap is not None else n // 6 + 2
        dib = np.empty((self.C, cap), dtype=np.uint8)
        spos = np.empty((self.C, scap), dtype=np.int64)
        sdib = np.empty((self.C, scap), dtype=np.uint64)
        nd = (C.c_size_t * self.C)()
        ns = (C.c_size_t * self.C)()
        self._chk(self.L.p25fe_slice(self.h, _p(bb), n, _p(dib), cap, nd, _p(spos), _p(sdib), scap, ns))
        outs = [(dib[c, :nd[c]].copy(), spos[c, :min(ns[c], scap)].copy(), sdib[c, :min(ns[c], scap)].copy())
                for c in range(self.C)]
        return outs[0] if self.C == 1 else outs

    def _run(self, fn, arr, n_units, n_samples):
        cap = n_samples // 30 + 4
        dib = np.empty((self.C, cap), dtype=np.uint8)
        nd = (C.c_size_t * self.C)()
        self._chk(fn(self.h, _p(arr), n_units, _p(dib), cap, nd))
        outs = [dib[c, :nd[c]].copy() for c in range(self.C)]
        return outs[0] if self.C == 1 else outs

    def run_u8(self, data):
        data = np.ascontiguousarray(data, dtype=np.uint8).reshape(self.C, -1)
        return self._run(self.L.p25fe_run_u8, data, data.shape[1], data.shape[1] // 2)

    def run_cf32(self, iq):
        iq = np.ascontiguousarray(iq, dtype=np.complex64).reshape(self.C, -1)
        return self._run(self.L.p25fe_run_cf32, iq, iq.shape[1], iq.shape[1])

    def run_host_windows(self, iq, window=0, fmt=None):
        if hasattr(iq, "data_ptr"):
            import torch
            assert not iq.is_cuda and iq.is_contiguous()
            is_u8 = iq.dtype == torch.uint8
            n_el = iq.numel() // self.C
            n = n_el // 2
            ptr = C.c_void_p(iq.data_ptr())
        else:
            is_u8 = iq.dtype == np.uint8
            iq = np.ascontiguousarray(iq if is_u8 else iq.view(np.float32) if iq.dtype == np.complex64 else iq.astype(np.float32))
            n = iq.size // self.C // 2
            ptr = _p(iq)
        fmt = (FMT_U8 if is_u8 else FMT_CF32) if fmt is None else fmt
        cap = n // 30 + 4
        dib = np.empty((self.C, cap), dtype=np.uint8)
        nd = (C.c_size_t * self.C)()
        st = _lib.WindowsStats()
        self._chk(self.L.p25fe_run_host_windows(self.h, ptr, fmt, n, int(window), _p(dib), cap, nd, C.byref(st)))
        outs = [dib[c, :nd[c]].copy() for c in range(self.C)]
        stats = dict(n_windows=int(st.n_windows), ms_total=st.ms_total, ms_h2d=st.ms_h2d, ms_compute=st.ms_compute,
                     pinned_input=bool(st.pinned_input))
        return (outs[0] if self.C == 1 else outs), stats

    def resync(self):
        self._chk(self.L.p25fe_resync(self.h))

    def reset(self):
        self._chk(self.L.p25fe_reset(self.h))

    def resync_at_dev(self, idx):
        if idx is None or idx.numel() == 0:
            self._rs = None
            self._chk(self.L.p25fe_resync_at_dev(self.h, None, 0, 0))
            return
        import torch
        assert idx.is_cuda and idx.dtype == torch.int64 and idx.is_contiguous()
        if idx.dim() == 1:
            idx = idx.unsqueeze(0).expand(self.C, -1).contiguous() if self.C > 1 else idx.unsqueeze(0)
        assert idx.shape[0] == self.C
        self._rs = idx
        self._chk(self.L.p25fe_resync_at_dev(self.h, C.c_void_p(idx.data_ptr()), idx.shape[1], idx.stride(0)))

    def state_export(self):
        n = C.c_size_t(0)
        self._chk(self.L.p25fe_state_size(self.h, C.byref(n)))
        buf = np.empty(n.value, dtype=np.uint8)
        self._chk(self.L.p25fe_state_export(self.h, _p(buf), buf.size, C.byref(n)))
        return buf

    def state_import(self, blob):
        blob = np.ascontiguousarray(blob, dtype=np.uint8)
        self._chk(self.L.p25fe_state_import(self.h, _p(blob), blob.size))

    @staticmethod
    def _stream():
        import torch
        return C.c_void_p(torch.cuda.current_stream().cuda_stream)

    @staticmethod
    def _fmt_of(t):
        import torch
        if t.dtype == torch.float32:
            return FMT_CF32, t.shape[-2] if t.dim() == 3 else t.shape[0]
        if t.dtype == torch.uint8:
            return FMT_U8, t.shape[-2] if t.dim() == 3 else t.shape[0]
        raise TypeError("IQ tensor must be float32 [C, n, 2] or uint8 [C, n, 2]")

    def _iq_view(self, iq):
        import torch
        assert iq.is_cuda and iq.shape[-1] == 2
        if iq.dim() == 2:
            iq = iq.unsqueeze(0)
        assert iq.shape[0] == self.C and iq.stride(2) == 1 and iq.stride(1) == 2
        fmt = FMT_CF32 if iq.dtype == torch.float32 else FMT_U8
        if iq.dtype not in (torch.float32, torch.uint8):
            raise TypeError("IQ tensor must be float32 or uint8")
        return fmt, iq.shape[1], (iq.stride(0) // 2 if self.C > 1 else iq.shape[1])

    @staticmethod
    def dibit_cap(n_iq):
        return (n_iq // 50 + n_iq // 250000 + 64 + 15) // 16 * 16

    def run_dev(self, iq, dibits=None, result=None):
        import torch
        fmt, n, stride = self._iq_view(iq)
        cap = self.dibit_cap(n)
        if dibits is None:
            dibits = torch.empty((self.C, cap), dtype=torch.uint8, device=iq.device)
        if result is None:
            result = torch.empty((self.C, RESULT_DTYPE.itemsize), dtype=torch.uint8, device=iq.device)
        self._chk(self.L.p25fe_run_dev(self.h, C.c_void_p(iq.data_ptr()), fmt, stride, n, C.c_void_p(dibits.data_ptr()),
                                       dibits.stride(0), C.c_void_p(result.data_ptr()), self._stream()))
        return dibits, result

    def run_dev_pipelined(self, iq, dibits=None, result=None):
        import torch
        fmt, n, stride = self._iq_view(iq)
        cap = self.dibit_cap(n)
        if dibits is None:
            dibits = torch.empty((self.C, cap), dtype=torch.uint8, device=iq.device)
        if result is None:
            result = torch.empty((self.C, RESULT_DTYPE.itemsize), dtype=torch.uint8, device=iq.device)
        self._chk(self.L.p25fe_run_dev_pipelined(self.h, C.c_void_p(iq.data_ptr()), fmt, stride, n,
                                                 C.c_void_p(dibits.data_ptr()), dibits.stride(0),
                                                 C.c_void_p(result.data_ptr()), self._stream()))
        self._inflight = (getattr(self, "_inflight", ()) + ((dibits, result),))[-2:]
        return dibits, result

    def join_dev(self):
        self._chk(self.L.p25fe_join_dev(self.h, self._stream()))
        self._inflight = ()

    def demod_dev(self, iq, n_hist=0, abs0=0, bb=None, want_power=False, offset=0):
        import torch
        fmt, n_total, stride = self._iq_view(iq)
        n = n_total - offset
        nb = self.L.p25fe_n_baseband_h(self.h, abs0, n)
        if bb is None:
            bb = torch.empty((self.C, (nb + 7) // 4 * 4), dtype=torch.float32, device=iq.device)
        pw = torch.empty(self.C, dtype=torch.float32, device=iq.device) if want_power else None
        ptr = iq.data_ptr() + offset * (8 if fmt == FMT_CF32 else 2)
        self._chk(self.L.p25fe_demod_dev(self.h, C.c_void_p(ptr), fmt, stride, n_hist, n, abs0,
                                         C.c_void_p(bb.data_ptr()), bb.stride(0),
                                         C.c_void_p(pw.data_ptr()) if want_power else None, self._stream()))
        return (bb, nb, pw) if want_power else (bb, nb)

    def predecim_dev(self, iq, n_hist=0, abs0=0, offset=0, out=None):
        import torch
        fmt, n_total, stride = self._iq_view(iq)
        assert fmt == FMT_CF32
        n = n_total - offset
        no = self.L.p25fe_n_predecim(abs0, n)
        if out is None:
            out = torch.empty((self.C, (no + 3) // 2 * 2, 2), dtype=torch.float32, device=iq.device)
        self._chk(self.L.p25fe_predecim_dev(self.h, C.c_void_p(iq.data_ptr() + 8 * offset), stride, n_hist, n, abs0,
                                            C.c_void_p(out.data_ptr()), out.stride(0) // 2, self._stream()))
        return out, no

    def channelise_dev(self, iq, n_hist=0, abs0=0, offset=0, out=None):
        import torch
        assert iq.dtype == torch.float32 and iq.dim() == 2 and iq.shape[1] == 2
        n = iq.shape[0] - offset
        no = self.L.p25fe_n_predecim(abs0, n)
        if out is None:
            out = torch.empty((CHZ_CHANNELS, max(64, (no + 63) // 64 * 64), 2), dtype=torch.float32, device=iq.device)
        self._chk(self.L.p25fe_channelise_dev(self.h, C.c_void_p(iq.data_ptr() + 8 * offset), n_hist, n, abs0,
                                              C.c_void_p(out.data_ptr()), out.stride(0) // 2, self._stream()))
        return out, no

    def slice_dev(self, bb, n_bb, n_hist_bb=0, abs_bb0=0, anchor_in=None, offset=0, sync_cap=0):
        import torch
        dev = bb.device
        if bb.dim() == 1:
            bb = bb.unsqueeze(0)
        cap = (n_bb // 10 + 64 + 15) // 16 * 16
        dib = torch.empty((self.C, cap), dtype=torch.uint8, device=dev)
        res = torch.empty((self.C, RESULT_DTYPE.itemsize), dtype=torch.uint8, device=dev)
        spos = torch.empty((self.C, max(sync_cap, 1)), dtype=torch.int64, device=dev)
        sdib = torch.empty((self.C, max(sync_cap, 1)), dtype=torch.int64, device=dev)
        a_in = None
        if anchor_in is not None:
            a_in = torch.from_numpy(np.frombuffer(np.asarray(anchor_in, dtype=ANCHOR_DTYPE).tobytes(), dtype=np.uint8).copy()).to(dev)
        self._chk(self.L.p25fe_slice_dev(self.h, C.c_void_p(bb.data_ptr() + 4 * offset), bb.stride(0), n_hist_bb, n_bb,
                                         abs_bb0, C.c_void_p(a_in.data_ptr()) if a_in is not None else None,
                                         C.c_void_p(dib.data_ptr()), dib.stride(0),
                                         C.c_void_p(spos.data_ptr()) if sync_cap else None,
                                         C.c_void_p(sdib.data_ptr()) if sync_cap else None, sync_cap,
                                         C.c_void_p(res.data_ptr()), self._stream()))
        return dib, res, spos, sdib

    def nid_dev(self, dibits, n_dibits, sync_dibit, sync_pos=None, n_sync=None):
        import torch
        n_sync = int(sync_dibit.numel() if n_sync is None else n_sync)
        out = torch.empty((max(n_sync, 1), 24), dtype=torch.uint8, device=dibits.device)
        self._chk(self.L.p25fe_nid_dev(self.h, C.c_void_p(dibits.data_ptr()), int(n_dibits), C.c_void_p(sync_dibit.data_ptr()),
                                       C.c_void_p(sync_pos.data_ptr()) if sync_pos is not None else None, n_sync,
                                       C.c_void_p(out.data_ptr()), self._stream()))
        return out[:n_sync]

    def nid_batch_dev(self, dibits, results, sync_dibit, sync_pos=None):
        import torch
        sync_stride = sync_dibit.shape[1]
        out = torch.zeros((self.C, max(sync_stride, 1), 24), dtype=torch.uint8, device=dibits.device)
        self._chk(self.L.p25fe_nid_batch_dev(self.h, C.c_void_p(dibits.data_ptr()), dibits.stride(0),
                                             C.c_void_p(results.data_ptr()), C.c_void_p(sync_dibit.data_ptr()),
                                             C.c_void_p(sync_pos.data_ptr()) if sync_pos is not None else None,
                                             sync_stride, C.c_void_p(out.data_ptr()), self._stream()))
        return out[:, :sync_stride]

    def chan_stats_dev(self, results, nid=None, power_dbm=None):
        import torch
        out = torch.empty((self.C, 64), dtype=torch.uint8, device=results.device)
        self._chk(self.L.p25fe_chan_stats_dev(self.h, C.c_void_p(results.data_ptr()),
                                              C.c_void_p(nid.data_ptr()) if nid is not None else None,
                                              nid.shape[1] if nid is not None else 0,
                                              C.c_void_p(power_dbm.data_ptr()) if power_dbm is not None else None,
                                              C.c_void_p(out.data_ptr()), self._stream()))
        return out

    def profile_enable(self, on=True):
        self._chk(self.L.p25fe_profile_enable(self.h, int(on)))

    def profile_read(self):
        ms = (C.c_double * 4)()
        n = C.c_uint64(0)
        self._chk(self.L.p25fe_profile_read(self.h, C.byref(ms), C.byref(n)))
        return [ms[i] for i in range(4)], n.value

    def n_baseband(self, abs0, n):
        return int(self.L.p25fe_n_baseband_h(self.h, abs0, n))

    def shard_halo(self):
        return self.L.p25fe_shard_halo()

    def shard_pass1(self, iq, offset, n_hist, abs0, result=None):
        import torch
        fmt, n_total, stride = self._iq_view(iq)
        n = n_total - offset
        if result is None:
            result = torch.empty((self.C, RESULT_DTYPE.itemsize), dtype=torch.uint8, device=iq.device)
        ptr = iq.data_ptr() + offset * (8 if fmt == FMT_CF32 else 2)
        self._chk(self.L.p25fe_shard_pass1(self.h, C.c_void_p(ptr), fmt, stride, n_hist, n, abs0,
                                           C.c_void_p(result.data_ptr()), self._stream()))
        return result

    def shard_pass1_main(self, iq, offset, n_hist, abs0):
        fmt, n_total, stride = self._iq_view(iq)
        ptr = iq.data_ptr() + offset * (8 if fmt == FMT_CF32 else 2)
        self._chk(self.L.p25fe_shard_pass1_main(self.h, C.c_void_p(ptr), fmt, stride, n_hist, n_total - offset, abs0,
                                                self._stream()))

    def shard_pass1_finish(self, iq, offset, n_hist, abs0, result=None):
        import torch
        fmt, n_total, stride = self._iq_view(iq)
        if result is None:
            result = torch.empty((self.C, RESULT_DTYPE.itemsize), dtype=torch.uint8, device=iq.device)
        ptr = iq.data_ptr() + offset * (8 if fmt == FMT_CF32 else 2)
        self._chk(self.L.p25fe_shard_pass1_finish(self.h, C.c_void_p(ptr), fmt, stride, n_hist, n_total - offset, abs0,
                                                  C.c_void_p(result.data_ptr()), self._stream()))
        return result

    def shard_pass1_head(self, iq, offset, n_hist, abs0):
        fmt, n_total, stride = self._iq_view(iq)
        ptr = iq.data_ptr() + offset * (8 if fmt == FMT_CF32 else 2)
        self._chk(self.L.p25fe_shard_pass1_head(self.h, C.c_void_p(ptr), fmt, stride, n_hist, n_total - offset, abs0,
                                                self._stream()))

    def shard_head_check(self):
        self._chk(self.L.p25fe_shard_head_check(self.h))

    def shard_pipe_begin(self):
        import torch
        rx = C.c_void_p()
        self._chk(self.L.p25fe_shard_pipe_begin(self.h, self._stream(), C.byref(rx)))
        return torch.cuda.ExternalStream(rx.value)

    def shard_pipe_end(self, last=None):
        self._chk(self.L.p25fe_shard_pipe_end(self.h, C.c_void_p(last.cuda_stream) if last is not None else None))

# ... 85 lines not shown
```

Baseline: 550,700.

## Gate pipelined K1 on a device-side epoch word instead of stream event wait

In pipelined runs the front-end kernel no longer waits on the previous lane's receiver event through hipStreamWaitEvent. It launches a gated variant that computes freely and spins on a device epoch word, which a tiny kernel on the rx stream sets, only before writing the planar scratch. A timeout path reports errors through pinned memory. This lets K1's load and filter work overlap the prior receiver stage. The cost is spinning waves, an extra kernel launch per call, and deadlock or timeout risk if the two streams cannot run at the same time.

```diff
diff --git a/p25rx_amd/csrc/p25fe_api.hip b/p25rx_amd/csrc/p25fe_api.hip
--- a/p25rx_amd/csrc/p25fe_api.hip
+++ b/p25rx_amd/csrc/p25fe_api.hip
@@ -95,6 +95,7 @@
 static_assert(BBPAD == (size_t)TAILN && BBPAD >= (size_t)HIST_BB + CLK_L, "baseband tail kept between calls");
 
 constexpr int MAX_LANES = 4;
+constexpr int GATE_WORDS = MAX_LANES + 2, GATE_DELAY_WORD = MAX_LANES;
 constexpr int SH_FLAG_WORDS = 8, SH_FLAG_ERR = 4;
 constexpr int PROF_RING = 64, PROF_SAMPLE = 8;
 
@@ -111,6 +112,7 @@
     RxScratch s;
     hipEvent_t ev_k1 = nullptr, ev_rx = nullptr;
     bool pending = false;
+    unsigned epoch = 0u;
     hipStream_t joined = nullptr; bool joined_any = false;
 };
 
@@ -287,6 +289,10 @@
     RxScratch& rx() { return lanes[cur].s; }
     const RxScratch& rx() const { return lanes[cur].s; }
     DevBuf power_partial, chunk_cnt, evrec, evnext, evoff;
+    DevBuf gate_words;
+    PinBuf gate_err;
+    unsigned pipe_seq = 0u;
+    unsigned long long rx_delay_ticks = 0;
     unsigned long long ev_seq = 0;
     PinBuf hin, hbb, hout;
     unsigned chunk_seq = 0;
@@ -483,7 +489,7 @@
     case P25FE_ERR_FORMAT: return "sample format changed within a stream";
     case P25FE_ERR_NOMEM: return "out of memory";
     case P25FE_ERR_JIT: return "kernel specialisation failed (p25fe_specialize_log)";
-    case P25FE_ERR_TIMEOUT: return "a device-side wait gave up (time shard: the head segment never arrived)";
+    case P25FE_ERR_TIMEOUT: return "a device-side wait gave up (time shard: the head segment never arrived; pipelined call: the scratch set was never released)";
     default: return "unknown status";
     }
 }
@@ -602,6 +608,8 @@
         if (cfg->symbol_clock != P25FE_CLOCK_FIXED) h->run_depth = 3;
         const char* rd = getenv("P25FE_PIPE_DEPTH");
         if (rd && atoi(rd) >= 2 && atoi(rd) <= MAX_LANES) h->run_depth = atoi(rd);
+        const char* dl = getenv("P25FE_TEST_RX_DELAY_US");
+        if (dl && atol(dl) > 0) h->rx_delay_ticks = 100ull * (unsigned long long)(atol(dl) < 5000 ? atol(dl) : 5000);
     }
     if (e == hipSuccess) e = h->d_taps.ensure(sizeof(Taps));
     if (e == hipSuccess) e = hipMemcpy(h->d_taps.p, &h->taps, sizeof(Taps), hipMemcpyHostToDevice);
@@ -677,6 +685,7 @@
     const ChunkRecvArgs* chunk = nullptr;
     long* head_end = nullptr;
     unsigned* done_flag = nullptr; unsigned done_seq = 0u;
+    K1Gate gate = {nullptr, 0u, nullptr};
     hipStream_t stream = nullptr;
 };
 
@@ -695,6 +704,7 @@
     if ((reinterpret_cast<uintptr_t>(L.src) & 15u) != 0) return P25FE_ERR_ARG;
     if (h->C > 1 && (L.ch_stride % (fmt == P25FE_FMT_CF32 ? 2 : 8)) != 0) return P25FE_ERR_ARG;
     if (L.chunk && (!L.planar || L.part)) return P25FE_ERR_ARG;
+    if (L.gate.epoch && (!L.planar || L.chunk || !L.gate.err)) return P25FE_ERR_ARG;
     const bool pro = seg_prologue(fmt);
     const long m_begin = !L.planar ? 0 : (pro ? -(long)PLPAD - h->look : -(long)HIST_BB - h->look);
     const size_t n_out = p25fe_n_baseband_h(h, L.abs0, L.n);
@@ -766,6 +776,12 @@
     if (pk == 3) return ct ? k_frontend<FMT, true, 3, OUT_LINEAR, 0> : k_frontend<FMT, false, 3, OUT_LINEAR, 0>;
     return ct ? k_frontend<FMT, true, 5, OUT_LINEAR, 0> : k_frontend<FMT, false, 5, OUT_LINEAR, 0>;
 }
+using K1GatedKernel = void (*)(K1Args, const Taps*, K1Gate);
+template <int FMT> static K1GatedKernel k1_gated_kernel_of(bool ct, bool long_taps)
+{
+    if (long_taps) return k_frontend_gated<FMT, false, 1>;
+    return ct ? k_frontend_gated<FMT, true, 0> : k_frontend_gated<FMT, false, 0>;
+}
 template <int FMT> static ChunkKernel chunk_kernel_of(bool ct, bool long_taps)
 {
     if (long_taps) return k_chunk<FMT, false, 1>;
@@ -799,7 +815,8 @@
     const dim3 grid((unsigned)a.seg_count, (unsigned)h->C);
     if (h->variant == P25FE_VARIANT_SPECIALIZED) {
         hipFunction_t f = h->jit_fn[p.u8 ? 1 : 0][L.chunk ? 2 : (L.planar ? 1 : 0)];
-        void* params[3] = {&a, &dt, &tail};
+        K1Gate gate = L.gate;
+        void* params[3] = {&a, &dt, L.chunk ? (void*)&tail : (void*)&gate};
         if (L.ev0 || L.ev1)
             HIPCHK(h, hipExtModuleLaunchKernel(f, grid.x * WV, grid.y, 1, WV, 1, 1, p.lds, st, params, nullptr, L.ev0, L.ev1, 0));
         else
@@ -807,6 +824,9 @@
     } else if (L.chunk) {
         const ChunkKernel k = p.u8 ? chunk_kernel_of<P25FE_FMT_U8>(p.ct, h->long_taps) : chunk_kernel_of<P25FE_FMT_CF32>(p.ct, h->long_taps);
         hipLaunchKernelGGL(k, grid, dim3(WV), p.lds, st, a, dt, tail);
+    } else if (L.gate.epoch) {
+        const K1GatedKernel k = p.u8 ? k1_gated_kernel_of<P25FE_FMT_U8>(p.ct, h->long_taps) : k1_gated_kernel_of<P25FE_FMT_CF32>(p.ct, h->long_taps);
+        launch_ev(k, grid, dim3(WV), p.lds, st, L.ev0, L.ev1, a, dt, L.gate);
     } else {
         const K1Kernel k = p.u8 ? k1_kernel_of<P25FE_FMT_U8>(p.ct, p.pk, L.planar, h->long_taps)
                                 : k1_kernel_of<P25FE_FMT_CF32>(p.ct, p.pk, L.planar, h->long_taps);
@@ -863,6 +883,7 @@
     bool wait_head = false;
     const ShardFix* fix = nullptr;
     hipEvent_t ev_done = nullptr;
+    unsigned* delay_word = nullptr; unsigned long long delay_ticks = 0;
     hipStream_t stream = nullptr;
 };
 static RecvCall recv_call(const p25fe_t* h)
@@ -1017,6 +1038,10 @@
     const int n_tiles = n_tiles_of(rc.range);
     const bool detect = rc.detect && n_tiles != 0, slice = rc.slice && n_tiles != 0, scan = rc.fix == nullptr;
     hipStream_t st = rc.stream;
+    if (rc.delay_ticks) {
+        hipLaunchKernelGGL(k_queue_probe_wait, dim3(1), dim3(1), 0, st, rc.delay_word, rc.delay_ticks);
+        HIPCHK(h, hipGetLastError());
+    }
     int e = detect ? launch_detect(h, rc) : P25FE_OK;
     if (e) return e;
     h->prof.mark(2, st, h->ext_events);
@@ -1158,7 +1183,16 @@
 {
     if (!h) return P25FE_ERR_ARG;
     HIPCHK(h, hipSetDevice(h->cfg.device));
-    return pipe_join(h, (hipStream_t)stream);
+    if (int jrc = pipe_join(h, (hipStream_t)stream)) return jrc;
+    volatile unsigned* err = static_cast<volatile unsigned*>(h->gate_err.p);
+    if (err && *err != 0u) {
+        HIPCHK(h, hipStreamSynchronize((hipStream_t)stream));
+        if (h->rx_stream) HIPCHK(h, hipStreamSynchronize(h->rx_stream));
+        for (Lane& l : h->lanes) { l.pending = false; l.joined_any = false; l.epoch = 0u; }
+        *err = 0u;
+        return P25FE_ERR_TIMEOUT;
+    }
+    return P25FE_OK;
 }
 
 static int ensure_rx_stream(p25fe_t* h)
@@ -1186,9 +1220,15 @@
     }
     return P25FE_OK;
 }
-static int pipe_open(p25fe_t* h, hipStream_t st, int depth = 2)
+static int pipe_open(p25fe_t* h, hipStream_t st, int depth = 2, K1Gate* gate = nullptr)
 {
     if (int rc = ensure_rx_stream(h)) return rc;
+    if (gate && !h->gate_words.p) {
+        HIPCHK(h, h->gate_words.ensure(GATE_WORDS * sizeof(unsigned)));
+        HIPCHK(h, hipMemset(h->gate_words.p, 0, GATE_WORDS * sizeof(unsigned)));
+        HIPCHK(h, h->gate_err.ensure(64));
+        memset(h->gate_err.p, 0, 64);
+    }
     for (Lane& l : h->lanes) {
         if (!l.ev_k1) HIPCHK(h, hipEventCreateWithFlags(&l.ev_k1, hipEventDisableTiming));
         if (!l.ev_rx) HIPCHK(h, hipEventCreateWithFlags(&l.ev_rx, hipEventDisableTiming));
@@ -1196,11 +1236,12 @@
     rotate_lanes(&h->cur, h->lane_q, depth);
     Lane& l = h->lane();
     if (l.pending) {
-        const bool nowait = P25FE_M_PIPE_NOWAIT();
-        if (!nowait && !(l.joined_any && l.joined == st)) HIPCHK(h, hipStreamWaitEvent(st, l.ev_rx, 0));
+        if (l.joined_any && l.joined == st) { }
+        else if (gate && l.epoch) *gate = K1Gate{h->gate_words.as<unsigned>() + h->cur, l.epoch, static_cast<unsigned*>(h->gate_err.dp)};
+        else HIPCHK(h, hipStreamWaitEvent(st, l.ev_rx, 0));
         l.pending = false;
     }
-    l.joined_any = false;
+    l.joined_any = false; l.epoch = 0u;
     return P25FE_OK;
 }
 
@@ -1209,7 +1250,8 @@
     if (!h || !d_iq || !dest.dibits || !dest.result || p25fe_n_baseband_h(h, 0, n) > MAX_RANGE_BB) return P25FE_ERR_ARG;
     HIPCHK(h, hipSetDevice(h->cfg.device));
     h->sh.invalidate();
-    if (int orc = pipelined ? pipe_open(h, st, h->run_depth) : pipe_join(h, st)) return orc;
+    K1Gate gate = {nullptr, 0u, nullptr};
+    if (int orc = pipelined ? pipe_open(h, st, h->run_depth, &gate) : pipe_join(h, st)) return orc;
     Lane& lane = h->lane();
     const size_t n_bb = p25fe_n_baseband_h(h, 0, n);
     int rc = ensure_slice_scratch(h, n_bb ? n_bb : 1);
@@ -1221,14 +1263,18 @@
     rcall.dest = dest;
     rcall.stream = pipelined ? h->rx_stream : st;
     if (pipelined && h->ext_events) rcall.ev_done = lane.ev_rx;
+    if (pipelined && h->rx_delay_ticks) { rcall.delay_word = h->gate_words.as<unsigned>() + GATE_DELAY_WORD; rcall.delay_ticks = h->rx_delay_ticks; }
     K1Launch k;
-    k.src = d_iq; k.fmt = fmt; k.ch_stride = ch_stride; k.n = n; k.stream = st;
+    k.src = d_iq; k.fmt = fmt; k.ch_stride = ch_stride; k.n = n; k.stream = st; k.gate = gate;
     if (n_bb) h->prof.begin();
     rc = launch_planar_recv(h, k, rcall, pipelined ? lane.ev_k1 : nullptr);
     h->prof.end();
     if (rc || !pipelined) return rc;
+    if (++h->pipe_seq == 0u) ++h->pipe_seq;
+    hipLaunchKernelGGL(k_epoch_set, dim3(1), dim3(1), 0, h->rx_stream, h->gate_words.as<unsigned>() + h->cur, h->pipe_seq);
+    HIPCHK(h, hipGetLastError());
     if (!h->ext_events) HIPCHK(h, hipEventRecord(lane.ev_rx, h->rx_stream));
-    lane.pending = true;
+    lane.pending = true; lane.epoch = h->pipe_seq;
     return P25FE_OK;
 }
 
@@ -1371,7 +1417,7 @@
     h->sh.pipe = false;
     HIPCHK(h, hipSetDevice(h->cfg.device));
     HIPCHK(h, hipEventRecord(h->lane().ev_rx, last_stream ? (hipStream_t)last_stream : h->rx_stream));
-    h->lane().pending = true;
+    h->lane().pending = true; h->lane().epoch = 0u;
     return P25FE_OK;
 }
 
diff --git a/p25rx_amd/csrc/p25fe_jit.cpp b/p25rx_amd/csrc/p25fe_jit.cpp
--- a/p25rx_amd/csrc/p25fe_jit.cpp
+++ b/p25rx_amd/csrc/p25fe_jit.cpp
@@ -33,8 +33,10 @@
     "{ frontend_body<FMT, true, 5, OM, P25FE_JIT_TX>(a, t); }\n"
     "P25JIT_K1(p25jit_k1_cf32_lin, P25FE_FMT_CF32, OUT_LINEAR, Geo<5>::WAVES_PER_SIMD)\n"
     "P25JIT_K1(p25jit_k1_u8_lin, P25FE_FMT_U8, OUT_LINEAR, Geo<5>::WAVES_PER_SIMD)\n"
-    "P25JIT_K1(p25jit_k1_cf32_pl, P25FE_FMT_CF32, OUT_PLANAR, P25FE_K1_PLANAR_WPS)\n"
-    "P25JIT_K1(p25jit_k1_u8_pl, P25FE_FMT_U8, OUT_PLANAR, (P25FE_JIT_AVG_N > AVG_DPP_MAX ? 2 : P25FE_K1_PLANAR_WPS_U8))\n"
+    "#define P25JIT_K1G(NAME, FMT, WPS) extern \"C\" __global__ __launch_bounds__(WV, WPS) void NAME(K1Args a, const Taps* __restrict__ t, K1Gate g) "
+    "{ frontend_body<FMT, true, 5, OUT_PLANAR, P25FE_JIT_TX, true>(a, t, g); }\n"
+    "P25JIT_K1G(p25jit_k1_cf32_pl, P25FE_FMT_CF32, P25FE_K1_PLANAR_WPS)\n"
+    "P25JIT_K1G(p25jit_k1_u8_pl, P25FE_FMT_U8, (P25FE_JIT_AVG_N > AVG_DPP_MAX ? 2 : P25FE_K1_PLANAR_WPS_U8))\n"
     "extern \"C\" __global__ __launch_bounds__(WV, 2) void p25jit_chunk_cf32(K1Args a, const Taps* __restrict__ t, ChunkTail c) "
     "{ chunk_body<P25FE_FMT_CF32, true, P25FE_JIT_TX>(a, t, c); }\n"
     "extern \"C\" __global__ __launch_bounds__(WV, 2) void p25jit_chunk_u8(K1Args a, const Taps* __restrict__ t, ChunkTail c) "
@@ -88,7 +90,7 @@
 uint64_t spec_hash(const Spec& s)
 {
     uint64_t h = 0xcbf29ce484222325ull;
-    h = fnv(h, "p25fe-jit-2", 11);
+    h = fnv(h, "p25fe-jit-3", 11);
     h = fnv(h, P25FE_SRC_KERNELS, sizeof P25FE_SRC_KERNELS);
     h = fnv(h, P25FE_SRC_RECV, sizeof P25FE_SRC_RECV);
     h = fnv(h, P25FE_SRC_P25FE_H, sizeof P25FE_SRC_P25FE_H);
diff --git a/p25rx_amd/csrc/p25fe_kernels.hip b/p25rx_amd/csrc/p25fe_kernels.hip
--- a/p25rx_amd/csrc/p25fe_kernels.hip
+++ b/p25rx_amd/csrc/p25fe_kernels.hip
@@ -34,7 +34,6 @@
 #define P25FE_M_NO_OUT_STAGE false
 #define P25FE_M_DET_CUT_SCREEN do { } while (0)
 #define P25FE_M_DET_NO_PEAK_TEST false
-#define P25FE_M_PIPE_NOWAIT() false
 #define P25FE_M_API_EXTRAS
 #endif
 
@@ -455,6 +454,16 @@
     int seg_halo;
 };
 
+#ifndef P25FE_HEAD_WAIT_TICKS
+#define P25FE_HEAD_WAIT_TICKS 200000000ull
+#endif
+constexpr unsigned long long HEAD_WAIT_TICKS = P25FE_HEAD_WAIT_TICKS;
+struct K1Gate {
+    const unsigned* epoch;
+    unsigned want;
+    unsigned* err;
+};
+
 #ifndef P25FE_K1_PLANAR_WPS
 #define P25FE_K1_PLANAR_WPS 2
 #endif
@@ -473,14 +482,15 @@
 #ifndef P25FE_K1_PF_U8
 #define P25FE_K1_PF_U8 2
 #endif
-template <int FMT, bool CT, int PK, int OM = OUT_LINEAR, int TX = 0>
-__device__ __forceinline__ void frontend_body(const K1Args& a, const Taps* __restrict__ gtaps)
+template <int FMT, bool CT, int PK, int OM = OUT_LINEAR, int TX = 0, bool GATE = false>
+__device__ __forceinline__ void frontend_body(const K1Args& a, const Taps* __restrict__ gtaps, const K1Gate& gate = K1Gate{nullptr, 0u, nullptr})
 {
     constexpr int PF = (PK != 5 || TX != 0) ? 1 : (FMT == P25FE_FMT_U8 ? P25FE_K1_PF_U8 : P25FE_K1_PF_CF32);
 #ifndef P25FE_JIT
     static_assert(TX == 0 || !CT, "the 64-tap geometry is for caller-supplied taps");
 #endif
     static_assert(OM == OUT_LINEAR || PK == 5, "the planar epilogue maps a 320-sample sub-tile onto 10 planes x 32 symbols");
+    static_assert(!GATE || OM == OUT_PLANAR, "the epoch gate guards the planar scratch");
     P25FE_M_ENTRY;
     using G = Geo<PK, TX>;
     constexpr int SUB = G::SUB;
@@ -530,6 +540,7 @@
     P25FE_M_LOCALS;
     const long n_items = (long)a.seg_count * a.n_ch;
     const bool grid2d = gridDim.x == (unsigned)a.seg_count;
+    int gate_st = GATE && gate.epoch ? 0 : 1;
     for (long item = grid2d ? (long)blockIdx.y * a.seg_count + blockIdx.x : (long)blockIdx.x; item < n_items;
          item += grid2d ? n_items : (long)gridDim.x) {
     P25FE_M_ITEM;
@@ -546,6 +557,9 @@
     const char* xb = reinterpret_cast<const char*>(a.x) + (size_t)ch * a.ch_stride * (FMT == P25FE_FMT_CF32 ? 8 : 2);
     float* bb = a.bb + (size_t)ch * a.bb_stride;
     phase_sync();
+    unsigned gate_v = 0u;
+    if constexpr (GATE)
+        if (gate_st == 0 && tid == 0) gate_v = __hip_atomic_load(gate.epoch, __ATOMIC_RELAXED, __HIP_MEMORY_SCOPE_AGENT);
 
     using LoaderT = Loader<FMT, PK, TX>;
     using LoaderP = Loader<FMT, PK, TX, NVP>;
@@ -657,6 +671,21 @@
     uint8_t* const bits_ch = OM == OUT_PLANAR ? a.bits + (size_t)ch * a.bits_ch_stride : nullptr;
     unsigned bitsv = 0u;
     auto flush_outputs = [&]() {
+        if constexpr (GATE) {
+            if (gate_st == 0) gate_st = (int)((unsigned)__builtin_amdgcn_readfirstlane((int)gate_v) - gate.want) >= 0 ? 1 : 3;
+            if (gate_st == 3 && out_rel != -2 * SUB) {
+                const unsigned long long t0 = wall_clock64();
+                while (gate_st == 3) {
+                    __builtin_amdgcn_s_sleep(16);
+                    unsigned v = 0u;
+                    if (tid == 0) v = __hip_atomic_load(gate.epoch, __ATOMIC_RELAXED, __HIP_MEMORY_SCOPE_AGENT);
+                    if ((int)((unsigned)__builtin_amdgcn_readfirstlane((int)v) - gate.want) >= 0) gate_st = 1;
+                    else if (wall_clock64() - t0 > HEAD_WAIT_TICKS) gate_st = 2;
+                }
+                if (gate_st == 2 && tid == 0) __hip_atomic_store(gate.err, gate.want, __ATOMIC_RELAXED, __HIP_MEMORY_SCOPE_SYSTEM);
+            }
+            if (gate_st == 2) return;
+        }
         if constexpr (OM == OUT_LINEAR) {
 #pragma unroll
             for (int q = 0; q < P; ++q) {
@@ -967,6 +996,11 @@
 __global__ __launch_bounds__(WV, k1_wps(FMT, CT, PK, OM)) void k_frontend(K1Args a, const Taps* __restrict__ gtaps)
 {
     frontend_body<FMT, CT, PK, OM, TX>(a, gtaps);
+}
+template <int FMT, bool CT, int TX = 0>
+__global__ __launch_bounds__(WV, k1_wps(FMT, CT, 5, OUT_PLANAR)) void k_frontend_gated(K1Args a, const Taps* __restrict__ gtaps, K1Gate g)
+{
+    frontend_body<FMT, CT, 5, OUT_PLANAR, TX, true>(a, gtaps, g);
 }
 
 constexpr int PD = P25FE_PRE_DECIM;
@@ -1487,6 +1521,7 @@
     word[1] = seen ? 1u : 2u;
 }
 __global__ void k_queue_probe_set(unsigned* word) { __hip_atomic_store(word, 1u, __ATOMIC_RELAXED, __HIP_MEMORY_SCOPE_AGENT); }
+__global__ void k_epoch_set(unsigned* word, unsigned seq) { __hip_atomic_store(word, seq, __ATOMIC_RELAXED, __HIP_MEMORY_SCOPE_AGENT); }
 #endif
 
 #ifndef P25FE_JIT
diff --git a/p25rx_amd/csrc/p25fe_measure.inc b/p25rx_amd/csrc/p25fe_measure.inc
--- a/p25rx_amd/csrc/p25fe_measure.inc
+++ b/p25rx_amd/csrc/p25fe_measure.inc
@@ -139,11 +139,6 @@
         return; } } while (0)
 #define P25FE_M_DET_NO_PEAK_TEST (P25FE_ABLATE_DET == 2)
 
-#ifdef P25FE_MEASURE_UNSAFE
-#define P25FE_M_PIPE_NOWAIT() ([] { static const bool nowait = [] { const char* e = getenv("P25FE_PIPE_NOWAIT"); return e && atoi(e) != 0; }(); return nowait; }())
-#else
-#define P25FE_M_PIPE_NOWAIT() false
-#endif
 #ifdef P25FE_K1_STAMP
 #define P25FE_M_API_EXTRAS                                                                                               \
     int p25fe_debug_k1_stamps(uint64_t out[16])                                                                          \
diff --git a/p25rx_amd/csrc/p25fe_recv.hip b/p25rx_amd/csrc/p25fe_recv.hip
--- a/p25rx_amd/csrc/p25fe_recv.hip
+++ b/p25rx_amd/csrc/p25fe_recv.hip
@@ -231,10 +231,6 @@
 }
 
 constexpr int GT = 64;
-#ifndef P25FE_HEAD_WAIT_TICKS
-#define P25FE_HEAD_WAIT_TICKS 200000000ull
-#endif
-constexpr unsigned long long HEAD_WAIT_TICKS = P25FE_HEAD_WAIT_TICKS;
 struct GroupAgg {
     long first_event;
     long last_s;
diff --git a/p25rx_amd/frontend.py b/p25rx_amd/frontend.py
--- a/p25rx_amd/frontend.py
+++ b/p25rx_amd/frontend.py
@@ -197,7 +197,7 @@
         self._chk(self.L.p25fe_run_dev_pipelined(self.h, C.c_void_p(iq.data_ptr()), fmt, stride, n,
                                                  C.c_void_p(dibits.data_ptr()), dibits.stride(0),
                                                  C.c_void_p(result.data_ptr()), self._stream()))
-        self._inflight = (getattr(self, "_inflight", ()) + ((dibits, result),))[-2:]
+        self._inflight = (getattr(self, "_inflight", ()) + ((dibits, result),))[-4:]
         return dibits, result
 
     def join_dev(self):
```

Result: no change. 545,500 (-0.9%).
